# octree-nn/octfusion

Measured on AMD Instinct MI355X. Metric: denoising-steps/sec (depth-8 octree, batch 8), higher is better.
Workload: dtype f32 storage, fp16x3 products (fp16 hi + lo operand pairs = 22 significand bits, three fp16 MFMAs per product, fp32 accumulate)

## Files before the change

### include/ofx.h

```cpp
#ifndef OFX_H_
#define OFX_H_

#include <stddef.h>
#include <stdint.h>

#ifdef __cplusplus
extern "C" {
#endif

#define OFX_OK 0
#define OFX_EINVAL (-1)
#define OFX_ELAUNCH (-2)
#define OFX_ENODEV (-3)

#define OFX_ACT_NONE 0
#define OFX_ACT_SILU 1
#define OFX_ACT_GELU 2

#define OFX_MAX_DEPTH 16

int ofx_version(void);
const char* ofx_status_string(int status);
int ofx_device_check(void);
const char* ofx_build_hash(void);

int ofx_set_range_words(uint32_t* words);

int ofx_probe_mfma_sustained(int steps, int blocks, float* sink, unsigned long long* ticks, void* stream);

size_t ofx_scan_ws_bytes(int64_t n);
int ofx_scan_i32(const int32_t* in, int32_t* out, int64_t n, void* ws, void* stream);


int ofx_octree_full_layer(int depth, int batch_size, int64_t* keys, int32_t* children,
                          void* stream);
int ofx_octree_split(const int32_t* label, int64_t n, int32_t* children, int32_t* scan_out,
                     void* ws, void* stream);
int ofx_octree_grow(const int64_t* keys_parent, const int32_t* children_parent, int64_t n_parent,
                    int64_t* keys_child, int32_t* children_child, void* stream);
int ofx_split_small_label0(const float* split, int batch_size, int full_depth,
                           int32_t* label, void* stream);
int ofx_split_small_label1(const float* split, int batch_size, int full_depth,
                           const int32_t* children, int32_t* label1, void* stream);
int ofx_split_large_label0(const float* split, int64_t n, int32_t* label0, void* stream);
int ofx_split_large_label1(const float* split, int64_t n, const int32_t* children,
                           int32_t* label1, void* stream);
int ofx_octree2voxel_cf(const float* data, int64_t ld, int C, int batch_size, int depth,
                        float* vox, void* stream);
int ofx_voxel2octree_cf(const float* vox, int C, int batch_size, int depth, float* data,
                        int64_t ld, void* stream);

typedef struct {
  int depth, full_depth, batch_size;
  const int32_t* child_all;
  const int64_t* key_all;
  const int32_t* leafrank_all;
  const int64_t* nnum_host;
  const int64_t* nnum_nempty_host;
} ofx_tree_t;

size_t ofx_points_sort_ws_bytes(int64_t n);
int ofx_points_keys(const float* pts, int64_t ldp, const int32_t* batch_id, int batch_const, int64_t n, int depth,
                    int64_t* keys, int32_t* idx, void* stream);
int ofx_points_sort(const int64_t* keys_in, const int32_t* idx_in, int64_t n, int64_t* keys_out, int32_t* idx_out,
                    void* ws, size_t ws_bytes, void* stream);
int ofx_octree_label_from_points(const int64_t* sorted_keys, int64_t n_pts, const int64_t* node_keys, int64_t nnum,
                                 int depth_pts, int d, int32_t* label, void* stream);
int ofx_octree_point_features(const int64_t* sorted_keys, const int32_t* sorted_idx, int64_t n_pts, const float* pts,
                              int64_t ldp, const float* normals, int64_t ldn, const int64_t* node_keys, int64_t nnum,
                              int depth, float* feat, float* avg_points, float* avg_normals, void* stream);
size_t ofx_tree_leafrank_ws_bytes(int64_t max_nnum);
int ofx_tree_leafrank(const int32_t* child_all, const int64_t* nnum_host, int depth,
                      int32_t* leafrank_all, void* ws, void* stream);
int ofx_graph_nodes(const ofx_tree_t* tree, int d, int32_t* batch_id, uint8_t* node_type,
                    int64_t* keyd, uint8_t* node_mask, void* stream);
int ofx_graph_count(const ofx_tree_t* tree, int d, int32_t* seg_cnt, void* stream);
int ofx_graph_fill(const ofx_tree_t* tree, int d, const int32_t* seg_ptr, int32_t* col,
                   void* stream);
int ofx_graph_expand(const int32_t* seg_ptr, int64_t n_nodes, const int32_t* col,
                     int64_t* row_out, int64_t* col_out, int64_t* dir_out, void* stream);
int ofx_graph_primary(const int32_t* seg_ptr, const int32_t* col, int64_t n_nodes, int32_t* nbr,
                      void* stream);
int ofx_graph_reverse_count(const int32_t* seg_ptr, const int32_t* col, int64_t n_nodes, int32_t* rev_cnt,
                            void* stream);
int ofx_graph_reverse_fill(const int32_t* seg_ptr, const int32_t* col, int64_t n_nodes, const int32_t* rev_ptr,
                           int32_t* cursor, int32_t* rev_row, float* rev_w, void* stream);
int ofx_graph_primary_w(const int32_t* seg_ptr, const int32_t* col, const float* w, int64_t n_nodes, int32_t* nbr,
                        void* stream);
int ofx_graph_multi_flag_w(const int32_t* seg_ptr, const float* w, int64_t n_nodes, int32_t* flag, void* stream);
int ofx_graph_primary_ext_w(const int32_t* seg_ptr, const int32_t* col, const float* w, int64_t n_nodes,
                            const int32_t* rank, int32_t* nbr_ext, int32_t* multi_seg, void* stream);
int ofx_graphconv_bwd_data(const float* dy, int64_t ldy, int cout, int64_t n_nodes, const int32_t* nbr_rev,
                           const int32_t* rev_ptr, const int32_t* rev_row, const float* rev_w,
                           const int32_t* nbr_ext_rev, const int32_t* multi_seg, int64_t n_multi, float* aux,
                           const float* WpT, int64_t KpT, int cin, float* dx, int64_t ldx, void* ws, size_t ws_bytes,
                           void* stream);
int ofx_graphconv_bwd_weight(const float* x, int64_t ldx, int cin, int64_t n_nodes, const int32_t* nbr,
                             const int32_t* seg_ptr, const int32_t* col, const int32_t* nbr_ext,
                             const int32_t* multi_seg, int64_t n_multi, float* aux, const float* type_frac, int64_t ldt,
                             int nt_pad, const float* dy, int64_t ldy, int cout, float* dWp, int64_t Kp, void* ws,
                             size_t ws_bytes, void* stream);
int ofx_gn_backward(const float* x, int64_t ldx, const float* dy, int64_t ldy, int64_t n, int C,
                    const int32_t* batch_id, int batch_size, const float* count, int groups, float count_eps,
                    const float* mean, const float* rstd, const float* w, const float* bias, int act, double* sums,
                    float* coef, float* dx, int64_t lddx, float* dgamma, float* dbeta, void* stream);
int ofx_gemm_tn_f32(const float* P, int64_t ldp, const float* Q, int64_t ldq, int64_t rows, int64_t K, int64_t N,
                    float* out, void* ws, size_t ws_bytes, void* stream);
int ofx_table_reverse_count(const int32_t* nbr, int64_t n_out, int ndir, int64_t n_in, int32_t* rev_cnt, void* stream);
int ofx_table_reverse_fill(const int32_t* nbr, int64_t n_out, int ndir, int64_t n_in, const int32_t* rev_ptr,
                           int32_t* cursor, int32_t* rev_row, float* rev_w, void* stream);
int ofx_seg_primary_w(const int32_t* seg_ptr, const int32_t* col, const float* w, int64_t nseg, int32_t* nbr,
                      void* stream);
int ofx_seg_multi_flag_w(const int32_t* seg_ptr, const float* w, int64_t nseg, int32_t* flag, void* stream);
int ofx_seg_primary_ext_w(const int32_t* seg_ptr, const int32_t* col, const float* w, int64_t nseg, int64_t n_src,
                          const int32_t* rank, int32_t* nbr_ext, int32_t* multi_seg, void* stream);
int ofx_gridconv_bwd_data(const float* dy, int64_t ldy, int cout, int64_t n_out, int64_t n_in, const int32_t* nbr_rev,
                          const int32_t* rev_ptr, const int32_t* rev_row, const float* rev_w,
                          const int32_t* nbr_ext_rev, const int32_t* multi_seg, int64_t n_multi, float* aux,
                          const float* WpT, int cin, float* dx, int64_t ldx, void* ws, size_t ws_bytes, void* stream);
int ofx_gridconv_bwd_weight(const float* x, int64_t ldx, int cin, int64_t n_in, int64_t n_out, const int32_t* nbr27,
                            const int32_t* nbr27_ext, const float* zero_row, const float* dy, int64_t ldy, int cout,
                            float* dWp, void* ws, size_t ws_bytes, void* stream);
int ofx_adamw_step(float* param, const float* grad, float* exp_avg, float* exp_avg_sq, int64_t n, float lr,
                   float beta1, float beta2, float eps, float weight_decay, int step, void* stream);
int ofx_ema_update(float* ema, const float* param, int64_t n, float beta, void* stream);
int ofx_mpu_eval(const ofx_tree_t* tree, int depth_start, int depth_end, const float* pts, int64_t n_pts,
                 const float* code, float* sdf, uint8_t* mask, void* stream);
int ofx_mpu_eval_grid(const ofx_tree_t* tree, int depth_start, int depth_end, const float* code, int size,
                      float step, float bbmin, int batch_index, int64_t head, int64_t count, float* sdf,
                      uint8_t* mask, void* stream);
int ofx_mpu_eval_grad(const ofx_tree_t* tree, int depth_start, int depth_end, const float* pts, int64_t n_pts,
                      const float* code, float* sdf, float* grad, uint8_t* mask, void* stream);
int ofx_mpu_backward(const ofx_tree_t* tree, int depth_start, int depth_end, const float* pts, int64_t n_pts,
                     const float* code, const float* dsdf, const float* dgrad, float* dcode, void* stream);
int ofx_octree_ce(const float* logits, int64_t ld, const int32_t* child, int64_t n, float dscale, double* sums,
                  float* dlogits, int64_t ldd, void* stream);
int ofx_sdf_reg_loss(const float* sdf, const float* grad, const float* sdf_gt, const float* grad_gt, int64_t n,
                     float w_sdf, float w_grad, double* sums, float* dsdf, float* dgrad, void* stream);
int ofx_kl_sample_fwd(const float* params, int64_t ld, const float* noise, int64_t n, int embed_dim, float* z,
                      double* kl_sum, void* stream);
int ofx_kl_sample_bwd(const float* params, int64_t ld, const float* noise, const float* dz, int64_t n,
                      int embed_dim, float kl_scale, float* dparams, int64_t ldp, void* stream);
int ofx_graph_multi_flag(const int32_t* seg_ptr, int64_t n_nodes, int32_t* flag, void* stream);
int ofx_graph_primary_ext(const int32_t* seg_ptr, const int32_t* col, int64_t n_nodes,
                          const int32_t* rank, int32_t* nbr_ext, int32_t* multi_seg, void* stream);
int ofx_graph_type_frac(const int32_t* seg_ptr, const int32_t* col, const uint8_t* node_type,
                        int64_t n_nodes, int nt, float* type_frac, int64_t ld, void* stream);

int ofx_set_precision(int mode);
int ofx_get_precision(void);
int64_t ofx_packed_floats(int64_t Kp, int64_t N);
int64_t ofx_packed_k(int64_t K);
int64_t ofx_graphconv_packed_k(int cin, int nt);
int ofx_pack_weights(const float* W, int64_t sk, int64_t sn, int64_t K, int64_t N,
                     int cin, int nt, float* Wp, int64_t Kp, void* stream);

int ofx_gemm_f32(const float* A, int64_t lda, const int32_t* a_rows, int64_t M, int64_t K,
                 const float* Wp, int64_t Kp, int64_t N, const float* bias,
                 const float* res, int64_t ldr, float* out, int64_t ldc,
                 const int32_t* out_rows, void* ws, size_t ws_bytes, void* stream);
int ofx_gemm_f32_planes(const float* A, int64_t lda, const int32_t* a_rows, int64_t M, int64_t K,
                        const float* Wp, int64_t Kp, int64_t N, const float* bias,
                        const float* res, int64_t ldr, float* out, int64_t ldc,
                        const int32_t* out_rows, void* ws, size_t ws_bytes, int out_mode, void* stream);

int ofx_graphconv_fwd(const float* x, int64_t ldx, int cin, int64_t n_nodes,
                      const int32_t* nbr, const int32_t* seg_ptr, const int32_t* col,
                      const int32_t* nbr_ext, const int32_t* multi_seg, int64_t n_multi, float* aux,
                      const float* type_frac, int64_t ldt, int nt_pad,
                      const float* Wp, int64_t Kp, int cout, const float* bias,
                      const float* emb, int64_t lde, const int32_t* batch_id,
                      const float* res, int64_t ldr, float* out, int64_t ldc,
                      double* stats , int64_t stats_ld,
                      void* ws, size_t ws_bytes, void* stream);

int ofx_graphconv_narrow_in(const float* x, int64_t ldx, int cin, int64_t n_nodes, const int32_t* seg_ptr,
                            const int32_t* col, const uint8_t* node_type, int nt, const float* W, int cout,
                            const float* bias, const int32_t* batch_id, float* out, int64_t ldc,
                            double* stats , int64_t stats_ld, void* ws, size_t ws_bytes, void* stream);
int ofx_graphconv_narrow_in_tab(const float* x, int64_t ldx, int cin, int64_t n_nodes, const int32_t* seg_ptr,
                                const int32_t* col, const int32_t* nbr_ext, const int32_t* multi_seg, int64_t n_multi,
                                void* aux, const uint8_t* node_type, int nt, const float* W, int cout, const float* bias,
                                const int32_t* batch_id, float* out, int64_t ldc, double* stats ,
                                int64_t stats_ld, void* ws, size_t ws_bytes, void* stream);
int ofx_narrow_out_pack(const float* W, int C, int nt, int cout, int pw, float* Wd, void* stream);
int ofx_narrow_out_type_term(const float* type_frac, int64_t ldt, int nt, int64_t n_nodes, const float* W, int C,
                             int cout, const float* bias, float* type_term, void* stream);
int ofx_graphconv_narrow_out(const float* P, int64_t ldp, int cout, int64_t n_nodes, const int32_t* seg_ptr,
                             const int32_t* col, const float* type_term , float* out, int64_t ldc,
                             void* stream);

int ofx_planes_split(const float* x, int64_t ldx, int64_t n, int C, int Cpad, int mode, void* out,
                     int64_t ldo_bytes, void* stream);
int ofx_planes_merge(const void* planes, int64_t ldp_bytes, int64_t n, int C, int mode, float* out, int64_t ldo,
                     void* stream);
int ofx_gn_apply_planes(const float* x, int64_t ldx, int64_t n, int C, const int32_t* batch_id, const float* mean,
                        const float* rstd, const double* sums, const float* count, int groups, float eps,
                        float count_eps, const float* w, const float* bias, int act, int mode, void* out,
                        int64_t ldo_bytes, const int32_t* seg_ptr, const int32_t* col, const int32_t* multi_seg,
                        int64_t n_multi, void* aux , const int32_t* aux_plan ,
                        int64_t aux_left, void* stream);
int ofx_gn_apply_planes_oct(const float* x, int64_t ldx, int64_t n, int C, const int32_t* batch_id, const float* mean,
                            const float* rstd, const double* sums, const float* count, int groups, float eps,
                            float count_eps, const float* w, const float* bias, int act, int mode, void* out,
                            int64_t ldo_bytes, int64_t n_multi, void* aux, const int32_t* oct_ptr,
                            const int32_t* oct_ent, int64_t n_own, int shift, const int32_t* left_head,
                            const int32_t* left_src, int64_t n_left, void* stream);
int ofx_gn_apply_rows(void);
int64_t ofx_planes_packed_ktiles(int cin, int nt, int mode);
int64_t ofx_planes_packed_bytes(int cin, int nt, int cout, int mode);
int ofx_pack_weights_planes(const float* W, int64_t sk, int64_t sn, int cin, int nt, int cout, int mode, void* out,
                            void* stream);
int ofx_graphconv_fwd_planes(const void* xp, int64_t ldx_bytes, int cin, int64_t n_nodes, const int32_t* seg_ptr,
                             const int32_t* col, const int32_t* nbr_ext, const int32_t* multi_seg, int64_t n_multi,
                             void* aux, size_t aux_bytes, const void* tfp, int64_t ldt_bytes, int nt, const void* W2,
                             int cout, const float* bias, const float* emb, int64_t lde, const int32_t* batch_id,
                             const float* res, int64_t ldr, float* out, int64_t ldc, double* stats ,
                             int64_t stats_ld, void* ws, size_t ws_bytes, void* sync , size_t sync_bytes,
                             int mode, int aux_ready, void* stream);
int ofx_set_gconv_persistent(int on);
int64_t ofx_gemm_planes_packed_bytes(int K, int N, int mode);
int ofx_pack_gemm_planes(const float* W, int64_t sk, int64_t sn, int K, int N, int mode, void* out, void* stream);
int ofx_gemm_planes(const void* ap, int64_t lda_bytes, int64_t n_a, int64_t M, int K, const int32_t* row_tab,
                    const void* W2, int N, const float* bias, float* out, int64_t ldc, int out_mode, void* ws,
                    size_t ws_bytes, void* sync, size_t sync_bytes, int mode, void* stream);
int ofx_set_gconv_cus(int cus);
int ofx_gconv3_plan(int64_t n_rows, int cout, int nkt, int wm, int ni, int cus, int32_t* out, int64_t out_len);
int ofx_set_gconv2_tile(int wm);

int ofx_grid_conv_table(int mode, int depth_out, int batch_size, int32_t pad, int32_t* nbr27,
                        void* stream);
int64_t ofx_conv3d_packed_k(int cin);
int ofx_pack_conv3d(const float* W, int cin, int cout, float* Wp, void* stream);
int ofx_gridconv_fwd(const float* x, int64_t ldx, int cin, int64_t n_in, int64_t n_out,
                     const int32_t* nbr27 ,
                     const int32_t* nbr27_ext ,
                     const float* zero_row ,
                     const float* Wp, int cout, const float* bias, const float* emb, int64_t lde,
                     const int32_t* batch_id, const float* res, int64_t ldr, float* out,
                     int64_t ldc, void* ws, size_t ws_bytes, void* stream);
int ofx_gather_gemm_f32(const float* x, int64_t ldx, int cin, int ntap, int64_t n_src, int64_t n_out, const int32_t* tab,
                        const float* zero_row, const float* Wp, int64_t Kp, int cout, const float* bias,
                        const float* res, int64_t ldr, float* out, int64_t ldc, const int32_t* out_rows, void* ws,
                        size_t ws_bytes, int out_mode, void* stream);
int ofx_set_attention_split(int on);
int ofx_attention(const float* qkv, int64_t ldq, int batch_size, int T, int heads, int ch,
                  float* out, int64_t ldo, void* stream);

int ofx_attention_bwd(const float* qkv, int64_t ldq, const float* dout, int64_t ldo, int batch_size, int T, int heads,
                      int ch, float* rowstat, float* dqkv, int64_t ldd, void* stream);

int ofx_gather_mean(const float* x, int64_t ldx, int cin, int64_t n_nodes,
                    const int32_t* seg_ptr, const int32_t* col, float* col_data,
                    void* stream);

int ofx_gn_stats(const float* x, int64_t ldx, int64_t n, int C, const int32_t* batch_id,
                 int batch_size, double* sums, void* stream);
int ofx_gn_stats_acc(const float* x, int64_t ldx, int64_t n, int C, const int32_t* batch_id, int batch_size,
                     double* sums, void* stream);
int ofx_gn_finalize(const double* sums, const float* count, int batch_size, int C, int groups,
                    float eps, float count_eps, float* mean, float* rstd, void* stream);
int ofx_gn_apply(const float* x, int64_t ldx, int64_t n, int C, const int32_t* batch_id,
                 const float* mean , const float* rstd , const double* sums ,
                 const float* count, int groups, float eps, float count_eps, const float* w, const float* bias,
                 int act, float* out, int64_t ldo, void* stream);

int ofx_gn_fused_rows(const float* x, int64_t ldx, int rows_per_batch, int batch_size, int C, int groups, float eps,
                      float count_eps, const float* w, const float* bias, int act, float* out, int64_t ldo,
                      void* stream);

int ofx_set_gn_rows16(int on);

int ofx_rows_copy(const float* src, int64_t lds, const int32_t* smap, float* dst, int64_t ldd,
                  const int32_t* dmap, int64_t n, int C, void* stream);
int ofx_rows_copy_planes(const float* src, int64_t lds, const int32_t* smap, float* dst, int64_t ldd,
                         const int32_t* dmap, int64_t n, int C, int mode, void* stream);
int ofx_act(const float* x, float* y, int64_t n, int act, void* stream);
int ofx_timestep_embedding(const float* t, int batch_size, int dim, float max_period,
                           float* out, void* stream);
int ofx_learned_sinusoid(const float* t, const float* w, int batch_size, int half, float* out, void* stream);
int ofx_linear_small(const float* a, int64_t lda, int M, int K, const float* W, int64_t ldw, int N, const float* bias,
                     const float* res, int64_t ldr, int act_in, int act_out, float* out, int64_t ldo, void* stream);
int ofx_ddim_eps_update(float* x, const float* eps, const float* coef, float* x0_out, int64_t n,
                        void* stream);
int ofx_ddim_x0_update(float* x, const float* x0, const float* noise, const float* coef,
                       int64_t n, void* stream);

size_t ofx_mc_ws_bytes(int batch, int size);
int ofx_mc_count(const float* sdf, int batch, int size, float level, void* ws, int64_t* counts, void* stream);
int ofx_mc_emit(const float* sdf, int batch, int size, float level, float step, float bbmin, float scale, void* ws,
                const int64_t* vert_off, const int64_t* tri_off, float* verts, int32_t* faces, void* stream);
int ofx_mc_table_host(int8_t* tri_table, uint8_t* ntri);

size_t ofx_mesh_cc_ws_bytes(int64_t total_verts, int64_t total_faces, int batch);
int ofx_mesh_cc_label(const int32_t* faces, const int64_t* vert_off, const int64_t* tri_off, int batch,
                      int64_t total_verts, int64_t total_faces, int32_t* label, void* ws, int32_t* status,
                      void* stream);
int ofx_mesh_cc_table(const int32_t* faces, const int32_t* label, const int64_t* vert_off, const int64_t* tri_off,
                      int batch, int64_t total_verts, int64_t total_faces, int32_t* comp_of_vert, int32_t* comp_off,
                      void* ws, const int32_t* status, void* stream);
int ofx_mesh_cc_stats(const float* verts, const int32_t* faces, const int32_t* label, const int64_t* vert_off,
                      const int64_t* tri_off, int batch, int64_t total_verts, int64_t total_faces, int64_t n_comp,
                      int32_t* table, void* ws, const int32_t* status, void* stream);
int ofx_mesh_cc_select(const float* verts, const int32_t* faces, const int32_t* label, const int64_t* vert_off,
                       const int64_t* tri_off, int batch, int64_t total_verts, int64_t total_faces,
                       int32_t* winner_label, int64_t* keep_counts, void* ws, const int32_t* status, void* stream);
int ofx_mesh_cc_extract(const float* verts, const int32_t* faces, const int64_t* vert_off, const int64_t* tri_off,
                        int batch, int64_t total_verts, int64_t total_faces, const int64_t* new_vert_off,
                        const int64_t* new_tri_off, float* out_verts, int32_t* out_faces, void* ws,
                        const int32_t* status, void* stream);

#define OFX_EMD_MAX_POINTS 2048
size_t ofx_surface_sample_ws_bytes(int batch, int64_t total_faces);
int ofx_surface_sample(const float* verts, const int32_t* faces, const int64_t* offs, const int64_t* ids, int batch,
                       int64_t total_faces, int n, uint64_t seed, int normalize, void* ws, float* out, void* stream);
int ofx_nn_matrix(const float* a, int64_t na, int n, const float* b, int64_t nb, int m, float* d, void* stream);
int ofx_emd_matrix(const float* x, int64_t nx, const float* y, int64_t ny, int n, int m, float* e, void* stream);
uint64_t ofx_metrics_hash(uint64_t seed, int64_t shape, int64_t point, int draw);

#ifdef __cplusplus
}
#endif
#endif
```

### octfusion_amd/_lib.py

```python
import ctypes
import os

import torch

_HERE = os.path.dirname(os.path.abspath(__file__))
LIB_PATH = os.environ.get('OFX_LIB', os.path.join(_HERE, 'libofx.so'))

c_p = ctypes.c_void_p
c_i = ctypes.c_int
c_l = ctypes.c_int64
c_f = ctypes.c_float
c_sz = ctypes.c_size_t
c_u64 = ctypes.c_uint64


class OfxTree(ctypes.Structure):
    _fields_ = [('depth', c_i), ('full_depth', c_i), ('batch_size', c_i),
                ('child_all', c_p), ('key_all', c_p), ('leafrank_all', c_p),
                ('nnum_host', c_p), ('nnum_nempty_host', c_p)]


_SIGS = {
    'ofx_version': (c_i, [], False),
    'ofx_status_string': (ctypes.c_char_p, [c_i], False),
    'ofx_device_check': (c_i, [], False),
    'ofx_build_hash': (ctypes.c_char_p, [], False),
    'ofx_probe_mfma_sustained': (c_i, [c_i, c_i, c_p, c_p, c_p], True),
    'ofx_scan_ws_bytes': (c_sz, [c_l], False),
    'ofx_scan_i32': (c_i, [c_p, c_p, c_l, c_p, c_p], True),
    'ofx_octree_full_layer': (c_i, [c_i, c_i, c_p, c_p, c_p], True),
    'ofx_octree_split': (c_i, [c_p, c_l, c_p, c_p, c_p, c_p], True),
    'ofx_octree_grow': (c_i, [c_p, c_p, c_l, c_p, c_p, c_p], True),
    'ofx_split_small_label0': (c_i, [c_p, c_i, c_i, c_p, c_p], True),
    'ofx_split_small_label1': (c_i, [c_p, c_i, c_i, c_p, c_p, c_p], True),
    'ofx_split_large_label0': (c_i, [c_p, c_l, c_p, c_p], True),
    'ofx_split_large_label1': (c_i, [c_p, c_l, c_p, c_p, c_p], True),
    'ofx_octree2voxel_cf': (c_i, [c_p, c_l, c_i, c_i, c_i, c_p, c_p], True),
    'ofx_voxel2octree_cf': (c_i, [c_p, c_i, c_i, c_i, c_p, c_l, c_p], True),
    'ofx_points_sort_ws_bytes': (c_sz, [c_l], False),
    'ofx_points_keys': (c_i, [c_p, c_l, c_p, c_i, c_l, c_i, c_p, c_p, c_p], True),
    'ofx_points_sort': (c_i, [c_p, c_p, c_l, c_p, c_p, c_p, c_sz, c_p], True),
    'ofx_octree_label_from_points': (c_i, [c_p, c_l, c_p, c_l, c_i, c_i, c_p, c_p], True),
    'ofx_octree_point_features': (c_i, [c_p, c_p, c_l, c_p, c_l, c_p, c_l, c_p, c_l, c_i, c_p, c_p, c_p, c_p], True),
    'ofx_tree_leafrank_ws_bytes': (c_sz, [c_l], False),
    'ofx_tree_leafrank': (c_i, [c_p, c_p, c_i, c_p, c_p, c_p], True),
    'ofx_graph_nodes': (c_i, [ctypes.POINTER(OfxTree), c_i, c_p, c_p, c_p, c_p, c_p], True),
    'ofx_graph_count': (c_i, [ctypes.POINTER(OfxTree), c_i, c_p, c_p], True),
    'ofx_graph_reverse_count': (c_i, [c_p, c_p, c_l, c_p, c_p], True),
    'ofx_graph_reverse_fill': (c_i, [c_p, c_p, c_l, c_p, c_p, c_p, c_p, c_p], True),
    'ofx_graph_primary_w': (c_i, [c_p, c_p, c_p, c_l, c_p, c_p], True),
    'ofx_graph_multi_flag_w': (c_i, [c_p, c_p, c_l, c_p, c_p], True),
    'ofx_graph_primary_ext_w': (c_i, [c_p, c_p, c_p, c_l, c_p, c_p, c_p, c_p], True),
    'ofx_graphconv_bwd_data': (c_i, [c_p, c_l, c_i, c_l, c_p, c_p, c_p, c_p, c_p, c_p, c_l, c_p, c_p, c_l, c_i, c_p,
                                     c_l, c_p, c_sz, c_p], True),
    'ofx_graphconv_bwd_weight': (c_i, [c_p, c_l, c_i, c_l, c_p, c_p, c_p, c_p, c_p, c_l, c_p, c_p, c_l, c_i, c_p, c_l,
                                       c_i, c_p, c_l, c_p, c_sz, c_p], True),
    'ofx_gn_backward': (c_i, [c_p, c_l, c_p, c_l, c_l, c_i, c_p, c_i, c_p, c_i, c_f, c_p, c_p, c_p, c_p, c_i, c_p, c_p,
                              c_p, c_l, c_p, c_p, c_p], True),
    'ofx_gemm_tn_f32': (c_i, [c_p, c_l, c_p, c_l, c_l, c_l, c_l, c_p, c_p, c_sz, c_p], True),
    'ofx_table_reverse_count': (c_i, [c_p, c_l, c_i, c_l, c_p, c_p], True),
    'ofx_table_reverse_fill': (c_i, [c_p, c_l, c_i, c_l, c_p, c_p, c_p, c_p, c_p], True),
    'ofx_seg_primary_w': (c_i, [c_p, c_p, c_p, c_l, c_p, c_p], True),
    'ofx_seg_multi_flag_w': (c_i, [c_p, c_p, c_l, c_p, c_p], True),
    'ofx_seg_primary_ext_w': (c_i, [c_p, c_p, c_p, c_l, c_l, c_p, c_p, c_p, c_p], True),
    'ofx_gridconv_bwd_data': (c_i, [c_p, c_l, c_i, c_l, c_l, c_p, c_p, c_p, c_p, c_p, c_p, c_l, c_p, c_p, c_i, c_p, c_l,
                                    c_p, c_sz, c_p], True),
    'ofx_gridconv_bwd_weight': (c_i, [c_p, c_l, c_i, c_l, c_l, c_p, c_p, c_p, c_p, c_l, c_i, c_p, c_p, c_sz, c_p], True),
    'ofx_attention_bwd': (c_i, [c_p, c_l, c_p, c_l, c_i, c_i, c_i, c_i, c_p, c_p, c_l, c_p], True),
    'ofx_adamw_step': (c_i, [c_p, c_p, c_p, c_p, c_l, c_f, c_f, c_f, c_f, c_f, c_i, c_p], True),
    'ofx_ema_update': (c_i, [c_p, c_p, c_l, c_f, c_p], True),
    'ofx_gn_fused_rows': (c_i, [c_p, c_l, c_i, c_i, c_i, c_i, c_f, c_f, c_p, c_p, c_i, c_p, c_l, c_p], True),
    'ofx_set_gn_rows16': (c_i, [c_i], True),
    'ofx_mpu_eval': (c_i, [ctypes.POINTER(OfxTree), c_i, c_i, c_p, c_l, c_p, c_p, c_p, c_p], True),
    'ofx_mpu_eval_grid': (c_i, [ctypes.POINTER(OfxTree), c_i, c_i, c_p, c_i, c_f, c_f, c_i, c_l, c_l, c_p, c_p, c_p], True),
    'ofx_mpu_eval_grad': (c_i, [ctypes.POINTER(OfxTree), c_i, c_i, c_p, c_l, c_p, c_p, c_p, c_p, c_p], True),
    'ofx_mpu_backward': (c_i, [ctypes.POINTER(OfxTree), c_i, c_i, c_p, c_l, c_p, c_p, c_p, c_p, c_p], True),
    'ofx_octree_ce': (c_i, [c_p, c_l, c_p, c_l, c_f, c_p, c_p, c_l, c_p], True),
    'ofx_sdf_reg_loss': (c_i, [c_p, c_p, c_p, c_p, c_l, c_f, c_f, c_p, c_p, c_p, c_p], True),
    'ofx_kl_sample_fwd': (c_i, [c_p, c_l, c_p, c_l, c_i, c_p, c_p, c_p], True),
    'ofx_kl_sample_bwd': (c_i, [c_p, c_l, c_p, c_p, c_l, c_i, c_f, c_p, c_l, c_p], True),
    'ofx_graph_fill': (c_i, [ctypes.POINTER(OfxTree), c_i, c_p, c_p, c_p], True),
    'ofx_graph_expand': (c_i, [c_p, c_l, c_p, c_p, c_p, c_p, c_p], True),
    'ofx_graph_type_frac': (c_i, [c_p, c_p, c_p, c_l, c_i, c_p, c_l, c_p], True),
    'ofx_set_precision': (c_i, [c_i], True),
    'ofx_set_range_words': (c_i, [c_p], True),
    'ofx_get_precision': (c_i, [], False),
    'ofx_gn_apply_rows': (c_i, [], False),
    'ofx_set_attention_split': (c_i, [c_i], True),
    'ofx_gather_gemm_f32': (c_i, [c_p, c_l, c_i, c_i, c_l, c_l, c_p, c_p, c_p, c_l, c_i, c_p, c_p, c_l, c_p, c_l, c_p, c_p, c_sz, c_i, c_p], True),
    'ofx_graphconv_narrow_in_tab': (c_i, [c_p, c_l, c_i, c_l, c_p, c_p, c_p, c_p, c_l, c_p, c_p, c_i, c_p, c_i, c_p, c_p, c_p, c_l, c_p, c_l,
                                          c_p, c_sz, c_p], True),
    'ofx_graphconv_narrow_in': (c_i, [c_p, c_l, c_i, c_l, c_p, c_p, c_p, c_i, c_p, c_i, c_p, c_p, c_p, c_l, c_p, c_l, c_p, c_sz, c_p], True),
    'ofx_narrow_out_pack': (c_i, [c_p, c_i, c_i, c_i, c_i, c_p, c_p], True),
    'ofx_narrow_out_type_term': (c_i, [c_p, c_l, c_i, c_l, c_p, c_i, c_i, c_p, c_p, c_p], True),
    'ofx_graphconv_narrow_out': (c_i, [c_p, c_l, c_i, c_l, c_p, c_p, c_p, c_p, c_l, c_p], True),
    'ofx_packed_floats': (c_l, [c_l, c_l], False),
    'ofx_packed_k': (c_l, [c_l], False),
    'ofx_graphconv_packed_k': (c_l, [c_i, c_i], False),
    'ofx_pack_weights': (c_i, [c_p, c_l, c_l, c_l, c_l, c_i, c_i, c_p, c_l, c_p], True),
    'ofx_gemm_f32': (c_i, [c_p, c_l, c_p, c_l, c_l, c_p, c_l, c_l, c_p, c_p, c_l, c_p, c_l, c_p, c_p, c_sz, c_p], True),
    'ofx_gemm_f32_planes': (c_i, [c_p, c_l, c_p, c_l, c_l, c_p, c_l, c_l, c_p, c_p, c_l, c_p, c_l, c_p, c_p, c_sz, c_i, c_p], True),
    'ofx_graphconv_fwd': (c_i, [c_p, c_l, c_i, c_l, c_p, c_p, c_p, c_p, c_p, c_l, c_p, c_p, c_l, c_i, c_p, c_l,
                                c_i, c_p, c_p, c_l, c_p, c_p, c_l, c_p, c_l, c_p, c_l, c_p, c_sz, c_p], True),
    'ofx_planes_split': (c_i, [c_p, c_l, c_l, c_i, c_i, c_i, c_p, c_l, c_p], True),
    'ofx_planes_merge': (c_i, [c_p, c_l, c_l, c_i, c_i, c_p, c_l, c_p], True),
    'ofx_gn_apply_planes': (c_i, [c_p, c_l, c_l, c_i, c_p, c_p, c_p, c_p, c_p, c_i, c_f, c_f, c_p, c_p, c_i, c_i, c_p,
                                  c_l, c_p, c_p, c_p, c_l, c_p, c_p, c_l, c_p], True),
    'ofx_gn_apply_planes_oct': (c_i, [c_p, c_l, c_l, c_i, c_p, c_p, c_p, c_p, c_p, c_i, c_f, c_f, c_p, c_p, c_i, c_i, c_p,
                                      c_l, c_l, c_p, c_p, c_p, c_l, c_i, c_p, c_p, c_l, c_p], True),
    'ofx_planes_packed_ktiles': (c_l, [c_i, c_i, c_i], False),
    'ofx_planes_packed_bytes': (c_l, [c_i, c_i, c_i, c_i], False),
    'ofx_pack_weights_planes': (c_i, [c_p, c_l, c_l, c_i, c_i, c_i, c_i, c_p, c_p], True),
    'ofx_graphconv_fwd_planes': (c_i, [c_p, c_l, c_i, c_l, c_p, c_p, c_p, c_p, c_l, c_p, c_sz, c_p, c_l, c_i, c_p, c_i,
                                       c_p, c_p, c_l, c_p, c_p, c_l, c_p, c_l, c_p, c_l, c_p, c_sz, c_p, c_sz, c_i, c_i,
                                       c_p], True),
    'ofx_set_gconv_persistent': (c_i, [c_i], True),
    'ofx_set_gconv_cus': (c_i, [c_i], True),
    'ofx_gemm_planes_packed_bytes': (c_l, [c_i, c_i, c_i], False),
    'ofx_pack_gemm_planes': (c_i, [c_p, c_l, c_l, c_i, c_i, c_i, c_p, c_p], True),
    'ofx_gemm_planes': (c_i, [c_p, c_l, c_l, c_l, c_i, c_p, c_p, c_i, c_p, c_p, c_l, c_i, c_p, c_sz, c_p, c_sz, c_i, c_p], False),
    'ofx_gconv3_plan': (c_i, [c_l, c_i, c_i, c_i, c_i, c_i, c_p, c_l], False),
    'ofx_set_gconv2_tile': (c_i, [c_i], True),
    'ofx_graph_multi_flag': (c_i, [c_p, c_l, c_p, c_p], True),
    'ofx_graph_primary_ext': (c_i, [c_p, c_p, c_l, c_p, c_p, c_p, c_p], True),
    'ofx_graph_primary': (c_i, [c_p, c_p, c_l, c_p, c_p], True),
    'ofx_grid_conv_table': (c_i, [c_i, c_i, c_i, c_i, c_p, c_p], True),
    'ofx_conv3d_packed_k': (c_l, [c_i], False),
    'ofx_pack_conv3d': (c_i, [c_p, c_i, c_i, c_p, c_p], True),
    'ofx_gridconv_fwd': (c_i, [c_p, c_l, c_i, c_l, c_l, c_p, c_p, c_p, c_p, c_i, c_p, c_p, c_l, c_p, c_p, c_l, c_p,
                               c_l, c_p, c_sz, c_p], True),
    'ofx_attention': (c_i, [c_p, c_l, c_i, c_i, c_i, c_i, c_p, c_l, c_p], True),
    'ofx_gather_mean': (c_i, [c_p, c_l, c_i, c_l, c_p, c_p, c_p, c_p], True),
    'ofx_gn_stats': (c_i, [c_p, c_l, c_l, c_i, c_p, c_i, c_p, c_p], True),
    'ofx_gn_stats_acc': (c_i, [c_p, c_l, c_l, c_i, c_p, c_i, c_p, c_p], True),
    'ofx_gn_finalize': (c_i, [c_p, c_p, c_i, c_i, c_i, c_f, c_f, c_p, c_p, c_p], True),
    'ofx_gn_apply': (c_i, [c_p, c_l, c_l, c_i, c_p, c_p, c_p, c_p, c_p, c_i, c_f, c_f, c_p, c_p, c_i, c_p, c_l, c_p], True),
    'ofx_rows_copy': (c_i, [c_p, c_l, c_p, c_p, c_l, c_p, c_l, c_i, c_p], True),
    'ofx_rows_copy_planes': (c_i, [c_p, c_l, c_p, c_p, c_l, c_p, c_l, c_i, c_i, c_p], True),
    'ofx_act': (c_i, [c_p, c_p, c_l, c_i, c_p], True),
    'ofx_timestep_embedding': (c_i, [c_p, c_i, c_i, c_f, c_p, c_p], True),
    'ofx_learned_sinusoid': (c_i, [c_p, c_p, c_i, c_i, c_p, c_p], True),
    'ofx_linear_small': (c_i, [c_p, c_l, c_i, c_i, c_p, c_l, c_i, c_p, c_p, c_l, c_i, c_i, c_p, c_l, c_p], True),
    'ofx_ddim_eps_update': (c_i, [c_p, c_p, c_p, c_p, c_l, c_p], True),
    'ofx_ddim_x0_update': (c_i, [c_p, c_p, c_p, c_p, c_l, c_p], True),
    'ofx_mc_ws_bytes': (c_sz, [c_i, c_i], False),
    'ofx_mc_count': (c_i, [c_p, c_i, c_i, c_f, c_p, c_p, c_p], True),
    'ofx_mc_emit': (c_i, [c_p, c_i, c_i, c_f, c_f, c_f, c_f, c_p, c_p, c_p, c_p, c_p, c_p], True),
    'ofx_mc_table_host': (c_i, [c_p, c_p], True),
    'ofx_mesh_cc_ws_bytes': (c_sz, [c_l, c_l, c_i], False),
    'ofx_mesh_cc_label': (c_i, [c_p, c_p, c_p, c_i, c_l, c_l, c_p, c_p, c_p, c_p], True),
    'ofx_mesh_cc_table': (c_i, [c_p, c_p, c_p, c_p, c_i, c_l, c_l, c_p, c_p, c_p, c_p, c_p], True),
    'ofx_mesh_cc_stats': (c_i, [c_p, c_p, c_p, c_p, c_p, c_i, c_l, c_l, c_l, c_p, c_p, c_p, c_p], True),
    'ofx_mesh_cc_select': (c_i, [c_p, c_p, c_p, c_p, c_p, c_i, c_l, c_l, c_p, c_p, c_p, c_p, c_p], True),
    'ofx_mesh_cc_extract': (c_i, [c_p, c_p, c_p, c_p, c_i, c_l, c_l, c_p, c_p, c_p, c_p, c_p, c_p, c_p], True),
    'ofx_surface_sample_ws_bytes':(c_sz, [c_i, c_l], False),
    'ofx_surface_sample': (c_i, [c_p, c_p, c_p, c_p, c_i, c_l, c_i, c_u64, c_i, c_p, c_p, c_p], True),
    'ofx_nn_matrix': (c_i, [c_p, c_l, c_i, c_p, c_l, c_i, c_p, c_p], True),
    'ofx_emd_matrix': (c_i, [c_p, c_l, c_p, c_l, c_i, c_i, c_p, c_p], True),
    'ofx_metrics_hash': (c_u64, [c_u64, c_l, c_l, c_i], False),
}

EXPORTS = sorted(_SIGS)


class OfxError(RuntimeError):
    pass


_lib = None


def lib():
    global _lib
    if _lib is None:
        if not os.path.exists(LIB_PATH):
            raise OfxError('libofx.so not built: run `python -m octfusion_amd.build` '
                           '(the product has no CPU / eager fallback)')
        L = ctypes.CDLL(LIB_PATH)
        for name, (res, args, _) in _SIGS.items():
            fn = getattr(L, name)
            fn.restype = res
            fn.argtypes = args
        _check_fresh(L)
        _lib = L
    return _lib


def _check_fresh(L):
    if 'OFX_LIB' in os.environ:
        return
    from . import build
    try:
        want = build.source_hash()
    except OSError:
        return
    have = L.ofx_build_hash().decode()
    if have != want:
        raise OfxError('libofx.so is stale: built from sources %s, the tree is %s -- run `python -m octfusion_amd.build`'
                       % (have, want))


PROFILE = None
META = None


def _timed(prof, name, args, always):
    global META
    meta, META = META, None
    e0 = torch.cuda.Event(enable_timing=True)
    e1 = torch.cuda.Event(enable_timing=True)
    e0.record()
    rc = getattr(lib(), name)(*args)
    e1.record()
    if always or rc == 0:
        prof.append((name, e0, e1, meta))
    return rc


def call(name, *args):
    prof = PROFILE
    if prof is not None and _SIGS[name][2]:
        rc = _timed(prof, name, args, True)
    else:
        rc = getattr(lib(), name)(*args)
    if _SIGS[name][2] and rc != 0:
        msg = lib().ofx_status_string(rc).decode()
        raise OfxError('%s failed: %s (%d)' % (name, msg, rc))
    return rc


def call_may_decline(name, *args):
    prof = PROFILE
    if prof is not None:
        rc = _timed(prof, name, args, False)
    else:
        rc = getattr(lib(), name)(*args)
    if rc < 0:
        raise OfxError('%s failed with status %d' % (name, rc))
    return rc == 0


def ptr(t):
    if t is None:
        return None
    return t.data_ptr()


def stream():
    return torch.cuda.current_stream().cuda_stream


def require_device():
    if not torch.cuda.is_available():
        raise OfxError('no HIP device: octfusion_amd has no CPU path')
    rc = lib().ofx_device_check()
    if rc != 0:
        raise OfxError('ofx_device_check: %s' % lib().ofx_status_string(rc).decode())
```

### octfusion_amd/csrc/ofx_gemm.hip

```cpp
#include "ofx_gemm_common.h"

constexpr int BM = 128;
constexpr int BK = 32;
constexpr int A_LD = BK + 4;
constexpr int MODE_DENSE = 0;
constexpr int MODE_GATHER = 1;


__device__ __forceinline__ float4 gather_seg4(const GemmArgs& g, int64_t row, int dir, int cc) {
  const int64_t s = row * g.ndir + dir;
  const int32_t a = g.seg_ptr[s], e = g.seg_ptr[s + 1];
  float4 acc = f4zero();
  if (g.edge_w) {
    for (int32_t p = a; p < e; ++p) {
      const float w = g.edge_w[p];
      const float4 v = *reinterpret_cast<const float4*>(g.x + (int64_t)g.col[p] * g.ldx + cc);
      acc.x += w * v.x; acc.y += w * v.y; acc.z += w * v.z; acc.w += w * v.w;
    }
    return acc;
  }
  for (int32_t p = a; p < e; ++p) f4add(acc, *reinterpret_cast<const float4*>(g.x + (int64_t)g.col[p] * g.ldx + cc));
  if (e - a > 1) {
    const float inv = 1.f / (float)(e - a);
    acc.x *= inv; acc.y *= inv; acc.z *= inv; acc.w *= inv;
// ... 818 lines not shown
}

__global__ void __launch_bounds__(256) splitk_reduce_kernel(const GemmArgs g) {
  const int64_t total = g.M * g.N;
  for (int64_t t = (int64_t)blockIdx.x * blockDim.x + threadIdx.x; t < total; t += (int64_t)gridDim.x * blockDim.x) {
    const int64_t m = t / g.N, n = t - m * g.N;
    float v = 0.f;
    for (int s = 0; s < g.nsplit; ++s) v += g.ws[(int64_t)s * total + t];
    if (g.oscale_p) v *= *g.oscale_p;
    if (g.bias) v += g.bias[n];
    if (g.emb) v += g.emb[(int64_t)g.bid[m] * g.lde + n];
    if (g.res) v += g.res[m * g.ldr + n];
    int64_t om = m;
    if (g.out_rows) { om = g.out_rows[m]; if (om < 0) continue; }
    g.out[om * g.ldc + n] = v;
  }
}

__global__ void __launch_bounds__(256) splitk_reduce_v4_kernel(const GemmArgs g) {
  const int64_t n4 = g.N >> 2, total4 = g.M * n4, total = g.M * g.N;
  for (int64_t t = (int64_t)blockIdx.x * blockDim.x + threadIdx.x; t < total4; t += (int64_t)gridDim.x * blockDim.x) {
    const int64_t m = t / n4, n = (t - m * n4) * 4;
    const float* p = g.ws + m * g.N + n;
    float4 v = f4zero();
    int s = 0;
    for (; s + 7 < g.nsplit; s += 8) {
      float4 a[8];
#pragma unroll
      for (int u = 0; u < 8; ++u) a[u] = *reinterpret_cast<const float4*>(p + (int64_t)(s + u) * total);
#pragma unroll
      for (int u = 0; u < 8; ++u) f4add(v, a[u]);
    }
    for (; s + 3 < g.nsplit; s += 4) {
      const float4 a0 = *reinterpret_cast<const float4*>(p + (int64_t)s * total);
      const float4 a1 = *reinterpret_cast<const float4*>(p + (int64_t)(s + 1) * total);
      const float4 a2 = *reinterpret_cast<const float4*>(p + (int64_t)(s + 2) * total);
      const float4 a3 = *reinterpret_cast<const float4*>(p + (int64_t)(s + 3) * total);
      f4add(v, a0); f4add(v, a1); f4add(v, a2); f4add(v, a3);
    }
    for (; s < g.nsplit; ++s) f4add(v, *reinterpret_cast<const float4*>(p + (int64_t)s * total));
    if (g.oscale_p) { const float osc = *g.oscale_p; v.x *= osc; v.y *= osc; v.z *= osc; v.w *= osc; }
    if (g.bias) f4add(v, *reinterpret_cast<const float4*>(g.bias + n));
    if (g.emb) f4add(v, *reinterpret_cast<const float4*>(g.emb + (int64_t)g.bid[m] * g.lde + n));
    if (g.res) f4add(v, *reinterpret_cast<const float4*>(g.res + m * g.ldr + n));
    int64_t om = m;
    if (g.out_rows) { om = g.out_rows[m]; if (om < 0) continue; }
    if (g.out_planes) ofx_store_planes4(g.out, om * g.ldc + n, v, g.out_planes);
    else *reinterpret_cast<float4*>(g.out + om * g.ldc + n) = v;
  }
}

template <int MODE, int WM, int WN, int MI, int NI>
static int launch_cfg(GemmArgs& g, hipStream_t st) {
  constexpr int BN = WN * NI * 32;
  constexpr size_t lds = (2 * BM * A_LD + 2 * 8 * BN * 4) * sizeof(float);
  static bool attr_set[OFX_MAX_DEVICES] = {};
  if (lds > 64 * 1024 &&
      !ofx_raise_lds_limit(reinterpret_cast<const void*>(&gemm_kernel<MODE, WM, WN, MI, NI>), (int)lds, attr_set))
    return OFX_ELAUNCH;
  gemm_kernel<MODE, WM, WN, MI, NI><<<g.ntm * g.ntn * g.nsplit, 256, lds, st>>>(g);
  return OFX_OK;
}

template <int MODE, int WM, int WN, int MI, int NI>
static int launch_fast_cfg(GemmArgs& g, hipStream_t st) {
  constexpr int BN = WN * NI * 32;
  constexpr size_t lds = (2 * BM * A_LD + 2 * 8 * BN * 4) * sizeof(float);
  static bool attr_set[OFX_MAX_DEVICES] = {};
  if (lds > 64 * 1024 &&
      !ofx_raise_lds_limit(reinterpret_cast<const void*>(&gemm_fast_kernel<MODE, WM, WN, MI, NI>), (int)lds, attr_set))
    return OFX_ELAUNCH;
  gemm_fast_kernel<MODE, WM, WN, MI, NI><<<g.ntm * g.ntn * g.nsplit, 256, lds, st>>>(g);
  return OFX_OK;
}

template <int MODE, int WM, int WN, int MI, int NI, int H16>
static int launch_bf16x3_h(GemmArgs& g, hipStream_t st) {
  constexpr int BN = WN * NI * 32;
  constexpr size_t lds = 2 * (2 * BM * 80);
  static bool attr_set[OFX_MAX_DEVICES] = {};
  if (lds > 64 * 1024 &&
      !ofx_raise_lds_limit(reinterpret_cast<const void*>(&gemm_pairs_x3_kernel<MODE, WM, WN, MI, NI, H16>), (int)lds, attr_set))
    return OFX_ELAUNCH;
  gemm_pairs_x3_kernel<MODE, WM, WN, MI, NI, H16><<<g.ntm * g.ntn * g.nsplit, 256, lds, st>>>(g);
  return OFX_OK;
}
template <int MODE, int WM, int WN, int MI, int NI>
static int launch_bf16x3_cfg(GemmArgs& g, hipStream_t st) {
  return g_precision == 3 ? launch_bf16x3_h<MODE, WM, WN, MI, NI, 1>(g, st) : launch_bf16x3_h<MODE, WM, WN, MI, NI, 0>(g, st);
}

__global__ void __launch_bounds__(256) stats_reduce_kernel(const float* __restrict__ part, int64_t nwr, int wr_rows,
                                                            int64_t N, const int32_t* __restrict__ bid,
                                                            double* __restrict__ stats, int64_t stats_ld) {
  __shared__ double red[3][64][2];
  const int c = threadIdx.x & 63, rg = threadIdx.x >> 6;
  const int64_t n = (int64_t)blockIdx.y * 64 + c;
  const int64_t w0 = (int64_t)blockIdx.x * 64;
  const int64_t nc = n < N ? n : N - 1;
  int b[16];
  float2 v[16];
#pragma unroll
  for (int i = 0; i < 16; ++i) {
    const int64_t w = w0 + rg * 16 + i;
    const int64_t wc = w < nwr ? w : nwr - 1;
    b[i] = bid[wc * wr_rows];
    v[i] = *reinterpret_cast<const float2*>(part + (wc * N + nc) * 2);
    if (w >= nwr) { b[i] = -1; v[i] = make_float2(0.f, 0.f); }
  }
  const int bfirst = bid[w0 * wr_rows];
  bool ok = true;
#pragma unroll
  for (int i = 0; i < 16; ++i) ok = ok && (b[i] == bfirst || b[i] < 0);
  const bool uni = __syncthreads_and(ok);
  auto flush = [&](int bb, double s, double q) {
    double* o = stats + ((int64_t)bb * stats_ld + n) * 2;
    unsafeAtomicAdd(o, s); unsafeAtomicAdd(o + 1, q);
  };
  if (uni) {
    double s = 0.0, q = 0.0;
#pragma unroll
    for (int i = 0; i < 16; ++i) { s += (double)v[i].x; q += (double)v[i].y; }
    if (rg > 0) { red[rg - 1][c][0] = s; red[rg - 1][c][1] = q; }
    __syncthreads();
    if (rg == 0 && n < N) {
#pragma unroll
      for (int r = 0; r < 3; ++r) { s += red[r][c][0]; q += red[r][c][1]; }
      flush(bfirst, s, q);
    }
  } else if (n < N) {
    double s = 0.0, q = 0.0;
    int sb = -1;
#pragma unroll
    for (int i = 0; i < 16; ++i) {
      if (b[i] < 0) continue;
      if (b[i] != sb) {
        if (sb >= 0) flush(sb, s, q);
        sb = b[i]; s = 0.0; q = 0.0;
      }
      s += (double)v[i].x; q += (double)v[i].y;
    }
    if (sb >= 0) flush(sb, s, q);
  }
}

int ofx_launch_stats_reduce(const GemmArgs& g, int wr_rows, hipStream_t st) {
  const int64_t nwr = ofx_cdiv(g.M, wr_rows);
  stats_reduce_kernel<<<dim3((unsigned)ofx_cdiv(nwr, 64), (unsigned)ofx_cdiv(g.N, 64)), 256, 0, st>>>(
      g.stats_part, nwr, wr_rows, g.N, g.bid, g.stats, g.stats_ld);
  OFX_LAUNCH_CHECK();
  return OFX_OK;
}

template <int MODE>
static int launch_gemm(GemmArgs& g, float* ws, size_t ws_bytes, hipStream_t st) {
  if (g.M <= 0 || g.N <= 0) return OFX_OK;
  {
    auto al16 = [](const void* p) { return (reinterpret_cast<uintptr_t>(p) & 15) == 0; };
    g.vec4 = g.N % 4 == 0 && al16(g.out) && g.ldc % 4 == 0 && (!g.res || (al16(g.res) && g.ldr % 4 == 0)) &&
             (!g.emb || (al16(g.emb) && g.lde % 4 == 0)) && (!g.bias || al16(g.bias));
  }
  const int bn = g.N <= 32 ? 32 : (g.N <= 64 ? 64 : 128);
  g.ntm = (int)ofx_cdiv(g.M, BM);
  g.ntn = (int)ofx_cdiv(g.N, bn);
  const int nkt = (int)(g.Kp / BK);
  int nsplit = 1;
  const int tiles = g.ntm * g.ntn;
  if (ws && tiles < 256 && nkt >= 8) {
    nsplit = (int)ofx_cdiv(512, tiles);
    if (nsplit > nkt / 4) nsplit = nkt / 4;
    if (nsplit > 64) nsplit = 64;
    const size_t per = (size_t)g.M * g.N * sizeof(float);
    if ((size_t)nsplit * per > ws_bytes) nsplit = (int)(ws_bytes / per);
    if (nsplit < 2) nsplit = 1;
  }
  g.kt_per_split = (int)ofx_cdiv(nkt, nsplit);
  nsplit = (int)ofx_cdiv(nkt, g.kt_per_split);
  g.nsplit = nsplit;
  g.ws = ws;
  int rc;
  bool fast;
  if (MODE == MODE_GATHER) {
    fast = g.fast && g.nbr_ext && g.aux && (!g.out_rows || g.gather_out_rows);
  } else {
    fast = ((g.lda & 3) == 0) && ((g.K & 3) == 0) && g.K >= 4 && ((((uintptr_t)g.A) & 15) == 0);
    if (fast) { g.ndir = 1; g.n_src = 0; g.aux = g.A; g.tf = g.A; g.ldt = g.lda; g.nbr_ext = (const int32_t*)g.A; }
  }
  g.W16 = (g_precision != 1) ? reinterpret_cast<const uint16_t*>(g.Wp + g.Kp * g.N) : nullptr;
  const int wr_rows = bn == 32 ? 32 : 64;
  const int64_t nwr = ofx_cdiv(g.M, wr_rows);
  if (!(g.stats && g.vec4 && nsplit == 1 && g.stats_part &&
        (size_t)nwr * g.N * 2 * sizeof(float) <= g.stats_part_bytes && (((uintptr_t)g.stats_part) & 15) == 0))
    g.stats_part = nullptr;
  g.oscale_p = (fast && g.W16) ? g.Wp + 2 * g.Kp * g.N : nullptr;
  if (fast && g.W16) {
    if (bn == 32) rc = launch_bf16x3_cfg<MODE, 4, 1, 1, 1>(g, st);
    else if (bn == 64) rc = launch_bf16x3_cfg<MODE, 2, 2, 2, 1>(g, st);
    else rc = launch_bf16x3_cfg<MODE, 2, 2, 2, 2>(g, st);
  } else if (fast) {
    if (bn == 32) rc = launch_fast_cfg<MODE, 4, 1, 1, 1>(g, st);
    else if (bn == 64) rc = launch_fast_cfg<MODE, 2, 2, 2, 1>(g, st);
    else rc = launch_fast_cfg<MODE, 2, 2, 2, 2>(g, st);
  } else if (bn == 32) rc = launch_cfg<MODE, 4, 1, 1, 1>(g, st);
  else if (bn == 64) rc = launch_cfg<MODE, 2, 2, 2, 1>(g, st);
  else rc = launch_cfg<MODE, 2, 2, 2, 2>(g, st);
  if (rc) return rc;
  if (nsplit > 1) {
    const bool ws16 = (((uintptr_t)g.ws) & 15) == 0;
    if (g.vec4 && ws16) splitk_reduce_v4_kernel<<<ofx_grid(g.M * (g.N >> 2), 256), 256, 0, st>>>(g);
    else splitk_reduce_kernel<<<ofx_grid(g.M * g.N, 256), 256, 0, st>>>(g);
  }
  if (g.stats_part) {
    rc = ofx_launch_stats_reduce(g, wr_rows, st);
    if (rc) return rc;
  }
  OFX_LAUNCH_CHECK();
  return OFX_OK;
}

static inline int64_t pad32(int64_t v) { return (v + 31) / 32 * 32; }
static int pack_bf16x3(const float* Wp, int64_t Kp, int64_t N, hipStream_t st);

extern "C" int64_t ofx_packed_k(int64_t K) { return pad32(K); }
extern "C" int64_t ofx_graphconv_packed_k(int cin, int nt) {
  return pad32(7 * (int64_t)cin) + (nt > 1 ? pad32(7 * (int64_t)nt) : 0);
}

__global__ void pack_weights_kernel(const float* __restrict__ W, int64_t sk, int64_t sn, int64_t K, int64_t N, int cin,
                                    int nt, float* __restrict__ Wp, int64_t Kp) {
  const int64_t total = (Kp / 4) * N;
  const int ntc = nt > 1 ? nt : 0;
  const int64_t Kf = (7 * (int64_t)cin + 31) / 32 * 32;
  for (int64_t t = (int64_t)blockIdx.x * blockDim.x + threadIdx.x; t < total; t += (int64_t)gridDim.x * blockDim.x) {
    const int64_t kq = t / N, n = t - kq * N;
    float v[4];
#pragma unroll
    for (int kk = 0; kk < 4; ++kk) {
      const int64_t k = kq * 4 + kk;
      int64_t src = -1;
      if (cin > 0) {
        if (k < 7 * (int64_t)cin) {
          const int64_t dir = k / cin, c = k - dir * cin;
          src = dir * (cin + ntc) + c;
        } else if (k >= Kf && ntc > 0 && k - Kf < 7 * (int64_t)ntc) {
          const int64_t kt = k - Kf, dir = kt / ntc, ty = kt - dir * ntc;
          src = dir * (cin + ntc) + cin + ty;
        }
      } else if (k < K) {
        src = k;
      }
      v[kk] = src >= 0 ? W[src * sk + n * sn] : 0.f;
    }
    *reinterpret_cast<float4*>(Wp + t * 4) = make_float4(v[0], v[1], v[2], v[3]);
  }
}

extern "C" int ofx_pack_weights(const float* W, int64_t sk, int64_t sn, int64_t K, int64_t N, int cin, int nt,
                                float* Wp, int64_t Kp, void* stream) {
  if (!W || !Wp || K < 1 || N < 1 || (Kp & 31) || cin < 0 || nt < 0) return OFX_EINVAL;
  if (cin > 0) {
    if (Kp != ofx_graphconv_packed_k(cin, nt) || K != 7 * (int64_t)(cin + (nt > 1 ? nt : 0))) return OFX_EINVAL;
  } else if (Kp != pad32(K)) {
    return OFX_EINVAL;
  }
  if (((uintptr_t)Wp & 15) != 0) return OFX_EINVAL;
  pack_weights_kernel<<<ofx_grid((Kp / 4) * N, 256), 256, 0, ofx_stream(stream)>>>(W, sk, sn, K, N, cin, nt, Wp, Kp);
  if (int rc = pack_bf16x3(Wp, Kp, N, ofx_stream(stream))) return rc;
  OFX_LAUNCH_CHECK();
  return OFX_OK;
}

__global__ void pack_conv3d_kernel(const float* __restrict__ W, int cin, int64_t N, float* __restrict__ Wp, int64_t Kp) {
  const int64_t total = (Kp / 4) * N;
  for (int64_t t = (int64_t)blockIdx.x * blockDim.x + threadIdx.x; t < total; t += (int64_t)gridDim.x * blockDim.x) {
    const int64_t kq = t / N, n = t - kq * N;
    float v[4];
#pragma unroll
    for (int kk = 0; kk < 4; ++kk) {
      const int64_t k = kq * 4 + kk;
      float w = 0.f;
      if (k < 27 * (int64_t)cin) {
        const int64_t tap = k / cin, c = k - tap * cin;
        w = W[(n * cin + c) * 27 + tap];
      }
      v[kk] = w;
    }
    *reinterpret_cast<float4*>(Wp + t * 4) = make_float4(v[0], v[1], v[2], v[3]);
  }
}

extern "C" int64_t ofx_conv3d_packed_k(int cin) { return pad32(27 * (int64_t)cin); }

extern "C" int ofx_pack_conv3d(const float* W, int cin, int cout, float* Wp, void* stream) {
  if (!W || !Wp || cin < 1 || cout < 1 || ((uintptr_t)Wp & 15)) return OFX_EINVAL;
  const int64_t Kp = ofx_conv3d_packed_k(cin);
  pack_conv3d_kernel<<<ofx_grid((Kp / 4) * cout, 256), 256, 0, ofx_stream(stream)>>>(W, cin, cout, Wp, Kp);
  if (int rc = pack_bf16x3(Wp, Kp, cout, ofx_stream(stream))) return rc;
  OFX_LAUNCH_CHECK();
  return OFX_OK;
}

extern "C" int ofx_gemm_f32_planes(const float* A, int64_t lda, const int32_t* a_rows, int64_t M, int64_t K,
                                   const float* Wp, int64_t Kp, int64_t N, const float* bias, const float* res, int64_t ldr,
                                   float* out, int64_t ldc, const int32_t* out_rows, void* ws, size_t ws_bytes,
                                   int out_mode, void* stream) {
  if (M == 0 && K >= 1 && N >= 1) return OFX_OK;
  if (M < 0 || K < 1 || N < 1 || !Wp || !out || (M > 0 && !A) || Kp != pad32(K) || lda < K || ldc < N ||
      (res && ldr < N) || ((uintptr_t)Wp & 15))
    return OFX_EINVAL;
  if (out_mode != 0 && out_mode != 2 && out_mode != 3) return OFX_EINVAL;
  if (out_mode && ((N & 3) || (ldc & 31) || ((uintptr_t)out & 127) || (res && ((ldr & 3) || ((uintptr_t)res & 15))) ||
                   (bias && ((uintptr_t)bias & 15)) || ((uintptr_t)ws & 15)))
    return OFX_EINVAL;
  GemmArgs g = {};
  g.A = A; g.lda = lda; g.a_rows = a_rows;
  g.M = M; g.K = K; g.Wp = Wp; g.Kp = Kp; g.N = N; g.bias = bias;
  g.res = res; g.ldr = ldr; g.out = out; g.ldc = ldc; g.out_rows = out_rows; g.out_planes = out_mode;
  return launch_gemm<MODE_DENSE>(g, (float*)ws, ws_bytes, ofx_stream(stream));
}
extern "C" int ofx_gemm_f32(const float* A, int64_t lda, const int32_t* a_rows, int64_t M, int64_t K, const float* Wp,
                            int64_t Kp, int64_t N, const float* bias, const float* res, int64_t ldr, float* out,
                            int64_t ldc, const int32_t* out_rows, void* ws, size_t ws_bytes, void* stream) {
  return ofx_gemm_f32_planes(A, lda, a_rows, M, K, Wp, Kp, N, bias, res, ldr, out, ldc, out_rows, ws, ws_bytes, 0, stream);
}

static int gather_common(GemmArgs& g, const float* x, int64_t ldx, int cin, int ndir, int64_t n_rows,
                         const int32_t* nbr, const int32_t* seg_ptr, const int32_t* col, const float* Wp, int64_t Kp,
                         int cout, const float* bias, const float* emb, int64_t lde, const int32_t* batch_id,
                         const float* res, int64_t ldr, float* out, int64_t ldc) {
  if (n_rows < 0 || cin < 1 || cout < 1 || !x || !nbr || !Wp || !out || ldx < cin || ldc < cout ||
      (res && ldr < cout) || (emb && (!batch_id || lde < cout)) || ((uintptr_t)Wp & 15))
    return OFX_EINVAL;
  g.x = x; g.ldx = ldx; g.cin = cin; g.ndir = ndir;
  g.fast = (cin % 32 == 0) && ((ldx & 3) == 0) && (((uintptr_t)x & 15) == 0);
  g.nbr = nbr; g.seg_ptr = seg_ptr; g.col = col;
  g.Kf = pad32((int64_t)ndir * cin);
  g.M = n_rows; g.K = Kp; g.Wp = Wp; g.Kp = Kp; g.N = cout; g.bias = bias;
  g.emb = emb; g.lde = lde; g.bid = batch_id; g.res = res; g.ldr = ldr; g.out = out; g.ldc = ldc;
  return OFX_OK;
}

__global__ void __launch_bounds__(256) col_rows_kernel(const GemmArgs g, int64_t row0, int64_t rows,
                                                       float* __restrict__ colbuf) {
  const int64_t k4n = g.Kp >> 2, total = rows * k4n;
  for (int64_t t = (int64_t)blockIdx.x * blockDim.x + threadIdx.x; t < total; t += (int64_t)gridDim.x * blockDim.x) {
    const int64_t r = t / k4n, k = (t - r * k4n) * 4;
    const int64_t row = row0 + r;
    float v[4];
#pragma unroll
    for (int kk = 0; kk < 4; ++kk)
      v[kk] = (k + kk < g.Kf) ? gather_elem(g, row, k + kk) : g.tf[row * g.ldt + (k + kk - g.Kf)];
    *reinterpret_cast<float4*>(colbuf + t * 4) = make_float4(v[0], v[1], v[2], v[3]);
  }
}

template <int MODE> static int launch_gemm(GemmArgs& g, float* ws, size_t ws_bytes, hipStream_t st);

static int launch_gather_via_col(const GemmArgs& g, float* ws, size_t ws_bytes, hipStream_t st) {
  if (!ws || (((uintptr_t)ws) & 15)) return -1;
  size_t tail = ws_bytes / 8;
  if (tail > (size_t(16) << 20)) tail = size_t(16) << 20;
  tail &= ~size_t(15);
  const size_t row_bytes = (size_t)g.Kp * sizeof(float);
  int64_t chunk = (int64_t)((ws_bytes - tail) / row_bytes) / 128 * 128;
  if (chunk < 128) return -1;
  float* tail_ws = reinterpret_cast<float*>(reinterpret_cast<char*>(ws) + (ws_bytes - tail));
  for (int64_t r0 = 0; r0 < g.M; r0 += chunk) {
    const int64_t rows = g.M - r0 < chunk ? g.M - r0 : chunk;
    col_rows_kernel<<<ofx_grid(rows * (g.Kp >> 2), 256), 256, 0, st>>>(g, r0, rows, ws);
    GemmArgs d = {};
    d.A = ws; d.lda = g.Kp; d.M = rows; d.K = g.Kp; d.Wp = g.Wp; d.Kp = g.Kp; d.N = g.N; d.bias = g.bias;
    d.emb = g.emb; d.lde = g.lde; d.bid = g.bid ? g.bid + r0 : nullptr;
    d.res = g.res ? g.res + r0 * g.ldr : nullptr; d.ldr = g.ldr;
    d.out = g.out + r0 * g.ldc; d.ldc = g.ldc;
    d.stats = g.stats; d.stats_ld = g.stats_ld;
    if (g.stats) { d.stats_part = tail_ws; d.stats_part_bytes = tail; }
    const int rc = launch_gemm<MODE_DENSE>(d, g.stats ? nullptr : tail_ws, tail, st);
    if (rc) return rc;
  }
  return OFX_OK;
}

extern "C" int ofx_graphconv_fwd(const float* x, int64_t ldx, int cin, int64_t n_nodes, const int32_t* nbr,
                                 const int32_t* seg_ptr, const int32_t* col, const int32_t* nbr_ext,
                                 const int32_t* multi_seg, int64_t n_multi, float* aux, const float* type_frac,
                                 int64_t ldt, int nt_pad, const float* Wp, int64_t Kp, int cout, const float* bias,
                                 const float* emb, int64_t lde, const int32_t* batch_id, const float* res, int64_t ldr,
                                 float* out, int64_t ldc, double* stats, int64_t stats_ld, void* ws, size_t ws_bytes,
                                 void* stream) {
  if (n_nodes == 0 && cin >= 1 && cout >= 1) return OFX_OK;
  GemmArgs g = {};
  int rc = gather_common(g, x, ldx, cin, 7, n_nodes, nbr, seg_ptr, col, Wp, Kp, cout, bias, emb, lde, batch_id, res,
                         ldr, out, ldc);
  if (rc) return rc;
  if (!seg_ptr || !col) return OFX_EINVAL;
  if (nt_pad < 0 || (nt_pad & 31) || Kp != g.Kf + nt_pad) return OFX_EINVAL;
  if (nt_pad > 0 && (!type_frac || ldt < nt_pad || (ldt & 3) || ((uintptr_t)type_frac & 15))) return OFX_EINVAL;
  g.tf = type_frac; g.ldt = ldt;
  if (stats) {
    if (!batch_id || stats_ld < cout) return OFX_EINVAL;
    g.stats = stats; g.stats_ld = stats_ld; g.bid = batch_id;
    g.stats_part = (float*)ws; g.stats_part_bytes = ws_bytes;
    ws = nullptr;
  }
  hipStream_t st = ofx_stream(stream);
  if (g.fast && nbr_ext && aux && n_nodes > 0 && (((uintptr_t)aux & 15) == 0)) {
    if (n_multi < 0 || (n_multi > 0 && !multi_seg)) return OFX_EINVAL;
    multi_mean_kernel<<<ofx_grid((n_multi + 1) * (cin / 4), 256), 256, 0, st>>>(x, ldx, cin, seg_ptr, col, multi_seg,
                                                                               n_multi, aux, ldx, nullptr);
    g.nbr_ext = nbr_ext; g.aux = aux; g.ldaux = ldx; g.n_src = n_nodes;
    if (!g.tf) { g.tf = x; g.ldt = ldx; }
  }
  if (!g.nbr_ext && n_nodes > 0) {
    rc = launch_gather_via_col(g, stats ? g.stats_part : (float*)ws, stats ? g.stats_part_bytes : ws_bytes, st);
    if (rc >= 0) return rc;
  }
  return launch_gemm<MODE_GATHER>(g, (float*)ws, ws_bytes, st);
}

extern "C" int ofx_graphconv_bwd_data(const float* dy, int64_t ldy, int cout, int64_t n_nodes, const int32_t* nbr_rev,
                                      const int32_t* rev_ptr, const int32_t* rev_row, const float* rev_w,
                                      const int32_t* nbr_ext_rev, const int32_t* multi_seg, int64_t n_multi, float* aux,
                                      const float* WpT, int64_t KpT, int cin, float* dx, int64_t ldx, void* ws,
                                      size_t ws_bytes, void* stream) {
  if (n_nodes == 0 && cin >= 1 && cout >= 1) return OFX_OK;
  GemmArgs g = {};
  int rc = gather_common(g, dy, ldy, cout, 7, n_nodes, nbr_rev, rev_ptr, rev_row, WpT, KpT, cin, nullptr, nullptr, 0,
                         nullptr, nullptr, 0, dx, ldx);
  if (rc) return rc;
  if (!rev_ptr || !rev_row || !rev_w || KpT != g.Kf) return OFX_EINVAL;
  g.edge_w = rev_w;
  hipStream_t st = ofx_stream(stream);
  if (g.fast && nbr_ext_rev && aux && (((uintptr_t)aux & 15) == 0)) {
    if (n_multi < 0 || (n_multi > 0 && !multi_seg)) return OFX_EINVAL;
    multi_mean_kernel<<<ofx_grid((n_multi + 1) * (cout / 4), 256), 256, 0, st>>>(dy, ldy, cout, rev_ptr, rev_row,
                                                                                multi_seg, n_multi, aux, ldy, rev_w);
    g.nbr_ext = nbr_ext_rev; g.aux = aux; g.ldaux = ldy; g.n_src = n_nodes;
    g.tf = dy; g.ldt = ldy;
  } else {
    g.tf = dy; g.ldt = ldy;
    rc = launch_gather_via_col(g, (float*)ws, ws_bytes, st);
    if (rc >= 0) return rc;
  }
  return launch_gemm<MODE_GATHER>(g, (float*)ws, ws_bytes, st);
}

struct TnArgs {
  const float* P; int64_t ldp;
  const float* x; int64_t ldx; int cin; int ndir;
  const int32_t* nbr_ext; const float* aux; int64_t n_src;
  const float* tf; int64_t ldt; int64_t Kf;
  const float* Q; int64_t ldq;
  int64_t rows, row0, Kp, N;
  int64_t rows_per_slice;
  float* part;
};

template <bool DENSE_P, bool BF16X3>
__global__ void __launch_bounds__(256, 2) tn_gemm_kernel(const TnArgs a) {
  constexpr int LD = 132;
  constexpr int TP = 128 * 80;
  __shared__ __attribute__((aligned(16))) char tn_smem[BF16X3 ? 4 * TP : 2 * 32 * LD * 4];
  float* const Ps = reinterpret_cast<float*>(tn_smem);
  float* const Qs = Ps + 32 * LD;
  char* const Pt = tn_smem;
  char* const Qt = tn_smem + 2 * TP;
  const int lane = threadIdx.x & 63, wid = threadIdx.x >> 6;
  const int wm = wid >> 1, wn = wid & 1, l31 = lane & 31, h = lane >> 5;
  const int64_t m0 = (int64_t)blockIdx.x * 128, n0 = (int64_t)blockIdx.y * 128;
  const int64_t r_begin = (int64_t)blockIdx.z * a.rows_per_slice;
  const int64_t r_end = r_begin + a.rows_per_slice < a.rows ? r_begin + a.rows_per_slice : a.rows;
  f32x16 acc[2][2];
#pragma unroll
  for (int i = 0; i < 2; ++i)
#pragma unroll
    for (int j = 0; j < 2; ++j)
#pragma unroll
      for (int r = 0; r < 16; ++r) acc[i][j][r] = 0.f;
  const int q4 = threadIdx.x & 3;
  const int kr = BF16X3 ? q4 + 4 * (threadIdx.x >> 5) : threadIdx.x >> 3;
  const int f0 = BF16X3 ? (threadIdx.x >> 2) & 7 : threadIdx.x & 7;
  float4 vp[4], vq[4];
  auto load_tile = [&](int64_t r) {
    const int64_t row = r + kr;
    const bool rok = row < r_end;
#pragma unroll
    for (int p = 0; p < 4; ++p) {
      const int64_t m = m0 + 4 * (f0 + 8 * p), n = n0 + 4 * (f0 + 8 * p);
      float4 v = f4zero();
      if (rok && m < a.Kp) {
        if (DENSE_P) {
          v = *reinterpret_cast<const float4*>(a.P + row * a.ldp + m);
        } else if (m < a.Kf) {
          const int64_t kk = m;
          if (kk < a.ndir * (int64_t)a.cin) {
            const int dir = (int)(kk / a.cin), c = (int)(kk - (int64_t)dir * a.cin);
            const int64_t id = a.nbr_ext[(a.row0 + row) * a.ndir + dir];
            const float* src = id < a.n_src ? a.x + id * a.ldx : a.aux + (id - a.n_src) * a.ldx;
            v = *reinterpret_cast<const float4*>(src + c);
          }
        } else {
          v = *reinterpret_cast<const float4*>(a.tf + (a.row0 + row) * a.ldt + (m - a.Kf));
        }
      }
      vp[p] = v;
      float4 q = f4zero();
      if (rok && n < a.N) q = *reinterpret_cast<const float4*>(a.Q + row * a.ldq + n);
      vq[p] = q;
    }
// ... 154 lines not shown
    const int64_t rows = n_nodes - r0 < chunk ? n_nodes - r0 : chunk;
    col_rows_kernel<<<ofx_grid(rows * (Kp >> 2), 256), 256, 0, st>>>(g, r0, rows, colbuf);
    a.Q = dy + r0 * ldy; a.rows = rows; a.row0 = r0;
    a.rows_per_slice = ofx_cdiv(ofx_cdiv(rows, slices), 32) * 32;
    const int sl = (int)ofx_cdiv(rows, a.rows_per_slice);
    launch_tn<true>(a, dim3((unsigned)ofx_cdiv(Kp, 128), (unsigned)ofx_cdiv(cout, 128), (unsigned)sl), st);
    tn_reduce_kernel<<<ofx_grid(total, 256), 256, 0, st>>>(a.part, sl, total, dWp, first ? 0 : 1);
    first = 0;
  }
  OFX_LAUNCH_CHECK();
  return OFX_OK;
}

extern "C" int ofx_gridconv_bwd_data(const float* dy, int64_t ldy, int cout, int64_t n_out, int64_t n_in,
                                     const int32_t* nbr_rev, const int32_t* rev_ptr, const int32_t* rev_row,
                                     const float* rev_w, const int32_t* nbr_ext_rev, const int32_t* multi_seg,
                                     int64_t n_multi, float* aux, const float* WpT, int cin, float* dx, int64_t ldx,
                                     void* ws, size_t ws_bytes, void* stream) {
  if (n_in == 0 && cin >= 1 && cout >= 1) return OFX_OK;
  GemmArgs g = {};
  const int64_t KpT = ofx_conv3d_packed_k(cout);
  int rc = gather_common(g, dy, ldy, cout, 27, n_in, nbr_rev, rev_ptr, rev_row, WpT, KpT, cin, nullptr, nullptr, 0,
                         nullptr, nullptr, 0, dx, ldx);
  if (rc) return rc;
  if (!rev_ptr || !rev_row || !rev_w || n_out < 1) return OFX_EINVAL;
  g.edge_w = rev_w;
  g.tf = dy; g.ldt = ldy;
  hipStream_t st = ofx_stream(stream);
  if (g.fast && nbr_ext_rev && aux && (((uintptr_t)aux & 15) == 0)) {
    if (n_multi < 0 || (n_multi > 0 && !multi_seg)) return OFX_EINVAL;
    multi_mean_kernel<<<ofx_grid((n_multi + 1) * (cout / 4), 256), 256, 0, st>>>(dy, ldy, cout, rev_ptr, rev_row,
                                                                                multi_seg, n_multi, aux, ldy, rev_w);
    g.nbr_ext = nbr_ext_rev; g.aux = aux; g.ldaux = ldy; g.n_src = n_out;
  } else {
    rc = launch_gather_via_col(g, (float*)ws, ws_bytes, st);
    if (rc >= 0) return rc;
  }
  return launch_gemm<MODE_GATHER>(g, (float*)ws, ws_bytes, st);
}

extern "C" int ofx_gridconv_bwd_weight(const float* x, int64_t ldx, int cin, int64_t n_in, int64_t n_out,
                                       const int32_t* nbr27, const int32_t* nbr27_ext, const float* zero_row,
                                       const float* dy, int64_t ldy, int cout, float* dWp, void* ws, size_t ws_bytes,
                                       void* stream) {
  if (n_in < 1 || n_out < 0 || cin < 1 || cout < 1 || (cout & 3) || !x || !dy || !dWp || !ws || ldy < cout ||
      (ldy & 3) || ldx < cin || (((uintptr_t)dy | (uintptr_t)ws) & 15))
    return OFX_EINVAL;
  const int64_t Kp = ofx_conv3d_packed_k(cin), total = Kp * cout;
  hipStream_t st = ofx_stream(stream);
  if (n_out == 0) {
    if (hipMemsetAsync(dWp, 0, (size_t)total * sizeof(float), st) != hipSuccess) return OFX_ELAUNCH;
    return OFX_OK;
  }
  const int tiles = (int)(ofx_cdiv(Kp, 128) * ofx_cdiv(cout, 128));
  TnArgs a = {};
  a.Q = dy; a.ldq = ldy; a.Kp = Kp; a.N = cout; a.Kf = Kp; a.part = (float*)ws;
  const bool fast = (cin % 32 == 0) && ((ldx & 3) == 0) && (((uintptr_t)x & 15) == 0) && nbr27_ext && zero_row &&
                    (((uintptr_t)zero_row & 15) == 0);
  if (fast) {
    int slices = (int)ofx_cdiv(1024, tiles);
    if (slices > 256) slices = 256;
    if (slices > (int)ofx_cdiv(n_out, 32)) slices = (int)ofx_cdiv(n_out, 32);
    while (slices > 1 && (size_t)slices * total * sizeof(float) > ws_bytes) --slices;
    if ((size_t)slices * total * sizeof(float) > ws_bytes) return OFX_EINVAL;
    a.x = x; a.ldx = ldx; a.cin = cin; a.ndir = 27; a.nbr_ext = nbr27_ext; a.aux = zero_row; a.n_src = n_in;
    a.tf = x; a.ldt = ldx; a.rows = n_out; a.row0 = 0;
    a.rows_per_slice = ofx_cdiv(ofx_cdiv(n_out, slices), 32) * 32;
    slices = (int)ofx_cdiv(n_out, a.rows_per_slice);
    launch_tn<false>(a, dim3((unsigned)ofx_cdiv(Kp, 128), (unsigned)ofx_cdiv(cout, 128), (unsigned)slices), st);
    tn_reduce_kernel<<<ofx_grid(total, 256), 256, 0, st>>>(a.part, slices, total, dWp, 0);
    OFX_LAUNCH_CHECK();
    return OFX_OK;
  }
  if (!nbr27) return OFX_EINVAL;
  GemmArgs g = {};
  g.x = x; g.ldx = ldx; g.cin = cin; g.ndir = 27; g.nbr = nbr27; g.tf = x; g.ldt = ldx; g.Kf = Kp; g.Kp = Kp; g.M = n_out;
  int slices = (int)ofx_cdiv(512, tiles);
  if (slices > 64) slices = 64;
  const size_t part_bytes = ((size_t)slices * total * sizeof(float) + 255) & ~size_t(255);
  if (part_bytes >= ws_bytes) return OFX_EINVAL;
  int64_t chunk = (int64_t)((ws_bytes - part_bytes) / ((size_t)Kp * sizeof(float))) / 32 * 32;
  if (chunk < 32) return OFX_EINVAL;
  float* colbuf = reinterpret_cast<float*>(reinterpret_cast<char*>(ws) + part_bytes);
  a.P = colbuf; a.ldp = Kp;
  int first = 1;
  for (int64_t r0 = 0; r0 < n_out; r0 += chunk) {
    const int64_t rows = n_out - r0 < chunk ? n_out - r0 : chunk;
    col_rows_kernel<<<ofx_grid(rows * (Kp >> 2), 256), 256, 0, st>>>(g, r0, rows, colbuf);
    a.Q = dy + r0 * ldy; a.rows = rows; a.row0 = r0;
    a.rows_per_slice = ofx_cdiv(ofx_cdiv(rows, slices), 32) * 32;
    const int sl = (int)ofx_cdiv(rows, a.rows_per_slice);
    launch_tn<true>(a, dim3((unsigned)ofx_cdiv(Kp, 128), (unsigned)ofx_cdiv(cout, 128), (unsigned)sl), st);
    tn_reduce_kernel<<<ofx_grid(total, 256), 256, 0, st>>>(a.part, sl, total, dWp, first ? 0 : 1);
    first = 0;
  }
  OFX_LAUNCH_CHECK();
  return OFX_OK;
}

extern "C" int ofx_gemm_tn_f32(const float* P, int64_t ldp, const float* Q, int64_t ldq, int64_t rows, int64_t K,
                               int64_t N, float* out, void* ws, size_t ws_bytes, void* stream) {
  if (rows < 0 || K < 4 || N < 4 || (K & 3) || (N & 3) || !out || !ws || ldp < K || ldq < N || ((ldp | ldq) & 3) ||
      (rows > 0 && (!P || !Q)) || (((uintptr_t)P | (uintptr_t)Q | (uintptr_t)ws) & 15))
    return OFX_EINVAL;
  hipStream_t st = ofx_stream(stream);
  const int64_t total = K * N;
  if (rows == 0) {
    if (hipMemsetAsync(out, 0, (size_t)total * sizeof(float), st) != hipSuccess) return OFX_ELAUNCH;
    return OFX_OK;
  }
  const int tiles = (int)(ofx_cdiv(K, 128) * ofx_cdiv(N, 128));
  int slices = (int)ofx_cdiv(1024, tiles);
  if (slices > 256) slices = 256;
  if (slices > (int)ofx_cdiv(rows, 32)) slices = (int)ofx_cdiv(rows, 32);
  while (slices > 1 && (size_t)slices * total * sizeof(float) > ws_bytes) --slices;
  if ((size_t)slices * total * sizeof(float) > ws_bytes) return OFX_EINVAL;
  TnArgs a = {};
  a.P = P; a.ldp = ldp; a.Q = Q; a.ldq = ldq; a.Kp = K; a.N = N; a.Kf = K; a.rows = rows; a.row0 = 0;
  a.rows_per_slice = ofx_cdiv(ofx_cdiv(rows, slices), 32) * 32;
  slices = (int)ofx_cdiv(rows, a.rows_per_slice);
  a.part = (float*)ws;
  launch_tn<true>(a, dim3((unsigned)ofx_cdiv(K, 128), (unsigned)ofx_cdiv(N, 128), (unsigned)slices), st);
  tn_reduce_kernel<<<ofx_grid(total, 256), 256, 0, st>>>(a.part, slices, total, out, 0);
  OFX_LAUNCH_CHECK();
  return OFX_OK;
}

extern "C" int ofx_gridconv_fwd(const float* x, int64_t ldx, int cin, int64_t n_in, int64_t n_out,
                                const int32_t* nbr27, const int32_t* nbr27_ext, const float* zero_row,
                                const float* Wp, int cout,
                                const float* bias, const float* emb, int64_t lde, const int32_t* batch_id,
                                const float* res, int64_t ldr, float* out, int64_t ldc, void* ws, size_t ws_bytes,
                                void* stream) {
  if (n_out == 0 && cin >= 1 && cout >= 1) return OFX_OK;
  GemmArgs g = {};
  const int64_t Kp = ofx_conv3d_packed_k(cin);
  int rc = gather_common(g, x, ldx, cin, 27, n_out, nbr27 ? nbr27 : nbr27_ext, nullptr, nullptr, Wp, Kp, cout, bias,
                         emb, lde, batch_id, res, ldr, out, ldc);
  if (rc) return rc;
  if (n_in < 1) return OFX_EINVAL;
  if (g.fast && nbr27_ext && zero_row && (((uintptr_t)zero_row & 15) == 0)) {
    g.nbr_ext = nbr27_ext; g.aux = zero_row; g.ldaux = ldx; g.n_src = n_in;
    g.tf = x; g.ldt = ldx;
  } else if (!nbr27) {
    return OFX_EINVAL;
  }
  if (!g.nbr_ext) {
    rc = launch_gather_via_col(g, (float*)ws, ws_bytes, ofx_stream(stream));
    if (rc >= 0) return rc;
  }
  return launch_gemm<MODE_GATHER>(g, (float*)ws, ws_bytes, ofx_stream(stream));
}

extern "C" int ofx_gather_gemm_f32(const float* x, int64_t ldx, int cin, int ntap, int64_t n_src, int64_t n_out,
                                   const int32_t* tab, const float* zero_row, const float* Wp, int64_t Kp, int cout,
                                   const float* bias, const float* res, int64_t ldr, float* out, int64_t ldc,
                                   const int32_t* out_rows, void* ws, size_t ws_bytes, int out_mode, void* stream) {
  if (n_out == 0 && cin >= 1 && cout >= 1) return OFX_OK;
  if (ntap < 1 || ntap > 64 || n_src < 1 || !tab || !zero_row || ((uintptr_t)zero_row & 15) || (cin & 31) || (ldx & 3) ||
      ((uintptr_t)x & 15) || Kp != pad32((int64_t)ntap * cin))
    return OFX_EINVAL;
  if (out_mode != 0 && out_mode != 2 && out_mode != 3) return OFX_EINVAL;
  if (out_mode && ((cout & 3) || (ldc & 31) || ((uintptr_t)out & 127) || (res && ((ldr & 3) || ((uintptr_t)res & 15))) ||
                   (bias && ((uintptr_t)bias & 15)) || ((uintptr_t)ws & 15)))
    return OFX_EINVAL;
  GemmArgs g = {};
  int rc = gather_common(g, x, ldx, cin, ntap, n_out, tab, nullptr, nullptr, Wp, Kp, cout, bias, nullptr, 0, nullptr, res,
                         ldr, out, ldc);
  if (rc) return rc;
  if (!g.fast) return OFX_EINVAL;
  g.nbr_ext = tab; g.aux = zero_row; g.ldaux = ldx; g.n_src = n_src;
  g.tf = x; g.ldt = ldx;
  g.out_rows = out_rows; g.gather_out_rows = 1; g.out_planes = out_mode;
  return launch_gemm<MODE_GATHER>(g, (float*)ws, ws_bytes, ofx_stream(stream));
}

__global__ void __launch_bounds__(256) gather_mean_kernel(const float* __restrict__ x, int64_t ldx, int cin, int64_t nseg,
                                                          const int32_t* __restrict__ seg_ptr,
                                                          const int32_t* __restrict__ col, float* __restrict__ out) {
  const int c4n = cin >> 2;
  const int64_t total = nseg * c4n;
  for (int64_t t = (int64_t)blockIdx.x * blockDim.x + threadIdx.x; t < total; t += (int64_t)gridDim.x * blockDim.x) {
    const int64_t s = t / c4n;
    const int c = (int)(t - s * c4n) * 4;
    const int32_t a = seg_ptr[s], e = seg_ptr[s + 1];
    float4 acc = f4zero();
    for (int32_t p = a; p < e; ++p) f4add(acc, *reinterpret_cast<const float4*>(x + (int64_t)col[p] * ldx + c));
    if (e - a > 1) {
      const float inv = 1.f / (float)(e - a);
      acc.x *= inv; acc.y *= inv; acc.z *= inv; acc.w *= inv;
    }
    *reinterpret_cast<float4*>(out + s * cin + c) = acc;
  }
}
__global__ void __launch_bounds__(256) gather_mean_scalar_kernel(const float* __restrict__ x, int64_t ldx, int cin,
                                                                 int64_t nseg, const int32_t* __restrict__ seg_ptr,
                                                                 const int32_t* __restrict__ col,
                                                                 float* __restrict__ out) {
  const int64_t total = nseg * cin;
  for (int64_t t = (int64_t)blockIdx.x * blockDim.x + threadIdx.x; t < total; t += (int64_t)gridDim.x * blockDim.x) {
    const int64_t s = t / cin;
    const int c = (int)(t - s * cin);
    const int32_t a = seg_ptr[s], e = seg_ptr[s + 1];
    float acc = 0.f;
    for (int32_t p = a; p < e; ++p) acc += x[(int64_t)col[p] * ldx + c];
    if (e - a > 1) acc /= (float)(e - a);
    out[t] = acc;
  }
}

extern "C" int ofx_gather_mean(const float* x, int64_t ldx, int cin, int64_t n_nodes, const int32_t* seg_ptr,
                               const int32_t* col, float* col_data, void* stream) {
  if (!x || !seg_ptr || !col || !col_data || cin < 1 || ldx < cin || n_nodes < 0) return OFX_EINVAL;
  const int64_t nseg = n_nodes * 7;
  hipStream_t st = ofx_stream(stream);
  const bool vec = (cin % 4 == 0) && ((ldx & 3) == 0) && (((uintptr_t)x & 15) == 0) && (((uintptr_t)col_data & 15) == 0);
  if (vec)
    gather_mean_kernel<<<ofx_grid(nseg * (cin / 4), 256), 256, 0, st>>>(x, ldx, cin, nseg, seg_ptr, col, col_data);
  else
    gather_mean_scalar_kernel<<<ofx_grid(nseg * cin, 256), 256, 0, st>>>(x, ldx, cin, nseg, seg_ptr, col, col_data);
  OFX_LAUNCH_CHECK();
  return OFX_OK;
}
```

### octfusion_amd/csrc/ofx_gemm_common.h

```cpp
#pragma once
#include "ofx_common.h"

typedef float f32x16 __attribute__((ext_vector_type(16)));

struct GemmArgs {
  const float* A; int64_t lda; const int32_t* a_rows;
  const float* x; int64_t ldx; int cin; int ndir; int fast;
  const int32_t* nbr;
  const int32_t* seg_ptr; const int32_t* col;
  const float* edge_w;
  const float* tf; int64_t ldt; int64_t Kf;
  const int32_t* nbr_ext;
  const float* aux; int64_t ldaux; int64_t n_src;
  int64_t M, K;
  const float* Wp; int64_t Kp, N;
  const uint16_t* W16;
  const float* oscale_p;
  const float* bias;
  const float* emb; int64_t lde; const int32_t* bid;
  const float* res; int64_t ldr;
  float* out; int64_t ldc; const int32_t* out_rows;
  int gather_out_rows;
  int out_planes;
  double* stats; int64_t stats_ld;
  int ntm, ntn, nsplit, kt_per_split;
  float* ws;
  int vec4;
  float* stats_part; size_t stats_part_bytes;
};

static __global__ void __launch_bounds__(256) weight_absmax_kernel(const float* __restrict__ W, int64_t sk, int64_t sn, int64_t K,
                                                            int64_t N, unsigned* __restrict__ acc) {
  __shared__ float red[256];
  float m = 0.f;
  for (int64_t t = (int64_t)blockIdx.x * 256 + threadIdx.x; t < K * N; t += (int64_t)gridDim.x * 256) {
    const float a = fabsf(W[(t / N) * sk + (t % N) * sn]);
    if (a <= 3.0e38f) m = fmaxf(m, a);
  }
  red[threadIdx.x] = m;
  __syncthreads();
  for (int o = 128; o > 0; o >>= 1) {
    if ((int)threadIdx.x < o) red[threadIdx.x] = fmaxf(red[threadIdx.x], red[threadIdx.x + o]);
    __syncthreads();
  }
  if (threadIdx.x == 0) atomicMax(acc, __float_as_uint(red[0]));
}
static __global__ void weight_scale_finish_kernel(int fp16_operands, float* __restrict__ scale) {
  const float mx = __uint_as_float(reinterpret_cast<const unsigned*>(scale)[0]);
  float s = 1.f;
  if (fp16_operands && mx > 0.f) {
    int e;
    frexpf(mx, &e);
    int sh = 15 - e;
    sh = sh < -60 ? -60 : (sh > 60 ? 60 : sh);
    s = ldexpf(1.f, sh);
  }
  scale[0] = 1.f / s;
  scale[1] = s;
}
static inline int ofx_launch_weight_scale(const float* W, int64_t sk, int64_t sn, int64_t K, int64_t N, int fp16_operands,
                                          float* scale, hipStream_t st) {
  if (hipMemsetAsync(scale, 0, sizeof(float), st) != hipSuccess) return OFX_ELAUNCH;
  int64_t nb = (K * N + 256 * 16 - 1) / (256 * 16);
  nb = nb < 1 ? 1 : (nb > 1024 ? 1024 : nb);
  weight_absmax_kernel<<<(unsigned)nb, 256, 0, st>>>(W, sk, sn, K, N, reinterpret_cast<unsigned*>(scale));
  if (hipGetLastError() != hipSuccess) return OFX_ELAUNCH;
  weight_scale_finish_kernel<<<1, 1, 0, st>>>(fp16_operands, scale);
  if (hipGetLastError() != hipSuccess) return OFX_ELAUNCH;
  return OFX_OK;
}


__device__ __forceinline__ unsigned g2_pk_bf16(float a, float b) {
  unsigned r;
  asm("v_cvt_pk_bf16_f32 %0, %1, %2" : "=v"(r) : "v"(a), "v"(b));
  return r;
}
__device__ __forceinline__ unsigned g2_pk_f16(float a, float b) {
  const _Float16 x = (_Float16)a, y = (_Float16)b;
  return (unsigned)__builtin_bit_cast(unsigned short, x) | ((unsigned)__builtin_bit_cast(unsigned short, y) << 16);
}
__device__ __forceinline__ float g2_bf16_lo(unsigned p) { return __uint_as_float(p << 16); }
__device__ __forceinline__ float g2_bf16_hi(unsigned p) { return __uint_as_float(p & 0xffff0000u); }
__device__ __forceinline__ float g2_f16_lo(unsigned p) { return (float)__builtin_bit_cast(_Float16, (unsigned short)(p & 0xffffu)); }
__device__ __forceinline__ float g2_f16_hi(unsigned p) { return (float)__builtin_bit_cast(_Float16, (unsigned short)(p >> 16)); }
__device__ __forceinline__ float g2_sat16(float v) { return fminf(fmaxf(v, -65504.f), 65504.f); }
__device__ __forceinline__ void g2_split2(int mode, float a, float b, unsigned& hi, unsigned& lo) {
  if (mode == 3) {
    hi = g2_pk_f16(a, b);
    lo = g2_pk_f16(a - g2_f16_lo(hi), b - g2_f16_hi(hi));
  } else {
    hi = g2_pk_bf16(a, b);
    lo = g2_pk_bf16(a - g2_bf16_lo(hi), b - g2_bf16_hi(hi));
  }
}
__device__ __forceinline__ void g2_join2(int mode, unsigned hi, unsigned lo, float& a, float& b) {
  if (mode == 3) { a = g2_f16_lo(hi) + g2_f16_lo(lo); b = g2_f16_hi(hi) + g2_f16_hi(lo); }
  else { a = g2_bf16_lo(hi) + g2_bf16_lo(lo); b = g2_bf16_hi(hi) + g2_bf16_hi(lo); }
}
__host__ __device__ static inline bool g2_pairs(int mode) { return mode == 2 || mode == 3; }

__device__ __forceinline__ void ofx_store_planes4(float* base, int64_t f, const float4& v, int mode) {
  unsigned h0, h1, l0, l1;
  g2_split2(mode, v.x, v.y, h0, l0);
  g2_split2(mode, v.z, v.w, h1, l1);
  char* o = reinterpret_cast<char*>(base) + (f >> 5) * 128 + (f & 31) * 2;
  *reinterpret_cast<uint2*>(o) = make_uint2(h0, h1);
  *reinterpret_cast<uint2*>(o + 64) = make_uint2(l0, l1);
}

__device__ __forceinline__ float4 f4zero() { return make_float4(0.f, 0.f, 0.f, 0.f); }
__device__ __forceinline__ void f4add(float4& a, const float4& b) { a.x += b.x; a.y += b.y; a.z += b.z; a.w += b.w; }

template <int WM, int WN, int MI, int NI>
__device__ __forceinline__ void epilogue_store_scalar(const GemmArgs& g, f32x16 (&acc)[MI][NI], int64_t m0, int64_t n0,
                                                      int wm, int wn, int l31, int h, int split) {
#pragma unroll
  for (int j = 0; j < NI; ++j) {
    const int64_t n = n0 + (wn * NI + j) * 32 + l31;
    if (n >= g.N) continue;
    if (g.nsplit > 1) {
#pragma unroll
      for (int i = 0; i < MI; ++i)
#pragma unroll
        for (int r = 0; r < 16; ++r) {
          const int64_t m = m0 + (wm * MI + i) * 32 + (r & 3) + 8 * (r >> 2) + 4 * h;
          if (m < g.M) g.ws[((int64_t)split * g.M + m) * g.N + n] = acc[i][j][r];
        }
      continue;
    }
    const float bv = g.bias ? g.bias[n] : 0.f;
    const float osc = g.oscale_p ? *g.oscale_p : 1.f;
    int sb = -1;
    float ssum = 0.f, ssq = 0.f;
#pragma unroll
    for (int i = 0; i < MI; ++i) {
#pragma unroll
      for (int r = 0; r < 16; ++r) {
        const int64_t m = m0 + (wm * MI + i) * 32 + (r & 3) + 8 * (r >> 2) + 4 * h;
        if (m >= g.M) continue;
        float v = fmaf(acc[i][j][r], osc, bv);
        int b = 0;
        if (g.emb || g.stats) b = g.bid[m];
        if (g.emb) v += g.emb[(int64_t)b * g.lde + n];
        if (g.res) v += g.res[m * g.ldr + n];
        if (g.stats) {
          if (b != sb) {
            if (sb >= 0) {
              double* o = g.stats + ((int64_t)sb * g.stats_ld + n) * 2;
              unsafeAtomicAdd(o, (double)ssum);
              unsafeAtomicAdd(o + 1, (double)ssq);
            }
            sb = b; ssum = 0.f; ssq = 0.f;
          }
          ssum += v; ssq += v * v;
        }
        int64_t om = m;
        if (g.out_rows) { om = g.out_rows[m]; if (om < 0) continue; }
        g.out[om * g.ldc + n] = v;
      }
    }
    if (g.stats && sb >= 0) {
      double* o = g.stats + ((int64_t)sb * g.stats_ld + n) * 2;
      unsafeAtomicAdd(o, (double)ssum);
      unsafeAtomicAdd(o + 1, (double)ssq);
    }
  }
}

__device__ __forceinline__ float dpp_xor1(float v) {
  return __builtin_bit_cast(float, __builtin_amdgcn_mov_dpp(__builtin_bit_cast(int, v), 0xB1, 0xf, 0xf, true));
}
__device__ __forceinline__ float dpp_xor2(float v) {
  return __builtin_bit_cast(float, __builtin_amdgcn_mov_dpp(__builtin_bit_cast(int, v), 0x4E, 0xf, 0xf, true));
}
__device__ __forceinline__ void quad_transpose(float& v0, float& v1, float& v2, float& v3, bool q0, bool q1) {
  float r = dpp_xor1(q0 ? v0 : v1);
  if (q0) v0 = r; else v1 = r;
  r = dpp_xor1(q0 ? v2 : v3);
  if (q0) v2 = r; else v3 = r;
  r = dpp_xor2(q1 ? v0 : v2);
  if (q1) v0 = r; else v2 = r;
  r = dpp_xor2(q1 ? v1 : v3);
// ... 108 lines not shown
```

### octfusion_amd/csrc/ofx_norm.hip

```cpp
#include "ofx_planes.h"

constexpr int GN_ROWS_PER_BLOCK = 64;

static inline int64_t gn_stats_rows(int64_t n, int batch_size, int C = 128) {
  const int64_t chunks = (n + GN_ROWS_PER_BLOCK - 1) / GN_ROWS_PER_BLOCK;
  const int64_t bytes_per_batch = n * (int64_t)C * 4 / (batch_size > 0 ? batch_size : 1);
  int64_t per_batch = bytes_per_batch / (512 << 10);
  per_batch = per_batch < 8 ? 8 : (per_batch > 128 ? 128 : per_batch);
  int64_t cap = per_batch * (int64_t)batch_size;
  if (cap < 64) cap = 64;
  return chunks <= cap ? GN_ROWS_PER_BLOCK : GN_ROWS_PER_BLOCK * ((chunks + cap - 1) / cap);
}

__global__ void __launch_bounds__(256) gn_stats_kernel(const float* __restrict__ x, int64_t ldx, int64_t n, int C,
                                                       const int32_t* __restrict__ bid, double* __restrict__ sums,
                                                       int64_t rpb) {
  __shared__ int sb[256];
  __shared__ float sv[256][8];
  const int CT = C >> 2;
  const int RP = 256 / CT;
  const int cl = threadIdx.x % CT, rl = threadIdx.x / CT;
  int cb = -1;
  float s[4] = {0, 0, 0, 0}, q[4] = {0, 0, 0, 0};
  auto flush_direct = [&](int b, const float* ps, const float* pq) {
// ... 859 lines not shown
  const int work = batch_size * groups > C ? batch_size * groups : C;
  gn_bwd_finalize_kernel<<<(work + 63) / 64, 64, 0, st>>>(sums, count, batch_size, C, groups, count_eps, mean, rstd, w,
                                                          coef, dgamma, dbeta);
  if (n > 0)
    gn_bwd_apply_kernel<<<ofx_grid(n * (C >> 2), 256), 256, 0, st>>>(x, ldx, dy, ldy, n, C, batch_id, mean, rstd, w,
                                                                     bias, act, coef, dx, lddx);
  OFX_LAUNCH_CHECK();
  return OFX_OK;
}

__global__ void __launch_bounds__(256) gn_fused_rows_kernel(const float* __restrict__ x, int64_t ldx, int rows, int C,
                                                            int G, float eps, float count_eps,
                                                            const float* __restrict__ w, const float* __restrict__ bias,
                                                            int act, float* __restrict__ out, int64_t ldo) {
  __shared__ double red[2][256];
  __shared__ float stat[2];
  const int cpg = C / G;
  const int b = blockIdx.x / G, g = blockIdx.x - b * G;
  const float* xb = x + (int64_t)b * rows * ldx + g * cpg;
  float* ob = out + (int64_t)b * rows * ldo + g * cpg;
  const int total = rows * cpg;
  float s = 0.f, q = 0.f;
  for (int t = threadIdx.x; t < total; t += 256) {
    const int r = t / cpg, c = t - r * cpg;
    const float v = xb[(int64_t)r * ldx + c];
    s += v; q += v * v;
  }
  red[0][threadIdx.x] = (double)s;
  red[1][threadIdx.x] = (double)q;
  __syncthreads();
  for (int o = 128; o > 0; o >>= 1) {
    if (threadIdx.x < o) { red[0][threadIdx.x] += red[0][threadIdx.x + o]; red[1][threadIdx.x] += red[1][threadIdx.x + o]; }
    __syncthreads();
  }
  if (threadIdx.x == 0) {
    const double S = red[0][0], SS = red[1][0];
    const float cnt = (float)rows * (float)cpg;
    const float inv = 1.0f / (cnt + count_eps);
    const double m = S * (double)inv;
    const double ssd = SS - 2.0 * m * S + (double)cnt * m * m;
    const double var = (ssd > 0 ? ssd : 0) * (double)inv;
    stat[0] = (float)m;
    stat[1] = (float)(1.0 / sqrt(var + (double)eps));
  }
  __syncthreads();
  const float m = stat[0], rs = stat[1];
  for (int t = threadIdx.x; t < total; t += 256) {
    const int r = t / cpg, c = t - r * cpg;
    const float v = xb[(int64_t)r * ldx + c];
    ob[(int64_t)r * ldo + c] = ofx_apply_act((v - m) * rs * w[g * cpg + c] + bias[g * cpg + c], act);
  }
}

static int g_gn_rows16 = 1;
extern "C" int ofx_set_gn_rows16(int on) { g_gn_rows16 = on ? 1 : 0; return OFX_OK; }

__global__ void __launch_bounds__(1024) gn_fused_rows16_kernel(const float* __restrict__ x, int64_t ldx, int rows, int C,
                                                               int G, float eps, float count_eps,
                                                               const float* __restrict__ w,
                                                               const float* __restrict__ bias, int act,
                                                               float* __restrict__ out, int64_t ldo) {
  __shared__ float part[16][4][4];
  __shared__ float stat[16][2];
  const int cpg = C / G;
  const int gpb = 16 / cpg;
  const int bpb = G / gpb;
  const int b = blockIdx.x / bpb, cb = (blockIdx.x - b * bpb) * 16;
  const int p = threadIdx.x & 3, rl = threadIdx.x >> 2;
  const float* xb = x + (int64_t)b * rows * ldx + cb + p * 4;
  float* ob = out + (int64_t)b * rows * ldo + cb + p * 4;
  const int ga = (4 * p) / cpg, gb = (4 * p + 3) / cpg;
  const bool two = ga != gb;
  float sa = 0.f, qa = 0.f, sb = 0.f, qb = 0.f;
  auto acc4 = [&](const float4& v) {
    if (two) {
      sa += v.x + v.y; qa += v.x * v.x + v.y * v.y;
      sb += v.z + v.w; qb += v.z * v.z + v.w * v.w;
    } else {
      sa += (v.x + v.y) + (v.z + v.w); qa += (v.x * v.x + v.y * v.y) + (v.z * v.z + v.w * v.w);
    }
  };
  int r = rl;
  for (; r + 768 < rows; r += 1024) {
    const float4 v0 = *reinterpret_cast<const float4*>(xb + (int64_t)r * ldx);
    const float4 v1 = *reinterpret_cast<const float4*>(xb + (int64_t)(r + 256) * ldx);
    const float4 v2 = *reinterpret_cast<const float4*>(xb + (int64_t)(r + 512) * ldx);
    const float4 v3 = *reinterpret_cast<const float4*>(xb + (int64_t)(r + 768) * ldx);
    acc4(v0); acc4(v1); acc4(v2); acc4(v3);
  }
  for (; r < rows; r += 256) acc4(*reinterpret_cast<const float4*>(xb + (int64_t)r * ldx));
#pragma unroll
  for (int o = 4; o < 64; o <<= 1) {
    sa += __shfl_xor(sa, o); qa += __shfl_xor(qa, o); sb += __shfl_xor(sb, o); qb += __shfl_xor(qb, o);
  }
  const int wv = threadIdx.x >> 6;
  if ((threadIdx.x & 63) < 4) {
    part[wv][p][0] = sa; part[wv][p][1] = qa; part[wv][p][2] = sb; part[wv][p][3] = qb;
  }
  __syncthreads();
  if (threadIdx.x < gpb) {
    const int j = threadIdx.x;
    double S = 0.0, SS = 0.0;
    for (int sl = 0; sl < 4; ++sl) {
      const int a0 = (4 * sl) / cpg, b0 = (4 * sl + 3) / cpg;
      for (int wq = 0; wq < 16; ++wq) {
        if (a0 == j) { S += (double)part[wq][sl][0]; SS += (double)part[wq][sl][1]; }
        if (b0 == j && b0 != a0) { S += (double)part[wq][sl][2]; SS += (double)part[wq][sl][3]; }
      }
    }
    const float cnt = (float)rows * (float)cpg;
    const float inv = 1.0f / (cnt + count_eps);
    const double m = S * (double)inv;
    const double ssd = SS - 2.0 * m * S + (double)cnt * m * m;
    const double var = (ssd > 0 ? ssd : 0) * (double)inv;
    stat[j][0] = (float)m;
    stat[j][1] = (float)(1.0 / sqrt(var + (double)eps));
  }
  __syncthreads();
  const float ma = stat[ga][0], ra = stat[ga][1], mb = stat[gb][0], rb = stat[gb][1];
  const float4 ww = *reinterpret_cast<const float4*>(w + cb + p * 4);
  const float4 bb = *reinterpret_cast<const float4*>(bias + cb + p * 4);
  auto apply = [&](int rr) {
    const float4 v = *reinterpret_cast<const float4*>(xb + (int64_t)rr * ldx);
    float4 y;
    y.x = ofx_apply_act((v.x - ma) * ra * ww.x + bb.x, act);
    y.y = ofx_apply_act((v.y - ma) * ra * ww.y + bb.y, act);
    y.z = ofx_apply_act((v.z - mb) * rb * ww.z + bb.z, act);
    y.w = ofx_apply_act((v.w - mb) * rb * ww.w + bb.w, act);
    *reinterpret_cast<float4*>(ob + (int64_t)rr * ldo) = y;
  };
  for (r = rl; r + 768 < rows; r += 1024) { apply(r); apply(r + 256); apply(r + 512); apply(r + 768); }
  for (; r < rows; r += 256) apply(r);
}

extern "C" int ofx_gn_fused_rows(const float* x, int64_t ldx, int rows_per_batch, int batch_size, int C, int groups,
                                 float eps, float count_eps, const float* w, const float* bias, int act, float* out,
                                 int64_t ldo, void* stream) {
  if (!x || !w || !bias || !out || rows_per_batch < 1 || batch_size < 1 || C < 1 || groups < 1 || C % groups ||
      ldx < C || ldo < C || act < 0 || act > OFX_ACT_GELU)
    return OFX_EINVAL;
  const int cpg = C / groups;
  const bool al16 = ((((uintptr_t)x | (uintptr_t)out | (uintptr_t)w | (uintptr_t)bias) & 15) == 0) && (ldx % 4 == 0) &&
                    (ldo % 4 == 0);
  if (g_gn_rows16 && al16 && (cpg == 2 || cpg == 4 || cpg == 8 || cpg == 16) && groups % (16 / cpg) == 0 &&
      rows_per_batch >= 2048)
    gn_fused_rows16_kernel<<<batch_size * (groups / (16 / cpg)), 1024, 0, ofx_stream(stream)>>>(
        x, ldx, rows_per_batch, C, groups, eps, count_eps, w, bias, act, out, ldo);
  else
    gn_fused_rows_kernel<<<batch_size * groups, 256, 0, ofx_stream(stream)>>>(x, ldx, rows_per_batch, C, groups, eps,
                                                                              count_eps, w, bias, act, out, ldo);
  OFX_LAUNCH_CHECK();
  return OFX_OK;
}
```

### octfusion_amd/graph_unet_lr.py

```python
import math

import torch
import torch.nn as nn

from . import ops
from .modules import _Linear


class _GridCache:

    _cache = {}

    @classmethod
    def get(cls, batch_size, device):
        key = (batch_size, device.type, device.index)
        c = cls._cache.get(key)
        if c is None:
            c = cls(batch_size, device)
            cls._cache[key] = c
        return c

    def __init__(self, batch_size, device):
        self.B = batch_size
        self.device = device
        self._tab = {}
        self._bid = {}
        self._cnt = {}

    def table(self, mode, depth_out, fast):
        k = (mode, depth_out, fast)
        if k not in self._tab:
            d_in = depth_out + (0, 1, -1)[mode]
            pad = self.B * 8 ** d_in if fast else -1
            self._tab[k] = ops.grid_conv_table(mode, depth_out, self.B, self.device, pad)
        return self._tab[k]

    def rev(self, mode, depth_out):
        k = ('rev', mode, depth_out)
        if k not in self._tab:
            from ._lib import call, ptr, stream, lib
            d_in = depth_out + (0, 1, -1)[mode]
            n_in, n_out = self.B * 8 ** d_in, self.B * 8 ** depth_out
            tab = self.table(mode, depth_out, False)
            dev = self.device
            nseg = n_in * 27
            cnt = torch.empty(nseg, dtype=torch.int32, device=dev)
            call('ofx_table_reverse_count', ptr(tab), n_out, 27, n_in, ptr(cnt), stream())
            rev_ptr = torch.empty(nseg + 1, dtype=torch.int32, device=dev)
            ws = torch.empty(lib().ofx_scan_ws_bytes(nseg), dtype=torch.uint8, device=dev)
            call('ofx_scan_i32', ptr(cnt), ptr(rev_ptr), nseg, ptr(ws), stream())
            E = int(rev_ptr[-1].item())
            rev_row = torch.empty(max(E, 1), dtype=torch.int32, device=dev)
            rev_w = torch.empty(max(E, 1), dtype=torch.float32, device=dev)
            call('ofx_table_reverse_fill', ptr(tab), n_out, 27, n_in, ptr(rev_ptr), ptr(cnt), ptr(rev_row), ptr(rev_w),
                 stream())
            nbr = torch.empty(nseg, dtype=torch.int32, device=dev)
            call('ofx_seg_primary_w', ptr(rev_ptr), ptr(rev_row), ptr(rev_w), nseg, ptr(nbr), stream())
            call('ofx_seg_multi_flag_w', ptr(rev_ptr), ptr(rev_w), nseg, ptr(cnt), stream())
            rank = torch.empty(nseg + 1, dtype=torch.int32, device=dev)
            call('ofx_scan_i32', ptr(cnt), ptr(rank), nseg, ptr(ws), stream())
            V = int(rank[-1].item())
            nbr_ext = torch.empty(nseg, dtype=torch.int32, device=dev)
            multi_seg = torch.empty(max(V, 1), dtype=torch.int32, device=dev)
            call('ofx_seg_primary_ext_w', ptr(rev_ptr), ptr(rev_row), ptr(rev_w), nseg, n_out, ptr(rank), ptr(nbr_ext),
                 ptr(multi_seg), stream())
            self._tab[k] = dict(rev_ptr=rev_ptr, rev_row=rev_row, rev_w=rev_w, nbr=nbr, nbr_ext=nbr_ext,
                                multi_seg=multi_seg, V=V, n_in=n_in, n_out=n_out)
        return self._tab[k]

    def batch_id(self, depth):
        if depth not in self._bid:
            per = 8 ** depth
            self._bid[depth] = (torch.arange(self.B * per, device=self.device) // per).to(torch.int32)
            self._cnt[depth] = torch.full((self.B,), float(per), dtype=torch.float32, device=self.device)
        return self._bid[depth]

    def count(self, depth):
        self.batch_id(depth)
        return self._cnt[depth]


class GridState:

    def __init__(self, batch_size, depth, device):
        self.B, self.depth = batch_size, depth
        self.cache = _GridCache.get(batch_size, device)

    def at(self, depth):
        g = GridState.__new__(GridState)
        g.B, g.depth, g.cache = self.B, depth, self.cache
        return g


def _dense_io(x):
    assert x.dim() == 5 and x.shape[2] == x.shape[3] == x.shape[4], 'dense blocks take cubic [b, c, S, S, S] grids'
    S = x.shape[2]
    depth = S.bit_length() - 1
    assert 1 << depth == S, 'grid edge must be a power of two'
    B = x.shape[0]
    rows = ops.voxel2octree_cf(x.float().contiguous(), depth)
    return rows, GridState(B, depth, x.device), (lambda r, d: ops.octree2voxel_cf(r, B, d))


class GroupNorm32(nn.GroupNorm):

    @torch.no_grad()
    def forward(self, x, gs, act=None, out=None):
        return ops.group_norm(x, gs.cache.batch_id(gs.depth), gs.cache.count(gs.depth), gs.B, self.weight,
                              self.bias, self.num_groups, self.eps, act, out, count_eps=0.0,
                              rows_per_batch=8 ** gs.depth)


def convnormalization(channels):
    return GroupNorm32(min(channels, 32), channels)


class our_Identity(nn.Module):
    def forward(self, x, *args, **kwargs):
        return x


class GridConv3d(nn.Module):

    def __init__(self, cin, cout, mode=0):
        super().__init__()
        self.in_channels, self.out_channels, self.mode = cin, cout, mode
        self.weight = nn.Parameter(torch.empty(cout, cin, 3, 3, 3))
        self.bias = nn.Parameter(torch.empty(cout))
        nn.init.kaiming_uniform_(self.weight, a=math.sqrt(5))
        bound = 1 / math.sqrt(cin * 27)
        nn.init.uniform_(self.bias, -bound, bound)
        self._pw = ops.PackedConv3d()

    def out_depth(self, depth):
        return depth + (0, -1, 1)[self.mode]

    @torch.no_grad()
    def forward(self, x, gs, emb=None, res=None, out=None):
        d_out = self.out_depth(gs.depth)
        n_out = gs.B * 8 ** d_out
        bid = gs.cache.batch_id(d_out) if emb is not None else None
        mode = self.mode
        return ops.gridconv(x, lambda fast: gs.cache.table(mode, d_out, fast), n_out, self._pw.get(self.weight),
                            self.bias, emb, bid, res, out)


class _PointConv(nn.Module):

    def __init__(self, cin, cout, kdims):
        super().__init__()
        self.weight = nn.Parameter(torch.empty(cout, cin, *([1] * kdims)))
        self.bias = nn.Parameter(torch.empty(cout))
        nn.init.kaiming_uniform_(self.weight, a=math.sqrt(5))
        nn.init.uniform_(self.bias, -1 / math.sqrt(cin), 1 / math.sqrt(cin))
        self._pw = ops.PackedWeight()

    @torch.no_grad()
    def forward(self, x, res=None, out=None):
        w = self.weight.view(self.weight.shape[0], self.weight.shape[1])
        return ops.gemm(x, self._pw.get(w, 'nk'), self.bias, res, out)


class ConvUpsample(nn.Module):

    def __init__(self, channels, use_conv=True, dims=3):
        super().__init__()
        self.channels = channels
        self.conv = GridConv3d(channels, channels, mode=2)

    def forward(self, x, gs=None, out=None):
        if gs is None:
            rows, gs, back = _dense_io(x)
            return back(self.conv(rows, gs), gs.depth + 1)
        return self.conv(x, gs, out=out), gs.at(gs.depth + 1)


class ConvDownsample(nn.Module):

    def __init__(self, channels, use_conv=True, dims=3):
        super().__init__()
        self.channels = channels
        self.op = GridConv3d(channels, channels, mode=1)

    def forward(self, x, gs=None):
        if gs is None:
            rows, gs, back = _dense_io(x)
            return back(self.op(rows, gs), gs.depth - 1)
        return self.op(x, gs), gs.at(gs.depth - 1)


class ResnetBlock(nn.Module):

    def __init__(self, world_dims, dim_in, dim_out, emb_dim, dropout=0.1, use_text_condition=False):
        super().__init__()
        assert world_dims == 3 and not use_text_condition
        self.time_mlp = nn.Sequential(nn.SiLU(), _Linear(emb_dim, dim_out))
        self.block1 = nn.Sequential(convnormalization(dim_in), nn.SiLU(), GridConv3d(dim_in, dim_out))
        conv2 = GridConv3d(dim_out, dim_out)
        for p in conv2.parameters():
            p.detach().zero_()
        self.block2 = nn.Sequential(convnormalization(dim_out), nn.SiLU(), nn.Dropout(dropout), conv2)
        self.res_conv = _PointConv(dim_in, dim_out, 3) if dim_in != dim_out else nn.Identity()

    @torch.no_grad()
    def forward(self, x, emb_act, gs=None, out=None, t=None):
        if gs is None:
            rows, gs, back = _dense_io(x)
            return back(self.forward(rows, ops.act(emb_act.float().contiguous(), 'silu'), gs), gs.depth)
        skip, main, fork = x, None, None
        if not isinstance(self.res_conv, nn.Identity):
            main, fork = ops.fork_stream(x.device, level=2)
            if fork is not None:
                with torch.cuda.stream(fork):
                    skip = self.res_conv(x)
            else:
                skip = self.res_conv(x)
        h = self.block1[0](x, gs, act='silu')
        if t is None:
            t = self.time_mlp[1](emb_act)
        h = self.block1[2](h, gs, emb=t)
        h = self.block2[0](h, gs, act='silu', out=h)
        if fork is not None:
            main.wait_stream(fork)
        return self.block2[3](h, gs, res=skip, out=out)


class QKVAttention(nn.Module):
    """reference modules.py:538-547 -- computed by ofx_attention."""


class AttentionBlock(nn.Module):

    def __init__(self, channels, num_heads=1):
        super().__init__()
        self.channels = channels
        self.num_heads = num_heads
        self.norm = convnormalization(channels)
        self.qkv = _PointConv(channels, channels * 3, 1)
        self.attention = QKVAttention()
        self.proj_out = _PointConv(channels, channels, 1)
        for p in self.proj_out.parameters():
            p.detach().zero_()

    @torch.no_grad()
    def forward(self, x, gs=None, out=None):
        if gs is None:
            rows, gs, back = _dense_io(x)
            return back(self.forward(rows, gs), gs.depth)
        qkv = self.qkv(self.norm(x, gs))
        h = ops.attention(qkv, gs.B, 8 ** gs.depth, self.num_heads)
        return self.proj_out(h, res=x, out=out)


class _AttnSeq(nn.Sequential):

    def forward(self, x, gs, out=None):
        return self[2](self[0](x, gs, act='silu'), gs, out=out)


class LearnedSinusoidalPosEmb(nn.Module):

    def __init__(self, dim):
        super().__init__()
        assert dim % 2 == 0
        self.weights = nn.Parameter(torch.randn(dim // 2))

    def forward(self, x):
        x = x[:, None]
        freqs = x * self.weights[None, :] * 2 * math.pi
        return torch.cat((x, freqs.sin(), freqs.cos()), dim=-1)


class UNet3DModel(nn.Module):
    def __init__(self, full_depth, in_split_channels, model_channels, out_split_channels,
                 attention_resolutions, dropout=0, channel_mult=(1, 2, 4, 8), dims=2, num_classes=None,
                 use_checkpoint=False, num_heads=-1, use_text_condition=False, context_dim=None,
                 n_embed=None, **kwargs):
        super().__init__()
        assert dims == 3
        self.full_depth = full_depth
        self.in_channels = in_split_channels
        self.model_channels = model_channels
        self.out_channels = out_split_channels
        self.attention_resolutions = attention_resolutions
        self.channel_mult = list(channel_mult)
        self.num_classes = num_classes
        self.num_heads = num_heads
        mc = model_channels
        chans = [mc] + [mc * m for m in self.channel_mult]
        in_out = list(zip(chans[:-1], chans[1:]))
        ted = mc * 4
        self.time_pos_emb = LearnedSinusoidalPosEmb(mc)
        self.time_emb = nn.Sequential(_Linear(mc + 1, ted), nn.SiLU(), _Linear(ted, ted))
        if num_classes is not None:
            self.label_emb = nn.Embedding(num_classes, ted)
        self.input_emb = GridConv3d(2 * self.in_channels, mc)

        def attn(c, ds):
            if ds in attention_resolutions:
                return _AttnSeq(convnormalization(c), nn.SiLU(), AttentionBlock(c, num_heads=num_heads))
            return our_Identity()

        self.downs = nn.ModuleList()
        self.ups = nn.ModuleList()
        nres = len(in_out)
        ds = 1
        for ind, (ci, co) in enumerate(in_out):
            last = ind >= nres - 1
            self.downs.append(nn.ModuleList([
                ResnetBlock(dims, ci, co, emb_dim=ted, dropout=dropout), attn(co, ds),
                ConvDownsample(co, dims=dims) if not last else our_Identity()]))
            if not last:
                ds *= 2
        mid = chans[-1]
        self.mid_block1 = ResnetBlock(dims, mid, mid, emb_dim=ted, dropout=dropout)
        self.mid_self_attn = attn(mid, ds)
        self.mid_block2 = ResnetBlock(dims, mid, mid, emb_dim=ted, dropout=dropout)
        for ci, co in reversed(in_out[1:]):
            self.ups.append(nn.ModuleList([
                ResnetBlock(dims, co * 2, ci, emb_dim=ted, dropout=dropout), attn(ci, ds),
                ConvUpsample(ci, dims=dims)]))
            ds //= 2
        self.end = nn.Sequential(convnormalization(mc), nn.SiLU())
        self.out = GridConv3d(mc, self.out_channels)

    @torch.no_grad()
    def _embed(self, timesteps, label, batch_size):
        pe = ops.learned_sinusoid(timesteps.float(), self.time_pos_emb.weights)
        lab = None
        if self.num_classes is not None:
            assert label.shape == (batch_size,)
            lab = self.label_emb(label)
        return self.time_emb[2](self.time_emb[0](pe, act_out='silu'), res=lab, act_out='silu')

    def _all_time_mlps(self, emb_act):
        blocks = [m for m in self.modules() if isinstance(m, ResnetBlock)]
        lins = [b.time_mlp[1] for b in blocks]
        key = tuple((l.weight.data_ptr(), l.weight._version, l.bias.data_ptr(), l.bias._version) for l in lins)
        if getattr(self, '_tm_key', None) != key:
            self._tm_w = torch.cat([l.weight.detach() for l in lins], dim=0).contiguous()
            self._tm_b = torch.cat([l.bias.detach() for l in lins], dim=0).contiguous()
            self._tm_pw = ops.PackedWeight()
            self._tm_key = key
        if ops.LINEAR_SMALL and emb_act.shape[0] <= 16:
            allout = ops.linear_small(emb_act, self._tm_w, self._tm_b)
        else:
            allout = ops.gemm(emb_act, self._tm_pw.get(self._tm_w, 'nk'), self._tm_b)
        outs, off = {}, 0
        for b, l in zip(blocks, lins):
            outs[id(b)] = allout[:, off:off + l.out_features]
            off += l.out_features
        return outs

    @torch.no_grad()
    def forward_rows(self, x, batch_size, timesteps, label=None, as_middle=False, out=None):
        with ops.policy_scope('dense_net'), ops.stats_scope(x.device):
            return self._forward_rows(x, batch_size, timesteps, label, as_middle, out)

    @torch.no_grad()
    def precompute_embeddings(self, timesteps, label, batch_size):
        main, fork = ops.fork_stream(timesteps.device)
        if fork is None:
            return
        with torch.cuda.stream(fork):
            emb_act = self._embed(timesteps, label, batch_size)
            tms = self._all_time_mlps(emb_act)
        self._pre = (timesteps, label, batch_size, emb_act, tms, main, fork)

    def _forward_rows(self, x, batch_size, timesteps, label, as_middle, out=None):
        gs = GridState(batch_size, self.full_depth, x.device)
        if not as_middle:
            x = self.input_emb(x, gs)
        pre, self._pre = getattr(self, '_pre', None), None
        if pre is not None and pre[0] is timesteps and pre[1] is label and pre[2] == batch_size:
            emb_act, tms = pre[3], pre[4]
            pre[5].wait_stream(pre[6])
        else:
            if pre is not None:
                pre[5].wait_stream(pre[6])
            emb_act = self._embed(timesteps, label, batch_size)
            tms = self._all_time_mlps(emb_act)

        nlev = len(self.downs)
        mc = self.model_channels
        cout = [mc * m_ for m_ in self.channel_mult]
        bufs = {}
        for i in range(1, nlev):
            d_i = self.full_depth - min(i, nlev - 1)
            bufs[i] = torch.empty(batch_size * 8 ** d_i, 2 * cout[i], dtype=torch.float32, device=x.device)

        def run_attn(m, x, gs, out=None):
            return x if isinstance(m, our_Identity) else m(x, gs, out=out)

        for i, (resnet, self_attn, downsample) in enumerate(self.downs):
            slot = bufs[i][:, cout[i]:] if i in bufs else None
            if isinstance(self_attn, our_Identity):
                x = resnet(x, emb_act, gs, out=slot, t=tms[id(resnet)])
            else:
                x = run_attn(self_attn, resnet(x, emb_act, gs, t=tms[id(resnet)]), gs, out=slot)
            if not isinstance(downsample, our_Identity):
                x, gs = downsample(x, gs)
        x = self.mid_block1(x, emb_act, gs, t=tms[id(self.mid_block1)])
        x = run_attn(self.mid_self_attn, x, gs)
        x = self.mid_block2(x, emb_act, gs, out=bufs[nlev - 1][:, :cout[nlev - 1]] if nlev > 1 else None,
                            t=tms[id(self.mid_block2)])
        for j, (resnet, self_attn, upsample) in enumerate(self.ups):
            i = nlev - 1 - j
            x = bufs[i]
            x = run_attn(self_attn, resnet(x, emb_act, gs, t=tms[id(resnet)]), gs)
            nxt = bufs[i - 1][:, :cout[i - 1]] if i - 1 in bufs else None
            x, gs = upsample(x, gs, out=nxt)
        x = self.end[0](x, gs, act='silu', out=out if as_middle else None)
        return x if as_middle else self.out(x, gs)

    @torch.no_grad()
    def forward_as_middle(self, h, doctree, timesteps, label, context, out=None):
        return self.forward_rows(h, doctree.batch_size, timesteps, label, as_middle=True, out=out)

    @torch.no_grad()
    def forward(self, x=None, timesteps=None, x_self_cond=None, label=None, context=None, as_middle=False,
                **kwargs):
        assert (label is not None) == (self.num_classes is not None), \
            'must specify label if and only if the model is class-conditional'
        B = x.shape[0]
        if not as_middle:
            C = x.shape[1]
            rows = torch.empty(B * 8 ** self.full_depth, 2 * C, dtype=torch.float32, device=x.device)
            ops.voxel2octree_cf(x.float(), self.full_depth, out=rows[:, :C])
            if x_self_cond is None:
                rows[:, C:].zero_()
            else:
                ops.voxel2octree_cf(x_self_cond.float(), self.full_depth, out=rows[:, C:])
        else:
            rows = ops.voxel2octree_cf(x.float(), self.full_depth)
        y = self.forward_rows(rows, B, timesteps, label, as_middle)
        return ops.octree2voxel_cf(y, B, self.full_depth)
```

### octfusion_amd/ops.py

```python
import contextlib
import os
from typing import NamedTuple

import torch

from . import _lib
from ._lib import call, call_may_decline, ptr, stream

ACT = {None: 0, 'none': 0, 'silu': 1, 'gelu': 2}

GRAPHCONV_PROFILE = None
_NO_BRACKET = contextlib.nullcontext()


@contextlib.contextmanager
def _timed_layer(prof, *rec):
    e0 = torch.cuda.Event(enable_timing=True)
    e1 = torch.cuda.Event(enable_timing=True)
    e0.record()
    yield
    e1.record()
    prof.append((e0, e1) + rec)


# ... 237 lines not shown
             n_multi, ptr(aux), aux.numel() * aux.element_size(), ptr(tf_planes), ldt, nt, ptr(pw.t), pw.N, ptr(bias),
             ptr(emb), lde, ptr(batch_id) if (emb is not None or stats is not None) else None, ptr(res), ldr, ptr(out),
             ldc, ptr(stats), pw.N, ptr(ws), ws.numel(), ptr(sync), sync.numel() * 4, mode, aux_ready, stream())
    return out


SIDE_STREAM = os.environ.get('OFX_SIDE_STREAM', '0') == '1'


def set_lane_cus(cus):
    call('ofx_set_gconv_cus', int(cus))


def side_stream(device):
    return _scratch('side', device, False, lambda: torch.cuda.Stream(device))


FORK = int(os.environ.get('OFX_FORK', '0'))


def fork_stream(device, level=1):
    if FORK < level or device.type != 'cuda':
        return None, None
    s = _scratch('fork', device, False, lambda: torch.cuda.Stream(device))
    main = torch.cuda.current_stream(device)
    if main.cuda_stream == s.cuda_stream:
        return None, None
    s.wait_stream(main)
    return main, s


SYNC_WORDS = 4096


def sync_words(device):
    def make():
        _no_capture('the flag words')
        return torch.zeros(SYNC_WORDS, dtype=torch.int32, device=device)
    return _scratch('sync', device, True, make)


def sync_error(device):
    return any(int(t.abs().sum().item()) != 0 for t in _scratch_all('sync', device))


def raise_on_sync_error(device):
    if not sync_error(device):
        return
    for t in _scratch_all('sync', device):
        t.zero_()
    call('ofx_set_gconv_persistent', 0)
    raise _lib.OfxError('a flag wait of the persistent GraphConv launch gave up on %s: the results of this call are '
                        'invalid; the process now uses the one-tile-per-block launch (ofx_set_gconv_persistent(0))' % device)


AUTO_RANGE_FALLBACK = True


class OfxRangeError(_lib.OfxError):
    """An operand left the range the fp16-pair contraction covers (include/ofx.h, fp16x3 range guard)."""


def range_words(device):
    def make():
        with torch.cuda.device(_dev_key(device)[1]):
            t = torch.zeros(4, dtype=torch.int32, device=device)
            call('ofx_set_range_words', ptr(t))
        return t
    return _scratch('range', device, False, make)


def reset_range_words(device):
    t = _SCRATCH.get(_scratch_key('range', device))
    if t is not None:
        t.zero_()


def range_error(device, result=None):
    t = _SCRATCH.get(_scratch_key('range', device))
    n = int(t[0].item()) if t is not None else 0
    bad = result is not None and not bool(torch.isfinite(result).all())
    return {'operands_beyond_fp16': n, 'result_non_finite': bad} if (n or bad) else None


def raise_on_range_error(device, result=None):
    err = range_error(device, result)
    if err is None:
        return
    range_words(device).zero_()
    was = get_precision()
    if was not in ('fp16x3', 'fp16'):
        raise _lib.OfxError('non-finite result on %s in precision %s (%s)' % (device, was, err))
    if AUTO_RANGE_FALLBACK and was == 'fp16x3':
        set_precision('bf16x3')
    raise OfxRangeError('fp16x3 range guard on %s: %s -- operands beyond +-65504 do not fit the fp16 operand pairs; the '
                        'results of this call are invalid%s' % (device, err, '; the process now computes in bf16x3: call again'
                                                               if AUTO_RANGE_FALLBACK and was == 'fp16x3' else ''))


def workspace(device, nbytes=96 << 20):
    def make():
        _no_capture('the split-K / hand-off workspace')
        return torch.empty(nbytes, dtype=torch.uint8, device=device)
    t = _scratch('ws', device, True, make)
    if t.numel() < nbytes:
        t = _SCRATCH[_scratch_key('ws', device, True)] = make()
    return t


def scan_i32(x):
    _chk(x, torch.int32)
    n = x.numel()
    out = torch.empty(n + 1, dtype=torch.int32, device=x.device)
    ws = torch.empty(_lib.lib().ofx_scan_ws_bytes(n), dtype=torch.uint8, device=x.device)
    call('ofx_scan_i32', ptr(x), ptr(out), n, ptr(ws), stream())
    return out


class PackedWeight:

    def __init__(self):
        self.t = None
        self.key = None
        self.K = self.N = self.Kp = 0

    def get(self, w, mode, cin=0, nt=0):
        key = (w.data_ptr(), w._version, tuple(w.shape), mode, cin, nt, _lib.lib().ofx_get_precision() == 3)
        if key == self.key:
            return self
        _chk(w)
        w = w.detach()
        if not w.is_contiguous():
            w = w.contiguous()
        L = _lib.lib()
        if mode == 'kn' or mode == 'graphconv':
            K, N = w.shape
            sk, sn = N, 1
        elif mode == 'nk':
            N, K = w.shape
            sk, sn = 1, K
        else:
            raise ValueError(mode)
        if mode == 'graphconv':
            Kp = L.ofx_graphconv_packed_k(cin, nt)
        else:
            cin = nt = 0
            Kp = L.ofx_packed_k(K)
        out = torch.empty(L.ofx_packed_floats(Kp, N), dtype=torch.float32, device=w.device)
        call('ofx_pack_weights', ptr(w), sk, sn, K, N, cin, nt, ptr(out), Kp, stream())
        self.t, self.key, self.K, self.N, self.Kp = out, key, K, N, Kp
        return self


def gemm(a, pw, bias=None, res=None, out=None, a_rows=None, out_rows=None, m=None, out_planes=0):
    a, lda = _row_major(a)
    M = m if m is not None else (a_rows.numel() if a_rows is not None else a.shape[0])
    if a.shape[1] != pw.K:
        raise ValueError('K mismatch: %d vs %d' % (a.shape[1], pw.K))
    out, ldc = _out2d(out, M, pw.N, a.device)
    res, ldr = _row_major(res)
    _chk(bias)
    _chk(a_rows, torch.int32)
    _chk(out_rows, torch.int32)
    ws = workspace(a.device)
    _meta('dense_gemm', 2.0 * M * pw.K * pw.N, 4.0 * (M * pw.K + pw.K * pw.N + M * pw.N * (2 if res is not None else 1)),
          (M, pw.K, pw.N))
    if out_planes:
        args = ('ofx_gemm_f32_planes', ptr(a), lda, ptr(a_rows), M, pw.K, ptr(pw.t), pw.Kp, pw.N, ptr(bias),
                ptr(res), ldr, ptr(out), ldc, ptr(out_rows), ptr(ws), ws.numel(), out_planes, stream())
    else:
        args = ('ofx_gemm_f32', ptr(a), lda, ptr(a_rows), M, pw.K, ptr(pw.t), pw.Kp, pw.N, ptr(bias),
                ptr(res), ldr, ptr(out), ldc, ptr(out_rows), ptr(ws), ws.numel(), stream())
    if pw.N <= 64 or pw.K <= 64:
        with policy_scope('small_gemm'):
            call(*args)
    else:
        call(*args)
    return out


def gather_gemm(x, tab, ntap, pw, n_out, bias=None, res=None, out=None, out_rows=None, out_planes=0):
    x, ldx = _row_major(x)
    cin = x.shape[1]
    assert pw.K == ntap * cin and cin % 32 == 0
    _chk(tab, torch.int32)
    out, ldc = _out2d(out, n_out, pw.N, x.device)
    res, ldr = _row_major(res)
    _chk(bias)
    _chk(out_rows, torch.int32)
    ws = workspace(x.device)
    _meta('dense_gemm', 2.0 * n_out * pw.K * pw.N, 4.0 * (n_out * pw.K + pw.K * pw.N + n_out * pw.N), (n_out, pw.K, pw.N))
    call('ofx_gather_gemm_f32', ptr(x), ldx, cin, ntap, x.shape[0], n_out, ptr(tab), ptr(zero_row(x.device)), ptr(pw.t), pw.Kp,
         pw.N, ptr(bias), ptr(res), ldr, ptr(out), ldc, ptr(out_rows), ptr(ws), ws.numel(), out_planes, stream())
    return out


GEMM_PLANES = os.environ.get('OFX_GEMM_PLANES', '0') == '1'


class PackedGemmPlanes:

    def __init__(self):
        self.t = None
        self.key = None

    def get(self, w2d, mode):
        key = (w2d.data_ptr(), w2d._version, tuple(w2d.shape), tuple(w2d.stride()), mode)
        if key != self.key:
            _chk(w2d)
            K, N = w2d.shape
            nb = _lib.lib().ofx_gemm_planes_packed_bytes(K, N, mode)
            assert nb > 0
            t = torch.empty(nb, dtype=torch.uint8, device=w2d.device)
            assert t.data_ptr() % 128 == 0
            call('ofx_pack_gemm_planes', ptr(w2d.detach()), w2d.stride(0), w2d.stride(1), K, N, mode, ptr(t), stream())
            self.t, self.key, self.K, self.N = t, key, K, N
        return self


def gemm_planes(a_planes, pgp, out, out_planes=0, bias=None):
    mode = planes_of(a_planes)
    M, K = a_planes.shape
    assert planes_pairs(mode) and K == pgp.K and a_planes.stride(1) == 1
    dev = a_planes.device
    out, ldc = _out2d(out, M, pgp.N, dev)
    tabs = _scratch('row_tab', dev, False, dict)
    tab = tabs.get(M)
    if tab is None:
        if len(tabs) > 64:
            tabs.clear()
        _no_capture('the row table of a dense planes GEMM')
        tab = torch.zeros(M * 7 + 4, dtype=torch.int32, device=dev)
        tab[:M * 7].view(M, 7)[:, 0] = torch.arange(M, dtype=torch.int32, device=dev)
        tabs[M] = tab
    ws = workspace(dev)
    sync = sync_words(dev)
    _meta('dense_gemm', 2.0 * M * K * pgp.N, 4.0 * (M * K + K * pgp.N + M * pgp.N), (M, K, pgp.N, 'planes'))
    return call_may_decline('ofx_gemm_planes', ptr(a_planes), a_planes.stride(0) * 4, M, M, K, ptr(tab), ptr(pgp.t), pgp.N,
                            ptr(bias), ptr(out), ldc, out_planes, ptr(ws), ws.numel(), ptr(sync), sync.numel() * 4, mode,
                            stream())


LINEAR_SMALL = True


def linear_small(a, weight, bias=None, res=None, act_in=None, act_out=None, out=None):
    a, lda = _row_major(a)
    w, ldw = _row_major(weight.detach())
    M, K = a.shape
    N = w.shape[0]
    assert w.shape[1] == K and M <= 16
    out, ldo = _out2d(out, M, N, a.device)
    res, ldr = _row_major(res)
    _chk(bias)
    _meta('small_linear', 2.0 * M * K * N, 4.0 * (N * K + M * K + M * N), (M, K, N))
    call('ofx_linear_small', ptr(a), lda, M, K, ptr(w), ldw, N, ptr(bias.detach() if bias is not None else None), ptr(res),
         ldr, ACT[act_in], ACT[act_out], ptr(out), ldo, stream())
    return out


def learned_sinusoid(t, w):
    _chk(t), _chk(w)
    t, w = t.contiguous(), w.detach().contiguous()
    out = torch.empty(t.shape[0], 2 * w.shape[0] + 1, dtype=torch.float32, device=t.device)
    _meta('elementwise', 0, 4.0 * out.numel(), (out.numel(),))
    call('ofx_learned_sinusoid', ptr(t), ptr(w), t.shape[0], w.shape[0], ptr(out), stream())
    return out


def zero_row(device, n=4096):
    return _scratch('zeros', device, False, lambda: torch.zeros(n, dtype=torch.float32, device=device))


def graphconv(x, nbr, seg_ptr, col, pw, cin, type_frac=None, bias=None, emb=None, batch_id=None,
              res=None, out=None, ext=None, stats=None):
    x, ldx = _row_major(x)
    N = x.shape[0]
    if x.shape[1] != cin:
        raise ValueError('cin mismatch')
    out, ldc = _out2d(out, N, pw.N, x.device)
    ldt = nt_pad = 0
    if type_frac is not None:
        _chk(type_frac)
        ldt = type_frac.stride(0)
        nt_pad = type_frac.shape[1]
    emb, lde = _row_major(emb)
    if emb is not None or stats is not None:
        _chk(batch_id, torch.int32)
    res, ldr = _row_major(res)
    _chk(bias)
    _chk(stats, torch.float64)
    E = col.numel()
    flops = 2.0 * N * pw.K * pw.N
    nbytes = 4.0 * (E * cin + N * pw.N + pw.K * pw.N) + 8.0 * E
    with _layer_bracket(flops, nbytes, pw.N, ('graph', N, cin, pw.N)):
        ws = workspace(x.device)
        nbr_ext = multi_seg = aux = None
        n_multi = 0
        if ext is not None and cin % 32 == 0:
            nbr_ext, multi_seg, n_multi = ext
            aux = torch.empty((n_multi + 1) * ldx, dtype=torch.float32, device=x.device)
        args = ('ofx_graphconv_fwd', ptr(x), ldx, cin, N, ptr(nbr), ptr(seg_ptr), ptr(col), ptr(nbr_ext), ptr(multi_seg),
                n_multi, ptr(aux), ptr(type_frac), ldt, nt_pad,
                ptr(pw.t), pw.Kp, pw.N, ptr(bias), ptr(emb), lde,
                ptr(batch_id) if (emb is not None or stats is not None) else None,
                ptr(res), ldr, ptr(out), ldc, ptr(stats), pw.N, ptr(ws), ws.numel(), stream())
        _meta('graphconv', flops, 0, (N, cin, pw.N, 'reg'))
        if pw.N <= 64 or cin <= 64:
            with policy_scope('small_gemm'):
                call(*args)
        else:
            call(*args)
    return out


NARROW_IN = os.environ.get('OFX_NARROW_IN', '1') == '1'
NARROW_OUT = os.environ.get('OFX_NARROW_OUT', '1') == '1'


def narrow_in_ok(cin, cout, nt):
    return NARROW_IN and cin <= 8 and cout in (64, 128) and 7 * (cin + nt) <= 96


NARROW_IN_TAB = os.environ.get('OFX_NARROW_IN_TAB', '1') == '1'
NARROW_IN_TAB_MIN_ROWS = int(os.environ.get('OFX_NARROW_IN_TAB_MIN_ROWS', str(1 << 19)))


def graphconv_narrow_in(x, seg_ptr, col, weights, cin, nt, node_type=None, bias=None, batch_id=None, out=None, stats=None,
                        ext=None):
    x, ldx = _row_major(x)
    w = weights.detach()
# ... 49 lines not shown
            self.w = wd
            self.key = key
        return self

    def type_term(self, type_frac, nt, N, C, bias):
        cout = self.w.shape[1]
        tt = torch.empty(N, cout, dtype=torch.float32, device=self.w.device)
        _chk(bias)
        call('ofx_narrow_out_type_term', ptr(type_frac) if nt else None, type_frac.stride(0) if nt else 0, nt, N, ptr(self.w),
             C, cout, ptr(bias), ptr(tt), stream())
        return tt


def graphconv_narrow_out(x, seg_ptr, col, pno, C, type_term=None, out=None):
    N = x.shape[0]
    cout = pno.w.shape[1]
    E = col.numel()
    flops = 2.0 * N * pno.w.shape[0] * cout
    pwid = pno.width
    agg_bytes = 4.0 * (N * pwid + E + 7 * N + 2 * N * cout)
    nbytes = agg_bytes + 4.0 * (N * C + N * pwid + pno.w.numel())
    with _layer_bracket(flops, nbytes, cout, ('graph', N, C, cout)):
        P = gemm(x, pno.pw.get(pno.wd, 'kn'))
        out, ldc = _out2d(out, N, cout, x.device)
        _chk(type_term)
        assert type_term is None or (type_term.is_contiguous() and tuple(type_term.shape) == (N, cout))
        _meta('graphconv_narrow', flops, agg_bytes, (N, C, cout, 'narrow_out'))
        call('ofx_graphconv_narrow_out', ptr(P), P.stride(0), cout, N, ptr(seg_ptr), ptr(col), ptr(type_term), ptr(out),
             ldc, stream())
    return out


def gemm_tn(p, q):
    _chk(p), _chk(q)
    assert p.shape[0] == q.shape[0]
    K0, N0 = p.shape[1], q.shape[1]

    def pad4(t):
        c = t.shape[1]
        if c % 4 == 0 and t.stride(0) % 4 == 0 and t.stride(1) == 1 and t.data_ptr() % 16 == 0:
            return t
        out = torch.zeros(t.shape[0], (c + 3) // 4 * 4, dtype=torch.float32, device=t.device)
        out[:, :c] = t
        return out
    p, q = pad4(p), pad4(q)
    if (K0, N0) != (p.shape[1], q.shape[1]):
        return gemm_tn(p, q)[:K0, :N0].contiguous()
    p, ldp = _row_major(p)
    q, ldq = _row_major(q)
    K, N = p.shape[1], q.shape[1]
    out = torch.empty(K, N, dtype=torch.float32, device=p.device)
    ws = workspace(p.device)
    call('ofx_gemm_tn_f32', ptr(p), ldp, ptr(q), ldq, p.shape[0], K, N, ptr(out), ptr(ws), ws.numel(), stream())
    return out


GRAD_TOP_EXP = 8


def grad_pow2(dy):
    lo, hi = torch.aminmax(dy) if dy.numel() else (dy.new_zeros(()), dy.new_zeros(()))
    _, e = torch.frexp(torch.maximum(-lo, hi))
    s = (GRAD_TOP_EXP - e).clamp(-100, 100)
    return torch.ldexp(dy, s), torch.ldexp(torch.ones_like(hi), -s)


def gemm_grad(dy, pw):
    dys, inv = grad_pow2(dy)
    return gemm(dys, pw).mul_(inv)


def linear_backward(x, dy, weight, need_dx=True):
    dW = gemm_tn(dy, x)
    dx = gemm_grad(dy, PackedWeight().get(weight, 'kn')) if need_dx else None
    return dx, dW, dy.sum(0)


def graphconv_backward(x, dy, doctree, d, weights, n_node_type, need_dx=True, need_dw=True):
    x, ldx = _row_major(x)
    dy, ldy = _row_major(dy)
    _chk(x), _chk(dy), _chk(weights)
    N, cin = x.shape
    cout = dy.shape[1]
    nt = n_node_type if n_node_type > 1 else 0
    assert weights.shape == (7 * (cin + nt), cout)
    seg_ptr, col, Ng, E = doctree.csr(d)
    assert N == Ng and dy.shape[0] == N
    ws = workspace(x.device)
    dx = dW = None
    if need_dx:
        rv = doctree.rev(d)
        wt = weights.detach().view(7, cin + nt, cout)[:, :cin, :].permute(0, 2, 1).reshape(7 * cout, cin).contiguous()
        pwt = PackedWeight().get(wt, 'graphconv', cout, 0)
        dx = torch.empty(N, cin, dtype=torch.float32, device=x.device)
        dys, inv = grad_pow2(dy)
        lds = dys.stride(0)
        fast = cout % 32 == 0 and lds % 4 == 0
        aux = torch.empty((rv['V'] + 1) * lds, dtype=torch.float32, device=x.device) if fast else None
        call('ofx_graphconv_bwd_data', ptr(dys), lds, cout, N, ptr(rv['nbr']), ptr(rv['rev_ptr']), ptr(rv['rev_row']),
             ptr(rv['rev_w']), ptr(rv['nbr_ext']) if fast else None, ptr(rv['multi_seg']) if fast else None,
             rv['V'] if fast else 0, ptr(aux), ptr(pwt.t), pwt.Kp, cin, ptr(dx), cin, ptr(ws), ws.numel(), stream())
        dx.mul_(inv)
    if need_dw:
        L = _lib.lib()
        Kp = L.ofx_graphconv_packed_k(cin, nt)
        Kf = Kp - (((7 * nt + 31) // 32) * 32 if nt else 0)
        tf = doctree.type_frac(d, nt) if nt else None
        fast = cin % 32 == 0 and ldx % 4 == 0
        nbr_ext, multi_seg, V = doctree.ext(d)
        aux = torch.empty((V + 1) * ldx, dtype=torch.float32, device=x.device) if fast else None
        dyw, ldw, cw = dy, ldy, cout
        if cout % 4 or ldy % 4 or dy.data_ptr() % 16:
            cw = (cout + 3) // 4 * 4
            dyw = torch.zeros(N, cw, dtype=torch.float32, device=x.device)
            dyw[:, :cout] = dy
            ldw = cw
        dwp = torch.empty(Kp, cw, dtype=torch.float32, device=x.device)
        call('ofx_graphconv_bwd_weight', ptr(x), ldx, cin, N, ptr(doctree.nbr(d)), ptr(seg_ptr), ptr(col),
             ptr(nbr_ext) if fast else None, ptr(multi_seg) if fast else None, V if fast else 0, ptr(aux),
             ptr(tf), tf.stride(0) if tf is not None else 0, tf.shape[1] if tf is not None else 0,
             ptr(dyw), ldw, cw, ptr(dwp), Kp, ptr(ws), ws.numel(), stream())
        dwp = dwp[:, :cout]
        dev = x.device
        dirs = torch.arange(7, device=dev).view(7, 1)
        idx = [dirs * cin + torch.arange(cin, device=dev).view(1, cin)]
        if nt:
            idx.append(Kf + dirs * nt + torch.arange(nt, device=dev).view(1, nt))
        dW = dwp.index_select(0, torch.cat(idx, 1).reshape(-1))
    return dx, dW


class PackedConv3d:

    def __init__(self):
        self.t = None
        self.key = None
        self.cin = self.N = 0

    def get(self, w):
        key = (w.data_ptr(), w._version, tuple(w.shape), _lib.lib().ofx_get_precision() == 3)
        if key == self.key:
            return self
        _chk(w)
        cout, cin = w.shape[:2]
        assert tuple(w.shape[2:]) == (3, 3, 3)
        w = w.detach().contiguous()
        Kp = _lib.lib().ofx_conv3d_packed_k(cin)
        out = torch.empty(_lib.lib().ofx_packed_floats(Kp, cout), dtype=torch.float32, device=w.device)
        call('ofx_pack_conv3d', ptr(w), cin, cout, ptr(out), stream())
        self.t, self.key, self.cin, self.N = out, key, cin, cout
        return self


def gridconv(x, tables, n_out, pw, bias=None, emb=None, batch_id=None, res=None, out=None):
    x, ldx = _row_major(x)
    if x.shape[1] != pw.cin:
        raise ValueError('cin mismatch')
    out, ldc = _out2d(out, n_out, pw.N, x.device)
    emb, lde = _row_major(emb)
    if emb is not None:
        _chk(batch_id, torch.int32)
    res, ldr = _row_major(res)
    _chk(bias)
    ws = workspace(x.device)
    fast = pw.cin % 32 == 0 and ldx % 4 == 0
    flops = 2.0 * n_out * 27 * pw.cin * pw.N
    nbytes = 4.0 * (27.0 * n_out * pw.cin + n_out * pw.N + 27.0 * pw.cin * pw.N) + 4.0 * 27 * n_out
    with _layer_bracket(flops, nbytes, pw.N, ('grid', n_out, pw.cin, pw.N)):
        _meta('gridconv_27tap', flops,
              4.0 * (x.shape[0] * pw.cin + n_out * pw.N * (2 if res is not None else 1) + 27.0 * pw.cin * pw.N) + 4.0 * 27 * n_out,
              (n_out, pw.cin, pw.N))
        call('ofx_gridconv_fwd', ptr(x), ldx, pw.cin, x.shape[0], n_out, None if fast else ptr(tables(False)),
             ptr(tables(True)) if fast else None, ptr(zero_row(x.device)), ptr(pw.t), pw.N, ptr(bias), ptr(emb), lde,
             ptr(batch_id) if emb is not None else None, ptr(res), ldr, ptr(out), ldc, ptr(ws), ws.numel(), stream())
    return out


def grid_conv_table(mode, depth_out, batch_size, device, pad=-1):
    n = (8 ** depth_out) * batch_size
    t = torch.empty(n, 27, dtype=torch.int32, device=device)
    call('ofx_grid_conv_table', mode, depth_out, batch_size, pad, ptr(t), stream())
    return t


def attention(qkv, batch_size, T, heads, out=None):
    qkv, ldq = _row_major(qkv)
    C = qkv.shape[1] // 3
    ch = C // heads
    out, ldo = _out2d(out, qkv.shape[0], C, qkv.device)
    _meta('attention', 4.0 * batch_size * heads * T * T * ch, 4.0 * qkv.shape[0] * 4 * C, (batch_size, T, heads, ch))
    call('ofx_attention', ptr(qkv), ldq, batch_size, T, heads, ch, ptr(out), ldo, stream())
    return out


def attention_backward(qkv, dout, batch_size, T, heads):
    qkv, ldq = _row_major(qkv)
    dout, ldo = _row_major(dout)
    _chk(qkv), _chk(dout)
    C = qkv.shape[1] // 3
    ch = C // heads
    dqkv = torch.empty(qkv.shape[0], 3 * C, dtype=torch.float32, device=qkv.device)
    rowstat = torch.empty(batch_size * heads * T * 3, dtype=torch.float32, device=qkv.device)
    call('ofx_attention_bwd', ptr(qkv), ldq, ptr(dout), ldo, batch_size, T, heads, ch, ptr(rowstat), ptr(dqkv), 3 * C,
         stream())
    return dqkv


def gather_mean(x, seg_ptr, col):
    x, ldx = _row_major(x)
    N, C = x.shape
    out = torch.empty(N, 7, C, dtype=torch.float32, device=x.device)
    call('ofx_gather_mean', ptr(x), ldx, C, N, ptr(seg_ptr), ptr(col), ptr(out), stream())
    return out


AUX_ATTR = '_ofx_aux'
GN_FINALIZE_LAUNCH = False
GN_ROWS_TWO_KERNELS = int(os.environ.get('OFX_GN_ROWS_TWO_KERNELS', '2048'))
GN_FUSE_AUX_FINALIZE = os.environ.get('OFX_GN_FUSE_AUX_FINALIZE', '0') == '1'
GN_OCT_FINALIZE = os.environ.get('OFX_GN_OCT_FINALIZE', '1') == '1'
GN_OCT_FINALIZE_MAX_ELEMS = int(os.environ.get('OFX_GN_OCT_FINALIZE_MAX_ELEMS', str(9 << 20)))
AUX_PLAN = {'1': 'oct', '0': ''}.get(os.environ.get('OFX_AUX_PLAN', 'oct'), os.environ.get('OFX_AUX_PLAN', 'oct'))


class AuxGraph(NamedTuple):
    seg_ptr: torch.Tensor
    col: torch.Tensor
    multi_seg: torch.Tensor
    n_multi: int
    oct_plan: tuple = None
    block_plan: tuple = None


def _gn_launch(planes, aux_graph, elems):
    g = aux_graph if planes else None
    oct_plan, block_plan = (g.oct_plan, g.block_plan) if g is not None and AUX_PLAN else (None, None)
    oct_fin = GN_OCT_FINALIZE and AUX_PLAN == 'oct' and oct_plan is not None and elems <= GN_OCT_FINALIZE_MAX_ELEMS
    finalize = GN_FINALIZE_LAUNCH or (g is not None and not GN_FUSE_AUX_FINALIZE and not oct_fin)
    if not planes:
        return 'fp32', finalize
    if oct_plan is not None:
        return ('oct' if finalize or oct_fin else 'plain'), finalize
    return ('block' if block_plan is not None else 'plain'), finalize


def group_norm(x, batch_id, count, batch_size, weight, bias, groups, eps=1e-5, act=None, out=None,
               count_eps=None, stats=None, rows_per_batch=None, planes=0, aux_graph=None):
    if count_eps is None:
        count_eps = eps
    x, ldx = _row_major(x)
    n, C = x.shape
    dev = x.device
    range_words(dev)
    if (rows_per_batch is not None and stats is None and not planes and rows_per_batch * (C // groups) <= (1 << 16)
            and rows_per_batch < GN_ROWS_TWO_KERNELS):
        assert n == rows_per_batch * batch_size
        out, ldo = _out2d(out, n, C, dev)
        _meta('gn_fused_rows', 0, 8.0 * n * C, (n, C))
        call('ofx_gn_fused_rows', ptr(x), ldx, rows_per_batch, batch_size, C, groups, eps, count_eps,
             ptr(weight.detach().reshape(-1)), ptr(bias.detach().reshape(-1)), ACT[act], ptr(out), ldo, stream())
        return out
    if stats is not None:
        _chk(stats, torch.float64)
        assert stats.numel() == batch_size * C * 2
        sums = stats
    else:
        _meta('gn_stats', 0, 4.0 * n * C, (n, C))
        if stats_pool_has_room(batch_size * C * 2, dev):
            sums = stats_zeros(batch_size * C * 2, dev)
            call('ofx_gn_stats_acc', ptr(x), ldx, n, C, ptr(batch_id), batch_size, ptr(sums), stream())
        else:
            sums = torch.empty(batch_size * C * 2, dtype=torch.float64, device=dev)
            call('ofx_gn_stats', ptr(x), ldx, n, C, ptr(batch_id), batch_size, ptr(sums), stream())
    w = weight.detach().reshape(-1)
    b = bias.detach().reshape(-1)
    mean = rstd = None
    launch, finalize = _gn_launch(planes, aux_graph, n * C)
    if finalize:
        mean = torch.empty(batch_size * C, dtype=torch.float32, device=dev)
        rstd = torch.empty(batch_size * C, dtype=torch.float32, device=dev)
        _meta('gn_finalize', 0, 24.0 * batch_size * C, (batch_size, C))
        call('ofx_gn_finalize', ptr(sums), ptr(count), batch_size, C, groups, eps, count_eps, ptr(mean), ptr(rstd),
             stream())
    if planes:
        if aux_graph is not None and out is not None and out.data_ptr() == x.data_ptr():
            out = None
        out, ldo = _planes_out(n, C, planes, dev, out if planes_pairs(planes) else None)
        aux = seg_ptr = col = multi_seg = None
        n_multi = 0
        if aux_graph is not None:
            seg_ptr, col, multi_seg, n_multi = aux_graph[:4]
            aux = torch.empty((n_multi + 1) * ldo, dtype=torch.uint8, device=dev)
            setattr(out, AUX_ATTR, aux)
        setattr(out, PLANES_ATTR, planes)
        _meta('gn_apply', 0, 8.0 * n * C + (n_multi + 1) * float(ldo), (n, C, 'planes+aux' if aux is not None else 'planes'))
        if launch == 'oct':
            op, shift, n_own, n_left, (o_ptr, o_ent, o_head, o_src) = aux_graph.oct_plan
            base = op.data_ptr()
            call('ofx_gn_apply_planes_oct', ptr(x), ldx, n, C, ptr(batch_id), ptr(mean), ptr(rstd), ptr(sums), ptr(count),
                 groups, eps, count_eps, ptr(w), ptr(b), ACT[act], planes, ptr(out), ldo, n_multi, ptr(aux), base + 4 * o_ptr,
                 base + 4 * o_ent, n_own, shift, base + 4 * o_head, base + 4 * o_src, n_left, stream())
        else:
            plan, n_left = aux_graph.block_plan if launch == 'block' else (None, 0)
            call('ofx_gn_apply_planes', ptr(x), ldx, n, C, ptr(batch_id), ptr(mean), ptr(rstd), ptr(sums), ptr(count), groups,
                 eps, count_eps, ptr(w), ptr(b), ACT[act], planes, ptr(out), ldo, ptr(seg_ptr), ptr(col), ptr(multi_seg),
                 n_multi, ptr(aux), ptr(plan), n_left, stream())
        return out
    out, ldo = _out2d(out, n, C, dev)
    _meta('gn_apply', 0, 8.0 * n * C, (n, C, 'fp32'))
    call('ofx_gn_apply', ptr(x), ldx, n, C, ptr(batch_id), ptr(mean), ptr(rstd), ptr(sums), ptr(count), groups, eps, count_eps,
         ptr(w), ptr(b), ACT[act], ptr(out), ldo, stream())
    return out


def group_norm_backward(x, dy, batch_id, count, batch_size, weight, bias, groups, eps=1e-5, act=None, count_eps=None):
    if count_eps is None:
        count_eps = eps
    x, ldx = _row_major(x)
    dy, ldy = _row_major(dy)
    _chk(x), _chk(dy)
    n, C = x.shape
    dev = x.device
    mean = torch.empty(batch_size * C, dtype=torch.float32, device=dev)
    rstd = torch.empty(batch_size * C, dtype=torch.float32, device=dev)
    sums = torch.empty(batch_size * C * 2, dtype=torch.float64, device=dev)
    call('ofx_gn_stats', ptr(x), ldx, n, C, ptr(batch_id), batch_size, ptr(sums), stream())
    call('ofx_gn_finalize', ptr(sums), ptr(count), batch_size, C, groups, eps, count_eps, ptr(mean), ptr(rstd),
# ... 144 lines not shown
```

Baseline: 120.5.

## Fuse next layer's GroupNorm+activation into GEMM and gridconv split-K reduce

Adds GEMM and gridconv entry points that carry a GroupNorm tail. When split-K is used and the channels-per-group and row count fit, the split-K reduction kernel also computes group statistics in shared memory and writes the normalized, activated output. Otherwise it falls back to a separate fused-rows GN launch. The model code threads a 'next norm' through resnet, attention and downsample blocks so the following layer's GN is produced by the preceding GEMM, and the raw output store can be skipped. This saves a full read pass and kernel launches per norm, at the cost of more code paths and of a reduce kernel that runs one block per batch×16 channels.

```diff
diff --git a/include/ofx.h b/include/ofx.h
--- a/include/ofx.h
+++ b/include/ofx.h
@@ -164,6 +164,12 @@
                         const float* res, int64_t ldr, float* out, int64_t ldc,
                         const int32_t* out_rows, void* ws, size_t ws_bytes, int out_mode, void* stream);
 
+int ofx_gemm_f32_gn(const float* A, int64_t lda, const int32_t* a_rows, int64_t M, int64_t K, const float* Wp, int64_t Kp,
+                    int64_t N, const float* bias, const float* res, int64_t ldr, float* out, int64_t ldc, void* ws,
+                    size_t ws_bytes, const float* gn_w, const float* gn_b, int groups, float eps, float count_eps, int act,
+                    int rows_per_batch, int batch_size, float* gn_out, int64_t ldo, void* stream);
+int ofx_gemm_gn_plan(int64_t M, int64_t N, int64_t Kp, size_t ws_bytes, int groups, int rows_per_batch);
+
 int ofx_graphconv_fwd(const float* x, int64_t ldx, int cin, int64_t n_nodes,
                       const int32_t* nbr, const int32_t* seg_ptr, const int32_t* col,
                       const int32_t* nbr_ext, const int32_t* multi_seg, int64_t n_multi, float* aux,
@@ -239,6 +245,12 @@
                      const float* Wp, int cout, const float* bias, const float* emb, int64_t lde,
                      const int32_t* batch_id, const float* res, int64_t ldr, float* out,
                      int64_t ldc, void* ws, size_t ws_bytes, void* stream);
+int ofx_gridconv_fwd_gn(const float* x, int64_t ldx, int cin, int64_t n_in, int64_t n_out, const int32_t* nbr27,
+                        const int32_t* nbr27_ext, const float* zero_row, const float* Wp, int cout, const float* bias,
+                        const float* emb, int64_t lde, const int32_t* batch_id, const float* res, int64_t ldr, float* out,
+                        int64_t ldc, void* ws, size_t ws_bytes, const float* gn_w, const float* gn_b, int groups,
+                        float eps, float count_eps, int act, int rows_per_batch, int batch_size, float* gn_out,
+                        int64_t ldo, void* stream);
 int ofx_gather_gemm_f32(const float* x, int64_t ldx, int cin, int ntap, int64_t n_src, int64_t n_out, const int32_t* tab,
                         const float* zero_row, const float* Wp, int64_t Kp, int cout, const float* bias,
                         const float* res, int64_t ldr, float* out, int64_t ldc, const int32_t* out_rows, void* ws,
diff --git a/octfusion_amd/_lib.py b/octfusion_amd/_lib.py
--- a/octfusion_amd/_lib.py
+++ b/octfusion_amd/_lib.py
@@ -100,6 +100,9 @@
     'ofx_pack_weights': (c_i, [c_p, c_l, c_l, c_l, c_l, c_i, c_i, c_p, c_l, c_p], True),
     'ofx_gemm_f32': (c_i, [c_p, c_l, c_p, c_l, c_l, c_p, c_l, c_l, c_p, c_p, c_l, c_p, c_l, c_p, c_p, c_sz, c_p], True),
     'ofx_gemm_f32_planes': (c_i, [c_p, c_l, c_p, c_l, c_l, c_p, c_l, c_l, c_p, c_p, c_l, c_p, c_l, c_p, c_p, c_sz, c_i, c_p], True),
+    'ofx_gemm_f32_gn': (c_i, [c_p, c_l, c_p, c_l, c_l, c_p, c_l, c_l, c_p, c_p, c_l, c_p, c_l, c_p, c_sz,
+                              c_p, c_p, c_i, c_f, c_f, c_i, c_i, c_i, c_p, c_l, c_p], True),
+    'ofx_gemm_gn_plan': (c_i, [c_l, c_l, c_l, c_sz, c_i, c_i], False),
     'ofx_graphconv_fwd': (c_i, [c_p, c_l, c_i, c_l, c_p, c_p, c_p, c_p, c_p, c_l, c_p, c_p, c_l, c_i, c_p, c_l,
                                 c_i, c_p, c_p, c_l, c_p, c_p, c_l, c_p, c_l, c_p, c_l, c_p, c_sz, c_p], True),
     'ofx_planes_split': (c_i, [c_p, c_l, c_l, c_i, c_i, c_i, c_p, c_l, c_p], True),
@@ -129,6 +132,8 @@
     'ofx_pack_conv3d': (c_i, [c_p, c_i, c_i, c_p, c_p], True),
     'ofx_gridconv_fwd': (c_i, [c_p, c_l, c_i, c_l, c_l, c_p, c_p, c_p, c_p, c_i, c_p, c_p, c_l, c_p, c_p, c_l, c_p,
                                c_l, c_p, c_sz, c_p], True),
+    'ofx_gridconv_fwd_gn': (c_i, [c_p, c_l, c_i, c_l, c_l, c_p, c_p, c_p, c_p, c_i, c_p, c_p, c_l, c_p, c_p, c_l, c_p,
+                                  c_l, c_p, c_sz, c_p, c_p, c_i, c_f, c_f, c_i, c_i, c_i, c_p, c_l, c_p], True),
     'ofx_attention': (c_i, [c_p, c_l, c_i, c_i, c_i, c_i, c_p, c_l, c_p], True),
     'ofx_gather_mean': (c_i, [c_p, c_l, c_i, c_l, c_p, c_p, c_p, c_p], True),
     'ofx_gn_stats': (c_i, [c_p, c_l, c_l, c_i, c_p, c_i, c_p, c_p], True),
diff --git a/octfusion_amd/csrc/ofx_gemm.hip b/octfusion_amd/csrc/ofx_gemm.hip
--- a/octfusion_amd/csrc/ofx_gemm.hip
+++ b/octfusion_amd/csrc/ofx_gemm.hip
@@ -994,21 +994,14 @@
   return OFX_OK;
 }
 
-template <int MODE>
-static int launch_gemm(GemmArgs& g, float* ws, size_t ws_bytes, hipStream_t st) {
-  if (g.M <= 0 || g.N <= 0) return OFX_OK;
-  {
-    auto al16 = [](const void* p) { return (reinterpret_cast<uintptr_t>(p) & 15) == 0; };
-    g.vec4 = g.N % 4 == 0 && al16(g.out) && g.ldc % 4 == 0 && (!g.res || (al16(g.res) && g.ldr % 4 == 0)) &&
-             (!g.emb || (al16(g.emb) && g.lde % 4 == 0)) && (!g.bias || al16(g.bias));
-  }
+static int plan_split(GemmArgs& g, bool have_ws, size_t ws_bytes) {
   const int bn = g.N <= 32 ? 32 : (g.N <= 64 ? 64 : 128);
   g.ntm = (int)ofx_cdiv(g.M, BM);
   g.ntn = (int)ofx_cdiv(g.N, bn);
   const int nkt = (int)(g.Kp / BK);
   int nsplit = 1;
   const int tiles = g.ntm * g.ntn;
-  if (ws && tiles < 256 && nkt >= 8) {
+  if (have_ws && tiles < 256 && nkt >= 8) {
     nsplit = (int)ofx_cdiv(512, tiles);
     if (nsplit > nkt / 4) nsplit = nkt / 4;
     if (nsplit > 64) nsplit = 64;
@@ -1017,8 +1010,26 @@
     if (nsplit < 2) nsplit = 1;
   }
   g.kt_per_split = (int)ofx_cdiv(nkt, nsplit);
-  nsplit = (int)ofx_cdiv(nkt, g.kt_per_split);
-  g.nsplit = nsplit;
+  g.nsplit = (int)ofx_cdiv(nkt, g.kt_per_split);
+  return bn;
+}
+
+static int run_gn_tail(const GemmArgs& g, const GnTail& t, hipStream_t st) {
+  return ofx_gn_fused_rows(g.out, g.ldc, t.rows, t.batch, (int)g.N, t.groups, t.eps, t.count_eps, t.w, t.b, t.act, t.out,
+                           t.ldo, st);
+}
+
+template <int MODE>
+static int launch_gemm(GemmArgs& g, float* ws, size_t ws_bytes, hipStream_t st, const GnTail* tail = nullptr) {
+  if (g.M <= 0 || g.N <= 0) return OFX_OK;
+  if (tail && (g.out_rows || g.out_planes || g.stats)) return OFX_EINVAL;
+  {
+    auto al16 = [](const void* p) { return (reinterpret_cast<uintptr_t>(p) & 15) == 0; };
+    g.vec4 = g.N % 4 == 0 && al16(g.out) && g.ldc % 4 == 0 && (!g.res || (al16(g.res) && g.ldr % 4 == 0)) &&
+             (!g.emb || (al16(g.emb) && g.lde % 4 == 0)) && (!g.bias || al16(g.bias));
+  }
+  const int bn = plan_split(g, ws != nullptr, ws_bytes);
+  const int nsplit = g.nsplit;
   g.ws = ws;
   int rc;
   bool fast;
@@ -1049,7 +1060,11 @@
   if (rc) return rc;
   if (nsplit > 1) {
     const bool ws16 = (((uintptr_t)g.ws) & 15) == 0;
-    if (g.vec4 && ws16) splitk_reduce_v4_kernel<<<ofx_grid(g.M * (g.N >> 2), 256), 256, 0, st>>>(g);
+    if (tail && g.vec4 && ws16 && ofx_splitk_gn_ok(g, *tail)) {
+      rc = ofx_launch_splitk_reduce_gn(g, *tail, st);
+      if (rc) return rc;
+      tail = nullptr;
+    } else if (g.vec4 && ws16) splitk_reduce_v4_kernel<<<ofx_grid(g.M * (g.N >> 2), 256), 256, 0, st>>>(g);
     else splitk_reduce_kernel<<<ofx_grid(g.M * g.N, 256), 256, 0, st>>>(g);
   }
   if (g.stats_part) {
@@ -1057,6 +1072,7 @@
     if (rc) return rc;
   }
   OFX_LAUNCH_CHECK();
+  if (tail) return run_gn_tail(g, *tail, st);
   return OFX_OK;
 }
 
@@ -1166,6 +1182,48 @@
   return ofx_gemm_f32_planes(A, lda, a_rows, M, K, Wp, Kp, N, bias, res, ldr, out, ldc, out_rows, ws, ws_bytes, 0, stream);
 }
 
+static int gn_tail_args(GnTail& t, int64_t M, int64_t N, float*& out, int64_t& ldc, const float* gn_w, const float* gn_b,
+                        int groups, float eps, float count_eps, int act, int rows_per_batch, int batch_size, float* gn_out,
+                        int64_t ldo) {
+  if (!gn_w || !gn_b || !gn_out || groups < 1 || N % groups || rows_per_batch < 1 || batch_size < 1 ||
+      (int64_t)rows_per_batch * batch_size != M || ldo < N || act < 0 || act > OFX_ACT_GELU)
+    return OFX_EINVAL;
+  t.w = gn_w; t.b = gn_b; t.groups = groups; t.eps = eps; t.count_eps = count_eps; t.act = act;
+  t.rows = rows_per_batch; t.batch = batch_size; t.out = gn_out; t.ldo = ldo;
+  t.store_raw = out != nullptr;
+  if (!out) { out = gn_out; ldc = ldo; }
+  return OFX_OK;
+}
+
+extern "C" int ofx_gemm_f32_gn(const float* A, int64_t lda, const int32_t* a_rows, int64_t M, int64_t K, const float* Wp,
+                               int64_t Kp, int64_t N, const float* bias, const float* res, int64_t ldr, float* out,
+                               int64_t ldc, void* ws, size_t ws_bytes, const float* gn_w, const float* gn_b, int groups,
+                               float eps, float count_eps, int act, int rows_per_batch, int batch_size, float* gn_out,
+                               int64_t ldo, void* stream) {
+  if (M < 1 || N < 1) return OFX_EINVAL;
+  GnTail t = {};
+  if (int rc = gn_tail_args(t, M, N, out, ldc, gn_w, gn_b, groups, eps, count_eps, act, rows_per_batch, batch_size,
+                            gn_out, ldo))
+    return rc;
+  if (K < 1 || !Wp || !A || Kp != pad32(K) || lda < K || ldc < N || (res && ldr < N) || ((uintptr_t)Wp & 15))
+    return OFX_EINVAL;
+  GemmArgs g = {};
+  g.A = A; g.lda = lda; g.a_rows = a_rows;
+  g.M = M; g.K = K; g.Wp = Wp; g.Kp = Kp; g.N = N; g.bias = bias;
+  g.res = res; g.ldr = ldr; g.out = out; g.ldc = ldc;
+  return launch_gemm<MODE_DENSE>(g, (float*)ws, ws_bytes, ofx_stream(stream), &t);
+}
+
+extern "C" int ofx_gemm_gn_plan(int64_t M, int64_t N, int64_t Kp, size_t ws_bytes, int groups, int rows_per_batch) {
+  if (M < 1 || N < 1 || Kp < 32 || (Kp & 31) || groups < 1 || N % groups || rows_per_batch < 1) return 0;
+  GemmArgs g = {};
+  g.M = M; g.N = N; g.Kp = Kp;
+  GnTail t = {};
+  t.groups = groups; t.rows = rows_per_batch;
+  plan_split(g, ws_bytes > 0, ws_bytes);
+  return (g.nsplit > 1 && ofx_splitk_gn_ok(g, t)) ? g.nsplit : 0;
+}
+
 static int gather_common(GemmArgs& g, const float* x, int64_t ldx, int cin, int ndir, int64_t n_rows,
                          const int32_t* nbr, const int32_t* seg_ptr, const int32_t* col, const float* Wp, int64_t Kp,
                          int cout, const float* bias, const float* emb, int64_t lde, const int32_t* batch_id,
@@ -1196,7 +1254,7 @@
   }
 }
 
-template <int MODE> static int launch_gemm(GemmArgs& g, float* ws, size_t ws_bytes, hipStream_t st);
+template <int MODE> static int launch_gemm(GemmArgs& g, float* ws, size_t ws_bytes, hipStream_t st, const GnTail* tail);
 
 static int launch_gather_via_col(const GemmArgs& g, float* ws, size_t ws_bytes, hipStream_t st) {
   if (!ws || (((uintptr_t)ws) & 15)) return -1;
@@ -1657,6 +1715,36 @@
   return launch_gemm<MODE_GATHER>(g, (float*)ws, ws_bytes, ofx_stream(stream));
 }
 
+extern "C" int ofx_gridconv_fwd_gn(const float* x, int64_t ldx, int cin, int64_t n_in, int64_t n_out,
+                                   const int32_t* nbr27, const int32_t* nbr27_ext, const float* zero_row, const float* Wp,
+                                   int cout, const float* bias, const float* emb, int64_t lde, const int32_t* batch_id,
+                                   const float* res, int64_t ldr, float* out, int64_t ldc, void* ws, size_t ws_bytes,
+                                   const float* gn_w, const float* gn_b, int groups, float eps, float count_eps, int act,
+                                   int rows_per_batch, int batch_size, float* gn_out, int64_t ldo, void* stream) {
+  if (n_out < 1 || cout < 1) return OFX_EINVAL;
+  GnTail t = {};
+  int rc = gn_tail_args(t, n_out, cout, out, ldc, gn_w, gn_b, groups, eps, count_eps, act, rows_per_batch, batch_size,
+                        gn_out, ldo);
+  if (rc) return rc;
+  GemmArgs g = {};
+  const int64_t Kp = ofx_conv3d_packed_k(cin);
+  rc = gather_common(g, x, ldx, cin, 27, n_out, nbr27 ? nbr27 : nbr27_ext, nullptr, nullptr, Wp, Kp, cout, bias, emb, lde,
+                     batch_id, res, ldr, out, ldc);
+  if (rc) return rc;
+  if (n_in < 1) return OFX_EINVAL;
+  if (g.fast && nbr27_ext && zero_row && (((uintptr_t)zero_row & 15) == 0)) {
+    g.nbr_ext = nbr27_ext; g.aux = zero_row; g.ldaux = ldx; g.n_src = n_in;
+    g.tf = x; g.ldt = ldx;
+  } else if (!nbr27) {
+    return OFX_EINVAL;
+  }
+  if (!g.nbr_ext) {
+    rc = launch_gather_via_col(g, (float*)ws, ws_bytes, ofx_stream(stream));
+    if (rc >= 0) return rc ? rc : run_gn_tail(g, t, ofx_stream(stream));
+  }
+  return launch_gemm<MODE_GATHER>(g, (float*)ws, ws_bytes, ofx_stream(stream), &t);
+}
+
 extern "C" int ofx_gather_gemm_f32(const float* x, int64_t ldx, int cin, int ntap, int64_t n_src, int64_t n_out,
                                    const int32_t* tab, const float* zero_row, const float* Wp, int64_t Kp, int cout,
                                    const float* bias, const float* res, int64_t ldr, float* out, int64_t ldc,
diff --git a/octfusion_amd/csrc/ofx_gemm_common.h b/octfusion_amd/csrc/ofx_gemm_common.h
--- a/octfusion_amd/csrc/ofx_gemm_common.h
+++ b/octfusion_amd/csrc/ofx_gemm_common.h
@@ -29,6 +29,20 @@
   float* stats_part; size_t stats_part_bytes;
 };
 
+struct GnTail {
+  const float* w; const float* b;
+  int groups; float eps, count_eps; int act;
+  int rows, batch;
+  float* out; int64_t ldo;
+  int store_raw;
+};
+static inline bool ofx_splitk_gn_ok(const GemmArgs& g, const GnTail& t) {
+  const int64_t cpg = g.N / t.groups;
+  return (cpg == 2 || cpg == 4 || cpg == 8 || cpg == 16) && g.N % 16 == 0 && t.rows <= 512 && t.ldo % 4 == 0 &&
+         ((((uintptr_t)t.out | (uintptr_t)t.w | (uintptr_t)t.b) & 15) == 0);
+}
+int ofx_launch_splitk_reduce_gn(const GemmArgs& g, const GnTail& t, hipStream_t st);
+
 static __global__ void __launch_bounds__(256) weight_absmax_kernel(const float* __restrict__ W, int64_t sk, int64_t sn, int64_t K,
                                                             int64_t N, unsigned* __restrict__ acc) {
   __shared__ float red[256];
diff --git a/octfusion_amd/csrc/ofx_norm.hip b/octfusion_amd/csrc/ofx_norm.hip
--- a/octfusion_amd/csrc/ofx_norm.hip
+++ b/octfusion_amd/csrc/ofx_norm.hip
@@ -1035,3 +1035,102 @@
   OFX_LAUNCH_CHECK();
   return OFX_OK;
 }
+
+__global__ void __launch_bounds__(1024) splitk_reduce_gn_kernel(const GemmArgs g, const GnTail t) {
+  extern __shared__ double gn_smem[];
+  const int nsets = blockDim.x >> 8;
+  double* red = gn_smem;
+  float* stat = reinterpret_cast<float*>(red + nsets * 512);
+  float* slab = stat + 32;
+  const int rows = t.rows, G = t.groups;
+  const int cpg = (int)(g.N / G), gpb = 16 / cpg, bpb = (int)(g.N >> 4);
+  const int b = blockIdx.x / bpb, cb = (blockIdx.x - b * bpb) * 16;
+  const int64_t total = g.M * g.N;
+  float* raw = t.store_raw ? g.out : nullptr;
+  const float osc = g.oscale_p ? *g.oscale_p : 1.f;
+  for (int idx = threadIdx.x; idx < rows * 4; idx += blockDim.x) {
+    const int r = idx >> 2, n = cb + (idx & 3) * 4;
+    const int64_t m = (int64_t)b * rows + r;
+    const float* p = g.ws + m * g.N + n;
+    float4 v = f4zero();
+    int s = 0;
+    for (; s + 7 < g.nsplit; s += 8) {
+      float4 a[8];
+#pragma unroll
+      for (int u = 0; u < 8; ++u) a[u] = *reinterpret_cast<const float4*>(p + (int64_t)(s + u) * total);
+#pragma unroll
+      for (int u = 0; u < 8; ++u) f4add(v, a[u]);
+    }
+    for (; s + 3 < g.nsplit; s += 4) {
+      const float4 a0 = *reinterpret_cast<const float4*>(p + (int64_t)s * total);
+      const float4 a1 = *reinterpret_cast<const float4*>(p + (int64_t)(s + 1) * total);
+      const float4 a2 = *reinterpret_cast<const float4*>(p + (int64_t)(s + 2) * total);
+      const float4 a3 = *reinterpret_cast<const float4*>(p + (int64_t)(s + 3) * total);
+      f4add(v, a0); f4add(v, a1); f4add(v, a2); f4add(v, a3);
+    }
+    for (; s < g.nsplit; ++s) f4add(v, *reinterpret_cast<const float4*>(p + (int64_t)s * total));
+    if (g.oscale_p) { v.x *= osc; v.y *= osc; v.z *= osc; v.w *= osc; }
+    if (g.bias) f4add(v, *reinterpret_cast<const float4*>(g.bias + n));
+    if (g.emb) f4add(v, *reinterpret_cast<const float4*>(g.emb + (int64_t)g.bid[m] * g.lde + n));
+    if (g.res) f4add(v, *reinterpret_cast<const float4*>(g.res + m * g.ldr + n));
+    if (raw) *reinterpret_cast<float4*>(raw + m * g.ldc + n) = v;
+    *reinterpret_cast<float4*>(slab + idx * 4) = v;
+  }
+  __syncthreads();
+  const int set = threadIdx.x >> 8, u = threadIdx.x & 255;
+  const int csh = cpg == 2 ? 1 : (cpg == 4 ? 2 : (cpg == 8 ? 3 : 4));
+  const int gtotal = rows * cpg;
+  double* rs_ = red + set * 512;
+  double* rq_ = rs_ + 256;
+  for (int j0 = 0; j0 < gpb; j0 += nsets) {
+    const int j = j0 + set;
+    float s = 0.f, q = 0.f;
+    if (j < gpb)
+      for (int e = u; e < gtotal; e += 256) {
+        const float v = slab[(e >> csh) * 16 + j * cpg + (e & (cpg - 1))];
+        s += v; q += v * v;
+      }
+    rs_[u] = (double)s;
+    rq_[u] = (double)q;
+    __syncthreads();
+    for (int o = 128; o > 0; o >>= 1) {
+      if (u < o) { rs_[u] += rs_[u + o]; rq_[u] += rq_[u + o]; }
+      __syncthreads();
+    }
+    if (u == 0 && j < gpb) {
+      const double S = rs_[0], SS = rq_[0];
+      const float cnt = (float)rows * (float)cpg;
+      const float inv = 1.0f / (cnt + t.count_eps);
+      const double m = S * (double)inv;
+      const double ssd = SS - 2.0 * m * S + (double)cnt * m * m;
+      const double var = (ssd > 0 ? ssd : 0) * (double)inv;
+      stat[j * 2] = (float)m;
+      stat[j * 2 + 1] = (float)(1.0 / sqrt(var + (double)t.eps));
+    }
+    __syncthreads();
+  }
+  const int p4 = (threadIdx.x & 3) * 4;
+  const int ga = p4 / cpg, gb = (p4 + 3) / cpg;
+  const float ma = stat[ga * 2], ra = stat[ga * 2 + 1], mb = stat[gb * 2], rb = stat[gb * 2 + 1];
+  const float4 ww = *reinterpret_cast<const float4*>(t.w + cb + p4);
+  const float4 bb = *reinterpret_cast<const float4*>(t.b + cb + p4);
+  for (int idx = threadIdx.x; idx < rows * 4; idx += blockDim.x) {
+    const int r = idx >> 2;
+    const float4 v = *reinterpret_cast<const float4*>(slab + idx * 4);
+    float4 y;
+    y.x = ofx_apply_act((v.x - ma) * ra * ww.x + bb.x, t.act);
+    y.y = ofx_apply_act((v.y - ma) * ra * ww.y + bb.y, t.act);
+    y.z = ofx_apply_act((v.z - mb) * rb * ww.z + bb.z, t.act);
+    y.w = ofx_apply_act((v.w - mb) * rb * ww.w + bb.w, t.act);
+    *reinterpret_cast<float4*>(t.out + ((int64_t)b * rows + r) * t.ldo + cb + p4) = y;
+  }
+}
+
+int ofx_launch_splitk_reduce_gn(const GemmArgs& g, const GnTail& t, hipStream_t st) {
+  int threads = (t.rows * 4 + 255) / 256 * 256;
+  threads = threads > 1024 ? 1024 : threads;
+  const size_t lds = (size_t)(threads >> 8) * 512 * sizeof(double) + 32 * sizeof(float) + (size_t)t.rows * 16 * sizeof(float);
+  splitk_reduce_gn_kernel<<<t.batch * (int)(g.N >> 4), threads, lds, st>>>(g, t);
+  OFX_LAUNCH_CHECK();
+  return OFX_OK;
+}
diff --git a/octfusion_amd/graph_unet_lr.py b/octfusion_amd/graph_unet_lr.py
--- a/octfusion_amd/graph_unet_lr.py
+++ b/octfusion_amd/graph_unet_lr.py
@@ -104,11 +104,31 @@
 
 class GroupNorm32(nn.GroupNorm):
 
+    def tail(self, gs, act=None, out=None):
+        return ops.GnTail(self.weight, self.bias, self.num_groups, self.eps, act, 8 ** gs.depth, gs.B,
+                          gs.cache.batch_id(gs.depth), gs.cache.count(gs.depth), out)
+
     @torch.no_grad()
     def forward(self, x, gs, act=None, out=None):
+        done = ops.take_gn(x, self.tail(gs, act).key())
+        if done is not None and out is None:
+            return done
         return ops.group_norm(x, gs.cache.batch_id(gs.depth), gs.cache.count(gs.depth), gs.B, self.weight,
                               self.bias, self.num_groups, self.eps, act, out, count_eps=0.0,
                               rows_per_batch=8 ** gs.depth)
+
+
+def _hand_forward(y, yn, tail):
+    setattr(y, ops.GN_ATTR, (tail.key(), yn))
+    return y
+
+
+def _with_next(conv, nxt, nxt_only, gs_out, *args, **kw):
+    if nxt is None:
+        return conv(*args, **kw)
+    tail = nxt[0].tail(gs_out, nxt[1])
+    y, yn = conv(*args, gn_tail=tail, want_raw=not nxt_only, **kw)
+    return yn if nxt_only else _hand_forward(y, yn, tail)
 
 
 def convnormalization(channels):
@@ -136,13 +156,13 @@
         return depth + (0, -1, 1)[self.mode]
 
     @torch.no_grad()
-    def forward(self, x, gs, emb=None, res=None, out=None):
+    def forward(self, x, gs, emb=None, res=None, out=None, gn_tail=None, want_raw=True):
         d_out = self.out_depth(gs.depth)
         n_out = gs.B * 8 ** d_out
         bid = gs.cache.batch_id(d_out) if emb is not None else None
         mode = self.mode
         return ops.gridconv(x, lambda fast: gs.cache.table(mode, d_out, fast), n_out, self._pw.get(self.weight),
-                            self.bias, emb, bid, res, out)
+                            self.bias, emb, bid, res, out, gn_tail, want_raw)
 
 
 class _PointConv(nn.Module):
@@ -156,9 +176,9 @@
         self._pw = ops.PackedWeight()
 
     @torch.no_grad()
-    def forward(self, x, res=None, out=None):
+    def forward(self, x, res=None, out=None, gn_tail=None, want_raw=True):
         w = self.weight.view(self.weight.shape[0], self.weight.shape[1])
-        return ops.gemm(x, self._pw.get(w, 'nk'), self.bias, res, out)
+        return ops.gemm(x, self._pw.get(w, 'nk'), self.bias, res, out, gn_tail=gn_tail, want_raw=want_raw)
 
 
 class ConvUpsample(nn.Module):
@@ -182,11 +202,12 @@
         self.channels = channels
         self.op = GridConv3d(channels, channels, mode=1)
 
-    def forward(self, x, gs=None):
+    def forward(self, x, gs=None, nxt=None):
         if gs is None:
             rows, gs, back = _dense_io(x)
             return back(self.op(rows, gs), gs.depth - 1)
-        return self.op(x, gs), gs.at(gs.depth - 1)
+        down = gs.at(gs.depth - 1)
+        return _with_next(self.op, nxt, False, down, x, gs), down
 
 
 class ResnetBlock(nn.Module):
@@ -203,7 +224,7 @@
         self.res_conv = _PointConv(dim_in, dim_out, 3) if dim_in != dim_out else nn.Identity()
 
     @torch.no_grad()
-    def forward(self, x, emb_act, gs=None, out=None, t=None):
+    def forward(self, x, emb_act, gs=None, out=None, t=None, nxt=None, nxt_only=False):
         if gs is None:
             rows, gs, back = _dense_io(x)
             return back(self.forward(rows, ops.act(emb_act.float().contiguous(), 'silu'), gs), gs.depth)
@@ -218,11 +239,10 @@
         h = self.block1[0](x, gs, act='silu')
         if t is None:
             t = self.time_mlp[1](emb_act)
-        h = self.block1[2](h, gs, emb=t)
-        h = self.block2[0](h, gs, act='silu', out=h)
+        h = _with_next(self.block1[2], (self.block2[0], 'silu'), True, gs, h, gs, emb=t)
         if fork is not None:
             main.wait_stream(fork)
-        return self.block2[3](h, gs, res=skip, out=out)
+        return _with_next(self.block2[3], nxt, nxt_only, gs, h, gs, res=skip, out=out)
 
 
 class QKVAttention(nn.Module):
@@ -243,19 +263,19 @@
             p.detach().zero_()
 
     @torch.no_grad()
-    def forward(self, x, gs=None, out=None):
+    def forward(self, x, gs=None, out=None, nxt=None):
         if gs is None:
             rows, gs, back = _dense_io(x)
             return back(self.forward(rows, gs), gs.depth)
         qkv = self.qkv(self.norm(x, gs))
         h = ops.attention(qkv, gs.B, 8 ** gs.depth, self.num_heads)
-        return self.proj_out(h, res=x, out=out)
+        return _with_next(self.proj_out, nxt, False, gs, h, res=x, out=out)
 
 
 class _AttnSeq(nn.Sequential):
 
-    def forward(self, x, gs, out=None):
-        return self[2](self[0](x, gs, act='silu'), gs, out=out)
+    def forward(self, x, gs, out=None, nxt=None, normed=False):
+        return self[2](x if normed else self[0](x, gs, act='silu'), gs, out=out, nxt=nxt)
 
 
 class LearnedSinusoidalPosEmb(nn.Module):
@@ -389,25 +409,28 @@
             d_i = self.full_depth - min(i, nlev - 1)
             bufs[i] = torch.empty(batch_size * 8 ** d_i, 2 * cout[i], dtype=torch.float32, device=x.device)
 
-        def run_attn(m, x, gs, out=None):
-            return x if isinstance(m, our_Identity) else m(x, gs, out=out)
+        def norm1(resnet):
+            return (resnet.block1[0], 'silu')
+
+        def res_attn(resnet, self_attn, x, gs, out=None, nxt=None):
+            if isinstance(self_attn, our_Identity):
+                return resnet(x, emb_act, gs, out=out, t=tms[id(resnet)], nxt=nxt)
+            h = resnet(x, emb_act, gs, t=tms[id(resnet)], nxt=(self_attn[0], 'silu'), nxt_only=True)
+            return self_attn(h, gs, out=out, nxt=nxt, normed=True)
 
         for i, (resnet, self_attn, downsample) in enumerate(self.downs):
             slot = bufs[i][:, cout[i]:] if i in bufs else None
-            if isinstance(self_attn, our_Identity):
-                x = resnet(x, emb_act, gs, out=slot, t=tms[id(resnet)])
-            else:
-                x = run_attn(self_attn, resnet(x, emb_act, gs, t=tms[id(resnet)]), gs, out=slot)
-            if not isinstance(downsample, our_Identity):
-                x, gs = downsample(x, gs)
-        x = self.mid_block1(x, emb_act, gs, t=tms[id(self.mid_block1)])
-        x = run_attn(self.mid_self_attn, x, gs)
+            last = isinstance(downsample, our_Identity)
+            x = res_attn(resnet, self_attn, x, gs, out=slot, nxt=norm1(self.mid_block1) if last else None)
+            if not last:
+                x, gs = downsample(x, gs, nxt=norm1(self.downs[i + 1][0]))
+        x = res_attn(self.mid_block1, self.mid_self_attn, x, gs, nxt=norm1(self.mid_block2))
         x = self.mid_block2(x, emb_act, gs, out=bufs[nlev - 1][:, :cout[nlev - 1]] if nlev > 1 else None,
                             t=tms[id(self.mid_block2)])
         for j, (resnet, self_attn, upsample) in enumerate(self.ups):
             i = nlev - 1 - j
             x = bufs[i]
-            x = run_attn(self_attn, resnet(x, emb_act, gs, t=tms[id(resnet)]), gs)
+            x = res_attn(resnet, self_attn, x, gs)
             nxt = bufs[i - 1][:, :cout[i - 1]] if i - 1 in bufs else None
             x, gs = upsample(x, gs, out=nxt)
         x = self.end[0](x, gs, act='silu', out=out if as_middle else None)
diff --git a/octfusion_amd/ops.py b/octfusion_amd/ops.py
--- a/octfusion_amd/ops.py
+++ b/octfusion_amd/ops.py
@@ -413,12 +413,68 @@
         return self
 
 
-def gemm(a, pw, bias=None, res=None, out=None, a_rows=None, out_rows=None, m=None, out_planes=0):
+class GnTail(NamedTuple):
+    weight: torch.Tensor
+    bias: torch.Tensor
+    groups: int
+    eps: float
+    act: str
+    rows_per_batch: int
+    batch_size: int
+    batch_id: torch.Tensor
+    count: torch.Tensor
+    out: torch.Tensor = None
+
+    def key(self):
+        return (self.weight.data_ptr(), self.weight._version, self.bias.data_ptr(), self.bias._version, self.groups,
+                self.eps, ACT[self.act])
+
+
+GN_ATTR = '_ofx_gn_done'
+GN_TAIL = os.environ.get('OFX_GN_TAIL', '1') == '1'
+
+
+def _gn_tail_fused(t, C):
+    return GN_TAIL and t.rows_per_batch * (C // t.groups) <= (1 << 16) and t.rows_per_batch < GN_ROWS_TWO_KERNELS
+
+
+def _gn_tail_args(t, n, C, dev):
+    gn_out, ldo = _out2d(t.out, n, C, dev)
+    assert n == t.rows_per_batch * t.batch_size
+    range_words(dev)
+    return gn_out, (ptr(t.weight.detach().reshape(-1)), ptr(t.bias.detach().reshape(-1)), t.groups, t.eps, 0.0, ACT[t.act],
+                    t.rows_per_batch, t.batch_size, ptr(gn_out), ldo)
+
+
+def _gn_tail_after(y, t, want_raw):
+    out = t.out if t.out is not None or want_raw else y
+    yn = group_norm(y, t.batch_id, t.count, t.batch_size, t.weight, t.bias, t.groups, t.eps, t.act, out,
+                    count_eps=0.0, rows_per_batch=t.rows_per_batch)
+    return (y if want_raw else None), yn
+
+
+def take_gn(x, key):
+    done = getattr(x, GN_ATTR, None)
+    if done is None:
+        return None
+    delattr(x, GN_ATTR)
+    return done[1] if done[0] == key else None
+
+
+def gemm(a, pw, bias=None, res=None, out=None, a_rows=None, out_rows=None, m=None, out_planes=0, gn_tail=None,
+         want_raw=True):
+    if gn_tail is not None and (out_rows is not None or out_planes or not _gn_tail_fused(gn_tail, pw.N)):
+        if out_rows is not None or out_planes:
+            raise ValueError('gn_tail: fp32 rows without an output row map only')
+        return _gn_tail_after(gemm(a, pw, bias, res, out, a_rows, None, m), gn_tail, want_raw)
     a, lda = _row_major(a)
     M = m if m is not None else (a_rows.numel() if a_rows is not None else a.shape[0])
     if a.shape[1] != pw.K:
         raise ValueError('K mismatch: %d vs %d' % (a.shape[1], pw.K))
-    out, ldc = _out2d(out, M, pw.N, a.device)
+    if gn_tail is not None and not want_raw:
+        out, ldc = None, 0
+    else:
+        out, ldc = _out2d(out, M, pw.N, a.device)
     res, ldr = _row_major(res)
     _chk(bias)
     _chk(a_rows, torch.int32)
@@ -426,7 +482,11 @@
     ws = workspace(a.device)
     _meta('dense_gemm', 2.0 * M * pw.K * pw.N, 4.0 * (M * pw.K + pw.K * pw.N + M * pw.N * (2 if res is not None else 1)),
           (M, pw.K, pw.N))
-    if out_planes:
+    if gn_tail is not None:
+        gn_out, targs = _gn_tail_args(gn_tail, M, pw.N, a.device)
+        args = ('ofx_gemm_f32_gn', ptr(a), lda, ptr(a_rows), M, pw.K, ptr(pw.t), pw.Kp, pw.N, ptr(bias),
+                ptr(res), ldr, ptr(out), ldc, ptr(ws), ws.numel()) + targs + (stream(),)
+    elif out_planes:
         args = ('ofx_gemm_f32_planes', ptr(a), lda, ptr(a_rows), M, pw.K, ptr(pw.t), pw.Kp, pw.N, ptr(bias),
                 ptr(res), ldr, ptr(out), ldc, ptr(out_rows), ptr(ws), ws.numel(), out_planes, stream())
     else:
@@ -437,7 +497,7 @@
             call(*args)
     else:
         call(*args)
-    return out
+    return out if gn_tail is None else (out, gn_out)
 
 
 def gather_gemm(x, tab, ntap, pw, n_out, bias=None, res=None, out=None, out_rows=None, out_planes=0):
@@ -793,11 +853,16 @@
         return self
 
 
-def gridconv(x, tables, n_out, pw, bias=None, emb=None, batch_id=None, res=None, out=None):
+def gridconv(x, tables, n_out, pw, bias=None, emb=None, batch_id=None, res=None, out=None, gn_tail=None, want_raw=True):
+    if gn_tail is not None and not _gn_tail_fused(gn_tail, pw.N):
+        return _gn_tail_after(gridconv(x, tables, n_out, pw, bias, emb, batch_id, res, out), gn_tail, want_raw)
     x, ldx = _row_major(x)
     if x.shape[1] != pw.cin:
         raise ValueError('cin mismatch')
-    out, ldc = _out2d(out, n_out, pw.N, x.device)
+    if gn_tail is not None and not want_raw:
+        out, ldc = None, 0
+    else:
+        out, ldc = _out2d(out, n_out, pw.N, x.device)
     emb, lde = _row_major(emb)
     if emb is not None:
         _chk(batch_id, torch.int32)
@@ -811,9 +876,14 @@
         _meta('gridconv_27tap', flops,
               4.0 * (x.shape[0] * pw.cin + n_out * pw.N * (2 if res is not None else 1) + 27.0 * pw.cin * pw.N) + 4.0 * 27 * n_out,
               (n_out, pw.cin, pw.N))
-        call('ofx_gridconv_fwd', ptr(x), ldx, pw.cin, x.shape[0], n_out, None if fast else ptr(tables(False)),
-             ptr(tables(True)) if fast else None, ptr(zero_row(x.device)), ptr(pw.t), pw.N, ptr(bias), ptr(emb), lde,
-             ptr(batch_id) if emb is not None else None, ptr(res), ldr, ptr(out), ldc, ptr(ws), ws.numel(), stream())
+        args = (ptr(x), ldx, pw.cin, x.shape[0], n_out, None if fast else ptr(tables(False)),
+                ptr(tables(True)) if fast else None, ptr(zero_row(x.device)), ptr(pw.t), pw.N, ptr(bias), ptr(emb), lde,
+                ptr(batch_id) if emb is not None else None, ptr(res), ldr, ptr(out), ldc, ptr(ws), ws.numel())
+        if gn_tail is not None:
+            gn_out, targs = _gn_tail_args(gn_tail, n_out, pw.N, x.device)
+            call('ofx_gridconv_fwd_gn', *(args + targs + (stream(),)))
+            return out, gn_out
+        call('ofx_gridconv_fwd', *(args + (stream(),)))
     return out
 
 
```

Result: no change. 120.0 (-0.4%).
